# gevaertlab/RNA-GAN

Measured on AMD Instinct MI355X. Metric: training imgs/sec (G+D WGAN-GP step, 256x256), higher is better.
Workload: dtype bf16; 1 GPU; RNA-GAN lung (betaVAE-conditioned wganvae path) 256x256, DCGAN enc2048/step64, per-GPU batch 64, one iteration = G-loss + D-loss + GP steps; global_batch=64, parallelism=dp1, ranks=1, rna_features=19198, hip_graphs=True, dp_statistics=rank-local (DDP)

## Files before the change

include/rnagan_hip.h:

```cpp
#ifndef RNAGAN_HIP_H
#define RNAGAN_HIP_H

#include <stddef.h>
#include <stdint.h>

#ifdef __cplusplus
extern "C" {
#endif

#define RG_OK 0
#define RG_EINVAL (-1)
#define RG_EUNSUPPORTED (-2)
#define RG_EWORKSPACE (-3)
#define RG_EHIP (-4)

#define RG_F32 0
#define RG_BF16 1
#define RG_F16 2

#define RG_ALGO_AUTO 0
#define RG_ALGO_GENERIC 1
#define RG_ALGO_MFMA 2

int rg_version(void);
const char* rg_last_error(void);
int rg_set_option(const char* name, int value);


int rg_pack_conv_weight(const float* w, void* wdn, void* wup, int O, int I, int dtype, void* stream);
int rg_pack_conv_wup_from_bf16(const void* w_bf16, void* wup, int O, int I, void* stream);
int rg_pack_conv_wup_from_bf16_multi(int n, const void* const* w_bf16, void* const* wup, const int* O, const int* I, void* stream);
int rg_pack_g0_weight_from_bf16(const void* w_bf16, void* wp, int E, int C, void* stream);

int rg_conv_stats_rows(int up, int N, int Hlow, int Wlow, int O, int I, int dtype, int algo);
int rg_conv_down(const void* x, const float* w, const void* wdn, void* y, int N, int Hi, int Wi, int I,
                 int O, float* stats_partial, int dtype, int algo, void* ws, size_t ws_bytes, void* stream);
size_t rg_conv_workspace_bytes(int up, int N, int Hlow, int Wlow, int O, int I, int dtype, int algo);

int rg_conv_up(const void* x, const float* w, const void* wup, void* y, int N, int Ho, int Wo, int O, int I,
               const void* mask_act, float mask_slope, float* stats_partial, int dtype, int algo, void* ws,
               size_t ws_bytes, void* stream);

size_t rg_conv_wgrad_workspace_bytes(int N, int Ho, int Wo, int O, int I, int dtype, int algo);
int rg_conv_wgrad(const void* low, const void* high, float* dw, int N, int Ho, int Wo, int O, int I, int dtype,
                  int accumulate, int algo, void* ws, size_t ws_bytes, void* stream);
int rg_conv_wgrad2(const void* low0, const void* high0, const void* low1, const void* high1, float* dw, int N,
                   int Ho, int Wo, int O, int I, int dtype, int accumulate, int algo, void* ws, size_t ws_bytes,
                   void* stream);
int rg_conv_wgrad_slabs(const void* low0, const void* high0, const void* low1, const void* high1, float* dw, int N, int Ho,
                        int Wo, int O, int I, int dtype, int algo, void* slab, size_t slab_bytes, int* nsplit_out,
                        int* slab_dtype_out, void* stream);
int rg_conv_wgrad_adam_supported(int N, int Ho, int Wo, int O, int I, int two, int dtype, int algo);
int rg_conv_wgrad_adam(const void* low0, const void* high0, const void* low1, const void* high1, float* p, float* m, float* v,
                       const float* hyper, void* shadow_bf16, int N, int Ho, int Wo, int O, int I, int dtype, int algo,
                       void* stream);

int rg_first_down(const float* x_nchw, const float* w, const float* bias, void* y, int N, int H, int W, int I,
                  int O, float slope, int dtype, void* stream);
int rg_last_up(const void* x, const float* w, const float* bias, float* y_nchw, int N, int Ho, int Wo, int O,
               int I, int apply_tanh, int dtype, void* stream);
int rg_first_down_bits(const float* x_nchw, const float* w, const float* bias, void* y, void* bits, int N, int H, int W,
                       int I, int O, float slope, int dtype, void* stream);
int rg_sign_pack(const void* a, void* bits, long long npix, int C, int dtype, void* stream);
int rg_first_down_masked_supported(int H, int W, int I, int O, int dtype);
int rg_first_down_masked(const float* x_nchw, const float* w, void* y, const void* mask_bits, float mask_slope, int N,
                         int H, int W, int I, int O, int dtype, void* stream);
int rg_conv_up_maskbits_supported(int N, int Ho, int Wo, int O, int I, int dtype, int algo);
int rg_conv_up_maskbits(const void* x, const void* wup, void* y, int N, int Ho, int Wo, int O, int I,
                        const void* mask_bits, float mask_slope, int dtype, int algo, void* ws, size_t ws_bytes,
                        void* stream);
int rg_last_up_post_blocks(int N, int Ho, int Wo, int O, int I, int dtype);
int rg_last_up_post(const void* x, const float* w, float* y_nchw, int N, int Ho, int Wo, int O, int I, int dtype,
                    const float* tanh_img, float* part, void* stream);
int rg_last_up_part_chan_sum(const float* part, int nblocks, float* out3, int accumulate, void* stream);
int rg_gp_coef_parts(const float* part, int nblocks, float* sq, float* loss, float* coef, float lambd, void* stream);
int rg_gp_coef_parts_scaled(const float* part, int nblocks, float* sq, float* loss, float* coef, float lambd, float in_scale,
                            float out_scale, void* stream);
int rg_gp_coef_parts_scaled_dev(const float* part, int nblocks, float* sq, float* loss, float* coef, float lambd,
                                const int* amp_state, int slot, void* stream);
int rg_last_up_pre_supported(int Wo, int O, int I, int dtype);
int rg_last_up_pre(const void* z, const float* w, const float* bias, float* y_nchw, const float* mean, const float* invstd,
                   const float* gamma, const float* beta, float slope, int N, int Ho, int Wo, int O, int I, int apply_tanh,
                   int dtype, void* stream);
size_t rg_skinny_wgrad_workspace_bytes(int N, int Ho, int Wo, int O, int I);
int rg_skinny_wgrad(const void* low, const float* high_nchw, float* dw, int N, int Ho, int Wo, int O, int I,
                    int dtype, int accumulate, void* ws, size_t ws_bytes, void* stream);
int rg_skinny_wgrad_slabs(const void* low, const float* high_nchw, int N, int Ho, int Wo, int O, int I, int dtype, void* slab,
                          size_t slab_bytes, int* nslab_out, float* bias_slab, int* bias_done_out, void* stream);
int rg_skinny_wgrad_bias(const void* low, const float* high_nchw, float* dw, float* dbias, int N, int Ho, int Wo, int O, int I,
                         int dtype, int accumulate, int bias_accumulate, void* ws, size_t ws_bytes, int* bias_done_out,
                         void* stream);


int rg_pack_g0_weight(const float* w, void* wp, int E, int C, int dtype, void* stream);
int rg_g0_fwd(const float* z, const float* w, const void* wp, void* y, int N, int E, int C, int dtype, int algo,
              void* ws, size_t ws_bytes, void* stream);
size_t rg_g0_workspace_bytes(int N, int E, int C, int dtype, int algo);
int rg_g0_wgrad(const float* z, const void* gy, float* dw, int N, int E, int C, int dtype, int accumulate,
                int algo, void* ws, size_t ws_bytes, void* stream);

int rg_head_fwd(const void* a, const float* w, float* h, float* out, int N, int C, float slope, int dtype,
                void* stream);
int rg_head_fwd_bias(const void* a, const float* w, const float* bias, float* h, float* out, int N, int C, float slope,
                     int dtype, void* stream);
int rg_vec_sum(const float* x, int n, float* out, int accumulate, void* stream);
int rg_head_grad(const float* h, float* gh, int N, float coef, float slope, void* stream);
int rg_head_grad_dev(const float* h, float* gh, int N, float coef, const int* amp_state, int slot, int part, float slope,
                     void* stream);
int rg_head_bwd_data(const float* gh, const float* w, void* ga, int N, int C, int dtype, void* stream);
int rg_head_wgrad(const float* gh, const void* a, float* dw, int N, int C, int dtype, int accumulate,
                  void* stream);

int rg_pack_linear_weight(const float* w, void* wp, int Nout, int K, int Nout_pad, int K_pad, void* stream);
size_t rg_linear_workspace_bytes(int M, int K, int Nout, int algo);
int rg_linear_affine_act(const float* x, int ldx, const float* w, const void* wp, const float* scale,
                         const float* shift, float* y, int ldy, int M, int K, int Nout, float slope, int algo,
                         void* ws, size_t ws_bytes, void* stream);

size_t rg_colreduce_workspace_bytes(int M, int C, int nq);

int rg_bn_stats(const void* z, float* sum, float* sumsq, int M, int C, int dtype, void* ws, size_t ws_bytes,
                void* stream);
int rg_bn_finalize(const float* sum, const float* sumsq, int M, int C, float eps, float momentum, float* mean,
                   float* invstd, float* running_mean, float* running_var, int64_t* num_batches_tracked,
                   void* stream);
int rg_bn_forward(const void* z, int M, int C, float eps, float momentum, const float* gamma, const float* beta,
                  float slope, float* mean, float* invstd, float* running_mean, float* running_var,
                  int64_t* num_batches_tracked, void* a, int dtype, void* ws, size_t ws_bytes, void* stream);
int rg_bn_forward_partials(const float* partial, int G, const void* z, int M, int C, float eps, float momentum,
                           const float* gamma, const float* beta, float slope, float* mean, float* invstd,
                           float* running_mean, float* running_var, int64_t* num_batches_tracked, void* a, int dtype,
                           void* ws, size_t ws_bytes, void* stream);
int rg_bn_stats_finalize(const void* z, int M, int C, float eps, float momentum, float* mean, float* invstd,
                         float* running_mean, float* running_var, int64_t* num_batches_tracked, int dtype, void* ws,
                         size_t ws_bytes, void* stream);
int rg_bn_act(const void* z, const float* mean, const float* invstd, const float* gamma, const float* beta,
              void* a, int M, int C, float slope, int dtype, void* stream);
int rg_bn_act_bwd(const void* z, const void* ga, const float* mean, const float* invstd, const float* gamma,
                  const float* beta, void* gz, float* s_gy, float* s_gyxh, float* dgamma, float* dbeta,
                  int accumulate, int M, int C, float slope, int dtype, void* ws, size_t ws_bytes, void* stream);
int rg_bn_finalize_partials(const float* partial, int G, int M, int C, float eps, float momentum, float* mean,
                            float* invstd, float* running_mean, float* running_var, int64_t* num_batches_tracked, void* ws,
                            size_t ws_bytes, void* stream);
int rg_g0_wgrad_adam_supported(int N, int E, int C, int dtype);
int rg_g0_wgrad_adam(const float* z, const void* gz0, float* p, float* m, float* v, const float* hyper, void* shadow_bf16,
                     int N, int E, int C, int dtype, void* stream);

int rg_linear_wgrad_adam(const void* gT, const void* xT, int ldn, int N, float* p, float* m, float* v, const float* hyper, int O,
                         int I, void* wpack_bf16, int Kp, void* stream);

int rg_im2col_nhwc(const float* x, int ldx, float* cols, int N, int H, int W, int C, int kh, int kw, int sh, int sw, int ph,
                   int pw, void* stream);
int rg_pool2d_nhwc(const float* x, int ldx, float* y, int ldy, int N, int H, int W, int C, int k, int stride, int pad, int mode,
                   void* stream);
int rg_nchw_to_nhwc_affine(const float* x_nchw, float* y_nhwc, int N, int C, int H, int W, const float* scale, const float* shift,
                           void* stream);
int rg_spatial_mean_nhwc(const float* x, float* y, int N, int HW, int C, void* stream);

int rg_conv_split(int up, int N, int Hlow, int Wlow, int O, int I, int dtype, int algo);
int rg_conv_slab_dtype(int up, int N, int Hlow, int Wlow, int O, int I, int dtype, int algo);
int rg_conv_down_partial(const void* x, const void* wdn, int N, int Hi, int Wi, int I, int O, int dtype, int algo,
                         void* ws, size_t ws_bytes, void* stream);
int rg_conv_up_partial(const void* x, const void* wup, int N, int Ho, int Wo, int O, int I, int dtype, int algo,
                       void* ws, size_t ws_bytes, void* stream);
int rg_slab_bn_supported(long long M, int C, int groups, int nsplit);
size_t rg_slab_bn_scratch_bytes(long long M, int C, int groups);
size_t rg_slab_bn_sync_words(void);
int rg_bn_forward_slabs(const void* slab, int nsplit, size_t slab_stride, int slab_dtype, void* z, void* a, long long M, int C, int groups,
                        float eps, float momentum, const float* gamma, const float* beta, float slope, float* mean,
                        float* invstd, float* running_mean, float* running_var, long long* num_batches_tracked,
                        void* scratch, size_t scratch_bytes, void* sync, void* stream);
int rg_bn_tangent_slabs(const void* slab, int nsplit, size_t slab_stride, int slab_dtype, const void* z, void* zt_out, void* at, long long M,
                        int C, const float* mean, const float* invstd, const float* gamma, const float* beta, float slope,
                        float* s_zt, float* s_xhzt, void* scratch, size_t scratch_bytes, void* sync, void* stream);
int rg_bn_act_bwd_slabs(const void* slab, int nsplit, size_t slab_stride, int slab_dtype, const void* z, void* ga_out, void* gz, long long M,
                        int C, int groups, const float* mean, const float* invstd, const float* gamma, const float* beta,
                        float slope, float* s_gy, float* s_gyxh, float* dgamma, float* dbeta, int accumulate, void* scratch,
                        size_t scratch_bytes, void* sync, void* stream);

int rg_bn_finalize_partials_g2(const float* partial, int G, int nblk, int M, int C, float eps, float momentum, float* mean,
                               float* invstd, float* running_mean, float* running_var, int64_t* num_batches_tracked,
                               void* ws, size_t ws_bytes, void* stream);
int rg_bn_forward_g2(const float* partial, int G, int nblk, const void* z, int M, int C, float eps, float momentum,
                     const float* gamma, const float* beta, float slope, float* mean, float* invstd, float* running_mean,
                     float* running_var, int64_t* num_batches_tracked, void* a, int dtype, void* ws, size_t ws_bytes,
                     void* stream);
int rg_bn_act_bwd_g2(const void* z, const void* ga, const float* mean, const float* invstd, const float* gamma,
                     const float* beta, void* gz, float* s_gy, float* s_gyxh, float* dgamma, float* dbeta, int accumulate,
                     int M, int C, float slope, int dtype, void* ws, size_t ws_bytes, void* stream);
int rg_bn_tangent(const void* z, const void* zt, const float* mean, const float* invstd, const float* gamma,
                  const float* beta, void* at, float* s_zt, float* s_xhzt, int M, int C, float slope, int dtype,
                  void* ws, size_t ws_bytes, void* stream);
int rg_bn_double_bwd(const void* z, const void* qa, const void* zt, const void* ga1, const float* mean,
                     const float* invstd, const float* gamma, const float* beta, const float* s_gy,
                     const float* s_gyxh, const float* s_zt, const float* s_xhzt, void* pz, float* dgamma,
                     float* dbeta, int accumulate, int M, int C, float slope, int dtype, void* ws,
                     size_t ws_bytes, void* stream);

int rg_slab_finish_rows(long long M, int C);
int rg_slab_bias_act(const void* slab, int nsplit, size_t stride, int slab_dtype, const float* bias, void* y, long long M, int C,
                     float slope, void* stream);
int rg_slab_mask(const void* slab, int nsplit, size_t stride, int slab_dtype, const void* mask_act, float mask_slope, void* y,
                 float* col_parts, long long M, int C, void* stream);
int rg_parts_col_sum(const float* parts, int rows, int C, float* out, int accumulate, void* stream);
int rg_bias_act(const void* z, const float* bias, void* y, long long M, int C, float slope, int dtype, void* stream);
int rg_conv_down_epi_supported(int N, int Hi, int Wi, int I, int O, int dtype, int algo);
int rg_conv_down_epi(const void* x, const void* wdn, void* y, int N, int Hi, int Wi, int I, int O, const float* shift, float slope,
                     const void* mask_act, float mask_slope, int dtype, int algo, void* ws, size_t ws_bytes, void* stream);

int rg_lrelu_bwd(const void* g, const void* a, void* out, size_t n, float slope, int dtype, void* stream);
int rg_col_sum(const void* g, float* out, int M, int C, int dtype, int accumulate, void* ws, size_t ws_bytes,
               void* stream);

int rg_tanh_bwd(const float* gy, const float* y, float* gz, size_t n, void* stream);
int rg_nchw_chan_sum(const float* g, float* out, int N, int C, int HW, int accumulate, void* ws, size_t ws_bytes,
                     void* stream);
int rg_interp(const float* real, const float* fake, float* out, size_t n, float eps, void* stream);
int rg_interp_dev(const float* real, const float* fake, float* out, size_t n, const float* eps, void* stream);
size_t rg_reduce_workspace_bytes(size_t n);
int rg_sqnorm(const float* x, float* out, size_t n, void* ws, size_t ws_bytes, void* stream);
int rg_gp_coef(const float* sq, float* loss, float* coef, float lambd, void* stream);
int rg_gp_coef_scaled(const float* sq, float* loss, float* coef, float lambd, float in_scale, float out_scale, void* stream);
int rg_gp_coef_scaled_dev(const float* sq, float* loss, float* coef, float lambd, const int* amp_state, int slot, void* stream);
int rg_scale_by(const float* x, const float* coef, float* out, size_t n, void* stream);
int rg_mean_diff(const float* a, const float* b, float* out, int n, float sign, void* stream);
int rg_latent_prep(const float* u, const float* z, float* out, int N, int E, void* stream);

int rg_adam_step(float* p, const float* g, float* m, float* v, size_t n, int step, double lr, double beta1,
                 double beta2, double eps, void* stream);
int rg_clamp(float* p, size_t n, float lo, float hi, void* stream);
int rg_adam_step_dev(float* p, const float* g, float* m, float* v, size_t n, const float* hyper, void* shadow_bf16,
                     const void* grad_bf16, void* stream);
int rg_adam_step_slabs(float* p, const float* g, float* m, float* v, size_t n, const float* hyper, void* shadow_bf16, int nseg,
                       const unsigned long long* seg_off, const unsigned long long* seg_n, const void* const* seg_slab,
                       const int* seg_nsplit, const int* seg_dtype, void* stream);
int rg_grad_to_wire(const float* g, void* wire_bf16, size_t n, int nseg, const unsigned long long* seg_off,
                    const unsigned long long* seg_n, const void* const* seg_slab, const int* seg_nsplit, const int* seg_dtype,
                    void* stream);
int rg_conv_wgrad_wire(const void* low0, const void* high0, const void* low1, const void* high1, void* wire_bf16, int N, int Ho,
                       int Wo, int O, int I, int dtype, int algo, void* stream);
int rg_adam_hyper_dev(int* step_dev, double lr, double beta1, double beta2, double eps, double weight_decay, float* hyper,
                      void* stream);
int rg_adam_hyper_dev2(int* step_dev, double lr, double beta1, double beta2, double eps, double weight_decay,
                       double grad_scale_inv, float* hyper, void* stream);
#define RG_AMP_EXP 0
#define RG_AMP_TRACKER 1
#define RG_AMP_SKIPPED 2
#define RG_AMP_LATCH 4
#define RG_AMP_FLAG 8
#define RG_AMP_SLOTS 4
#define RG_AMP_STATE_INTS 12
int rg_adam_hyper_dev3(int* step_dev, double lr, double beta1, double beta2, double eps, double weight_decay,
                       const int* amp_state, int slot, float* hyper, void* stream);
int rg_ema_update(const float* p, float* e, size_t n, float decay, const int* step_dev, const float* hyper, void* stream);
int rg_nonfinite_probe(int nseg, const void* const* seg_ptr, const unsigned long long* seg_n, const int* seg_dtype, int* flag,
                       void* stream);
int rg_amp_update(int* amp_state, int slot, int growth_interval, int min_exp, int max_exp, void* stream);
int rg_amp_latch(int* amp_state, int slot, void* stream);
int rg_storage_dtype(void);

int rg_transpose_f32(const float* src, float* dst, int R, int C, void* stream);
int rg_transpose_pack_bf16(const float* src, void* dst, int R, int C, int R_pad, int C_pad, void* stream);
size_t rg_gemm_nt_bf16_workspace_bytes(int M, int K_pad, int Nout);
int rg_gemm_nt_bf16(const void* a, const void* b, const float* scale, const float* shift, float* y, int ldy, int M,
                    int K_pad, int Nout, float slope, void* ws, size_t ws_bytes, void* stream);
int rg_vae_dropout(const float* x, const unsigned char* mask, float* y, int N, int F, int ld, float scale, void* stream);
int rg_vae_reparam(const float* mu, const float* logvar, const float* eps, float* z, size_t n, void* stream);
int rg_vae_reparam_bwd(const float* gz, const float* logvar, const float* eps, const float* gmu_loss,
                       const float* glv_loss, float* gmu, float* glv, size_t n, void* stream);
int rg_tanh_inplace(float* x, size_t n, void* stream);
int rg_add_inplace(float* y, const float* x, size_t n, void* stream);
size_t rg_vae_loss_workspace_bytes(void);
int rg_vae_loss(const float* x, const float* x_recons, int N, int F, int ld, const float* z_mean, const float* z_logvar,
                int Z, float beta, int training, float* losses, float* g_recons, float* g_mean, float* g_logvar, void* ws,
                size_t ws_bytes, void* stream);

int rg_widen_bf16(const void* src, float* dst, size_t n, void* stream);
int rg_cast_pad(const float* src, void* dst, int M, int K, int ldd, int dtype, void* stream);

int rg_selftest_layouts(int* detail, void* stream);

size_t rg_upconv3_workspace_bytes(int N, int H, int W, int Cin, int Cout);
int rg_upconv3_fwd(const void* x, const float* w, const float* bias, void* y, int N, int H, int W, int Cin, int Cout,
                   int out_nchw_f32, int dtype, int algo, void* ws, size_t ws_bytes, void* stream);
int rg_upconv3_bwd_data(const void* gy, int gy_nchw_f32, const float* w, void* gx, int N, int H, int W, int Cin,
                        int Cout, int dtype, int algo, void* ws, size_t ws_bytes, void* stream);
int rg_upconv3_wgrad(const void* gy, int gy_nchw_f32, const void* x, float* dw, int N, int H, int W, int Cin, int Cout,
                     int dtype, int algo, int accumulate, void* ws, size_t ws_bytes, void* stream);

int rg_bn_bwd_sums(const void* z, const void* ga, const float* mean, const float* invstd, const float* gamma,
                   const float* beta, float* s_gy, float* s_gyxh, int M, int C, float slope, int dtype, void* ws,
                   size_t ws_bytes, void* stream);
int rg_bn_bwd_apply(const void* z, const void* ga, const float* mean, const float* invstd, const float* gamma,
                    const float* beta, const float* s_gy, const float* s_gyxh, void* gz, int M, int C, int M_total,
                    float slope, int dtype, void* stream);
int rg_bn_tangent_sums(const void* z, const void* zt, const float* mean, const float* invstd, const float* gamma,
                       const float* beta, float* s_zt, float* s_xhzt, int M, int C, float slope, int dtype, void* ws,
                       size_t ws_bytes, void* stream);
int rg_bn_tangent_apply(const void* z, const void* zt, const float* mean, const float* invstd, const float* gamma,
                        const float* beta, const float* s_zt, const float* s_xhzt, void* at, int M, int C, int M_total,
                        float slope, int dtype, void* stream);
int rg_bn_dbl_sums(const void* z, const void* qa, const void* zt, const void* ga1, const float* mean, const float* invstd,
                   const float* gamma, const float* beta, float* raw3, int M, int C, float slope, int dtype, void* ws,
                   size_t ws_bytes, void* stream);
int rg_bn_dbl_apply(const void* z, const void* qa, const void* zt, const void* ga1, const float* mean, const float* invstd,
                    const float* gamma, const float* beta, const float* s_gy, const float* s_gyxh, const float* s_zt,
                    const float* s_xhzt, const float* raw3_global, const float* raw3_local, void* pz, float* dgamma,
                    float* dbeta, int accumulate, int M, int C, int M_total, float slope, int dtype, void* ws,
                    size_t ws_bytes, void* stream);
int rg_latent_stats(const float* u, const float* z, float* s, float* ss, int N, int E, void* stream);
int rg_latent_apply(const float* u, const float* z, const float* s, const float* ss, float* out, int N, int E, int N_total,
                    void* stream);

int rg_export_images_nhwc(const float* x_nchw, float* y_nhwc, int N, int C, int H, int W, void* stream);

int rg_conv_up_affine(const void* x, const void* wup, void* y, int N, int Ho, int Wo, int O, int I, const float* scale,
                      const float* shift, float slope, void* ws, size_t ws_bytes, void* stream);
int rg_g0_fwd_affine(const float* z, const void* wp, void* y, int N, int E, int C, const float* scale, const float* shift,
                     float slope, void* ws, size_t ws_bytes, void* stream);

int rg_conv_up_fp8(const void* x8, const void* wup8, void* y, int N, int Ho, int Wo, int O, int I, const float* scale,
                   const float* shift, float slope, int out_fp8, void* stream);
int rg_gemm_fp8(const void* a8, const void* b8, void* y, int M, int K, int Ncols, const float* scale, const float* shift,
                float slope, int out_fp8, void* stream);
int rg_fp8_supported(int M, int K, int Ncols, int taps);
int rg_cast_fp8(const float* src, void* dst, size_t n, float mul, void* stream);
int rg_selftest_fp8(int* detail, void* stream);

int rg_u8_to_norm(const void* src_u8, float* dst, size_t n, float mean, float stdv, void* stream);

int rg_split_planes(const float* src, void* planes_bf16, size_t n, void* stream);
int rg_f32p_conv_supported(int up, int N, int Hlow, int Wlow, int O, int I, int products);
size_t rg_f32p_conv_workspace_bytes(int up, int N, int Hlow, int Wlow, int O, int I, int products);
int rg_f32p_conv_stats_rows(int up, int N, int Hlow, int Wlow, int O, int I, int products);
int rg_f32p_conv(int up, const void* x_planes, const void* w_planes, float* y, int N, int Hlow, int Wlow, int O, int I,
                 int products, float* stats_partial, const float* mask_f32, float mask_slope, void* ws, size_t ws_bytes,
                 void* stream);
int rg_f32p_conv_mask_supported(int up, int N, int Hlow, int Wlow, int O, int I, int products);
int rg_f32p_wgrad_supported(int N, int Ho, int Wo, int O, int I, int products);
size_t rg_f32p_wgrad_workspace_bytes(int N, int Ho, int Wo, int O, int I, int products, int two);
int rg_f32p_wgrad(const void* low0, const void* high0, const void* low1, const void* high1, float* dw, int N, int Ho, int Wo,
                  int O, int I, int products, int accumulate, void* ws, size_t ws_bytes, void* stream);

int rg_probe_mfma_bare(int mfma_shape, int waves_per_simd, int blocks, int iters, float* scratch, double* flops_out, void* stream);
int rg_probe_lds_mfma(int mfma_shape, int blocks, int iters, const void* a, const void* b, void* c, double* flops_out,
                      void* stream);
int rg_probe_copy(const void* src, void* dst, size_t nbytes, int variant, int blocks, void* stream);
int rg_probe_fill_bf16(void* p, size_t n, unsigned seed, void* stream);


#ifdef __cplusplus
}
#endif
#endif
```

rna_gan_amd/_abi.py:

```python
from __future__ import annotations

import ctypes as C
import os

_HERE = os.path.dirname(os.path.abspath(__file__))
LIB_PATH = os.path.join(_HERE, "librnagan_hip.so")

RG_F32, RG_BF16, RG_F16 = 0, 1, 2
ALGO_AUTO, ALGO_GENERIC, ALGO_MFMA = 0, 1, 2

_p = C.c_void_p
_i = C.c_int
_f = C.c_float
_d = C.c_double
_z = C.c_size_t

PROTOTYPES = {
    "rg_version": (_i, []),
    "rg_last_error": (C.c_char_p, []),
    "rg_set_option": (_i, [C.c_char_p, _i]),
    "rg_pack_conv_weight": (_i, [_p, _p, _p, _i, _i, _i, _p]),
    "rg_conv_stats_rows": (_i, [_i, _i, _i, _i, _i, _i, _i, _i]),
    "rg_conv_down": (_i, [_p, _p, _p, _p, _i, _i, _i, _i, _i, _p, _i, _i, _p, _z, _p]),
    "rg_conv_up": (_i, [_p, _p, _p, _p, _i, _i, _i, _i, _i, _p, _f, _p, _i, _i, _p, _z, _p]),
    "rg_conv_workspace_bytes": (_z, [_i, _i, _i, _i, _i, _i, _i, _i]),
    "rg_conv_wgrad_workspace_bytes": (_z, [_i, _i, _i, _i, _i, _i, _i]),
    "rg_conv_wgrad": (_i, [_p, _p, _p, _i, _i, _i, _i, _i, _i, _i, _i, _p, _z, _p]),
    "rg_conv_wgrad2": (_i, [_p, _p, _p, _p, _p, _i, _i, _i, _i, _i, _i, _i, _i, _p, _z, _p]),
    "rg_conv_wgrad_slabs": (_i, [_p, _p, _p, _p, _p, _i, _i, _i, _i, _i, _i, _i, _p, _z, _p, _p, _p]),
    "rg_grad_to_wire": (_i, [_p, _p, _z, _i, _p, _p, _p, _p, _p, _p]),
    "rg_conv_wgrad_wire": (_i, [_p, _p, _p, _p, _p, _i, _i, _i, _i, _i, _i, _i, _p]),
    "rg_conv_wgrad_adam_supported": (_i, [_i, _i, _i, _i, _i, _i, _i, _i]),
    "rg_conv_wgrad_adam": (_i, [_p, _p, _p, _p, _p, _p, _p, _p, _p, _i, _i, _i, _i, _i, _i, _i, _p]),
    "rg_first_down": (_i, [_p, _p, _p, _p, _i, _i, _i, _i, _i, _f, _i, _p]),
    "rg_first_down_bits": (_i, [_p, _p, _p, _p, _p, _i, _i, _i, _i, _i, _f, _i, _p]),
    "rg_sign_pack": (_i, [_p, _p, C.c_longlong, _i, _i, _p]),
    "rg_first_down_masked_supported": (_i, [_i, _i, _i, _i, _i]),
    "rg_first_down_masked": (_i, [_p, _p, _p, _p, _f, _i, _i, _i, _i, _i, _i, _p]),
    "rg_conv_up_maskbits_supported": (_i, [_i, _i, _i, _i, _i, _i, _i]),
    "rg_conv_up_maskbits": (_i, [_p, _p, _p, _i, _i, _i, _i, _i, _p, _f, _i, _i, _p, _z, _p]),
    "rg_last_up": (_i, [_p, _p, _p, _p, _i, _i, _i, _i, _i, _i, _i, _p]),
    "rg_skinny_wgrad_workspace_bytes": (_z, [_i, _i, _i, _i, _i]),
    "rg_skinny_wgrad": (_i, [_p, _p, _p, _i, _i, _i, _i, _i, _i, _i, _p, _z, _p]),
    "rg_skinny_wgrad_slabs": (_i, [_p, _p, _i, _i, _i, _i, _i, _i, _p, _z, _p, _p, _p, _p]),
    "rg_skinny_wgrad_bias": (_i, [_p, _p, _p, _p, _i, _i, _i, _i, _i, _i, _i, _i, _p, _z, _p, _p]),
    "rg_pack_g0_weight": (_i, [_p, _p, _i, _i, _i, _p]),
    "rg_pack_conv_wup_from_bf16": (_i, [_p, _p, _i, _i, _p]),
    "rg_pack_conv_wup_from_bf16_multi": (_i, [_i, _p, _p, _p, _p, _p]),
    "rg_pack_g0_weight_from_bf16": (_i, [_p, _p, _i, _i, _p]),
    "rg_g0_fwd": (_i, [_p, _p, _p, _p, _i, _i, _i, _i, _i, _p, _z, _p]),
    "rg_g0_workspace_bytes": (_z, [_i, _i, _i, _i, _i]),
    "rg_g0_wgrad": (_i, [_p, _p, _p, _i, _i, _i, _i, _i, _i, _p, _z, _p]),
    "rg_head_fwd": (_i, [_p, _p, _p, _p, _i, _i, _f, _i, _p]),
    "rg_head_grad": (_i, [_p, _p, _i, _f, _f, _p]),
    "rg_head_grad_dev": (_i, [_p, _p, _i, _f, _p, _i, _i, _f, _p]),
    "rg_adam_hyper_dev3": (_i, [_p, _d, _d, _d, _d, _d, _p, _i, _p, _p]),
    "rg_nonfinite_probe": (_i, [_i, _p, _p, _p, _p, _p]),
    "rg_amp_update": (_i, [_p, _i, _i, _i, _i, _p]),
    "rg_amp_latch": (_i, [_p, _i, _p]),
    "rg_gp_coef_scaled_dev": (_i, [_p, _p, _p, _f, _p, _i, _p]),
    "rg_gp_coef_parts_scaled_dev": (_i, [_p, _i, _p, _p, _p, _f, _p, _i, _p]),
    "rg_head_bwd_data": (_i, [_p, _p, _p, _i, _i, _i, _p]),
    "rg_head_wgrad": (_i, [_p, _p, _p, _i, _i, _i, _i, _p]),
    "rg_pack_linear_weight": (_i, [_p, _p, _i, _i, _i, _i, _p]),
    "rg_linear_workspace_bytes": (_z, [_i, _i, _i, _i]),
    "rg_linear_affine_act": (_i, [_p, _i, _p, _p, _p, _p, _p, _i, _i, _i, _i, _f, _i, _p, _z, _p]),
    "rg_colreduce_workspace_bytes": (_z, [_i, _i, _i]),
    "rg_bn_stats": (_i, [_p, _p, _p, _i, _i, _i, _p, _z, _p]),
    "rg_bn_finalize": (_i, [_p, _p, _i, _i, _f, _f, _p, _p, _p, _p, _p, _p]),
    "rg_bn_forward": (_i, [_p, _i, _i, _f, _f, _p, _p, _f, _p, _p, _p, _p, _p, _p, _i, _p, _z, _p]),
    "rg_bn_forward_partials": (_i, [_p, _i, _p, _i, _i, _f, _f, _p, _p, _f, _p, _p, _p, _p, _p, _p, _i, _p, _z, _p]),
    "rg_bn_stats_finalize": (_i, [_p, _i, _i, _f, _f, _p, _p, _p, _p, _p, _i, _p, _z, _p]),
    "rg_bn_act": (_i, [_p, _p, _p, _p, _p, _p, _i, _i, _f, _i, _p]),
    "rg_bn_act_bwd": (_i, [_p, _p, _p, _p, _p, _p, _p, _p, _p, _p, _p, _i, _i, _i, _f, _i, _p, _z, _p]),
    "rg_bn_act_bwd_g2": (_i, [_p, _p, _p, _p, _p, _p, _p, _p, _p, _p, _p, _i, _i, _i, _f, _i, _p, _z, _p]),
    "rg_bn_finalize_partials": (_i, [_p, _i, _i, _i, _f, _f, _p, _p, _p, _p, _p, _p, _z, _p]),
    "rg_linear_wgrad_adam": (_i, [_p, _p, _i, _i, _p, _p, _p, _p, _i, _i, _p, _i, _p]),
    "rg_last_up_post_blocks": (_i, [_i, _i, _i, _i, _i, _i]),
    "rg_last_up_post": (_i, [_p, _p, _p, _i, _i, _i, _i, _i, _i, _p, _p, _p]),
    "rg_last_up_part_chan_sum": (_i, [_p, _i, _p, _i, _p]),
    "rg_gp_coef_parts": (_i, [_p, _i, _p, _p, _p, _f, _p]),
    "rg_last_up_pre_supported": (_i, [_i, _i, _i, _i]),
    "rg_last_up_pre": (_i, [_p, _p, _p, _p, _p, _p, _p, _p, _f, _i, _i, _i, _i, _i, _i, _i, _p]),
    "rg_bn_forward_g2": (_i, [_p, _i, _i, _p, _i, _i, _f, _f, _p, _p, _f, _p, _p, _p, _p, _p, _p, _i, _p, _z, _p]),
    "rg_bn_finalize_partials_g2": (_i, [_p, _i, _i, _i, _i, _f, _f, _p, _p, _p, _p, _p, _p, _z, _p]),
    "rg_bn_tangent": (_i, [_p, _p, _p, _p, _p, _p, _p, _p, _p, _i, _i, _f, _i, _p, _z, _p]),
    "rg_bn_double_bwd": (_i, [_p, _p, _p, _p, _p, _p, _p, _p, _p, _p, _p, _p, _p, _p, _p, _i, _i, _i, _f, _i,
                              _p, _z, _p]),
    "rg_lrelu_bwd": (_i, [_p, _p, _p, _z, _f, _i, _p]),
    "rg_col_sum": (_i, [_p, _p, _i, _i, _i, _i, _p, _z, _p]),
    "rg_tanh_bwd": (_i, [_p, _p, _p, _z, _p]),
    "rg_nchw_chan_sum": (_i, [_p, _p, _i, _i, _i, _i, _p, _z, _p]),
    "rg_interp": (_i, [_p, _p, _p, _z, _f, _p]),
    "rg_reduce_workspace_bytes": (_z, [_z]),
    "rg_sqnorm": (_i, [_p, _p, _z, _p, _z, _p]),
    "rg_gp_coef": (_i, [_p, _p, _p, _f, _p]),
    "rg_scale_by": (_i, [_p, _p, _p, _z, _p]),
    "rg_mean_diff": (_i, [_p, _p, _p, _i, _f, _p]),
    "rg_latent_prep": (_i, [_p, _p, _p, _i, _i, _p]),
    "rg_adam_step": (_i, [_p, _p, _p, _p, _z, _i, _d, _d, _d, _d, _p]),
    "rg_clamp": (_i, [_p, _z, _f, _f, _p]),
    "rg_upconv3_workspace_bytes": (_z, [_i, _i, _i, _i, _i]),
    "rg_upconv3_fwd": (_i, [_p, _p, _p, _p, _i, _i, _i, _i, _i, _i, _i, _i, _p, _z, _p]),
    "rg_upconv3_bwd_data": (_i, [_p, _i, _p, _p, _i, _i, _i, _i, _i, _i, _i, _p, _z, _p]),
    "rg_upconv3_wgrad": (_i, [_p, _i, _p, _p, _i, _i, _i, _i, _i, _i, _i, _i, _p, _z, _p]),
    "rg_export_images_nhwc": (_i, [_p, _p, _i, _i, _i, _i, _p]),
    "rg_bn_bwd_sums": (_i, [_p, _p, _p, _p, _p, _p, _p, _p, _i, _i, _f, _i, _p, _z, _p]),
    "rg_bn_bwd_apply": (_i, [_p, _p, _p, _p, _p, _p, _p, _p, _p, _i, _i, _i, _f, _i, _p]),
    "rg_bn_tangent_sums": (_i, [_p, _p, _p, _p, _p, _p, _p, _p, _i, _i, _f, _i, _p, _z, _p]),
    "rg_bn_tangent_apply": (_i, [_p, _p, _p, _p, _p, _p, _p, _p, _p, _i, _i, _i, _f, _i, _p]),
    "rg_bn_dbl_sums": (_i, [_p, _p, _p, _p, _p, _p, _p, _p, _p, _i, _i, _f, _i, _p, _z, _p]),
    "rg_bn_dbl_apply": (_i, [_p] * 17 + [_i, _i, _i, _i, _f, _i, _p, _z, _p]),
    "rg_latent_stats": (_i, [_p, _p, _p, _p, _i, _i, _p]),
    "rg_latent_apply": (_i, [_p, _p, _p, _p, _p, _i, _i, _i, _p]),
    "rg_adam_step_dev": (_i, [_p, _p, _p, _p, _z, _p, _p, _p, _p]),
    "rg_adam_step_slabs": (_i, [_p, _p, _p, _p, _z, _p, _p, _i, _p, _p, _p, _p, _p, _p]),
    "rg_ema_update": (_i, [_p, _p, _z, _f, _p, _p, _p]),
    "rg_interp_dev": (_i, [_p, _p, _p, _z, _p, _p]),
    "rg_adam_hyper_dev": (_i, [_p, _d, _d, _d, _d, _d, _p, _p]),
    "rg_adam_hyper_dev2": (_i, [_p, _d, _d, _d, _d, _d, _d, _p, _p]),
    "rg_storage_dtype": (_i, []),
    "rg_gp_coef_scaled": (_i, [_p, _p, _p, _f, _f, _f, _p]),
    "rg_gp_coef_parts_scaled": (_i, [_p, _i, _p, _p, _p, _f, _f, _f, _p]),
    "rg_transpose_f32": (_i, [_p, _p, _i, _i, _p]),
    "rg_transpose_pack_bf16": (_i, [_p, _p, _i, _i, _i, _i, _p]),
    "rg_gemm_nt_bf16_workspace_bytes": (_z, [_i, _i, _i]),
    "rg_gemm_nt_bf16": (_i, [_p, _p, _p, _p, _p, _i, _i, _i, _i, _f, _p, _z, _p]),
    "rg_vae_dropout": (_i, [_p, _p, _p, _i, _i, _i, _f, _p]),
    "rg_vae_reparam": (_i, [_p, _p, _p, _p, _z, _p]),
    "rg_vae_reparam_bwd": (_i, [_p, _p, _p, _p, _p, _p, _p, _z, _p]),
    "rg_tanh_inplace": (_i, [_p, _z, _p]),
    "rg_add_inplace": (_i, [_p, _p, _z, _p]),
    "rg_vae_loss_workspace_bytes": (_z, []),
    "rg_vae_loss": (_i, [_p, _p, _i, _i, _i, _p, _p, _i, _f, _i, _p, _p, _p, _p, _p, _z, _p]),
    "rg_widen_bf16": (_i, [_p, _p, _z, _p]),
    "rg_cast_pad": (_i, [_p, _p, _i, _i, _i, _i, _p]),
    "rg_selftest_layouts": (_i, [_p, _p]),
    "rg_u8_to_norm": (_i, [_p, _p, _z, _f, _f, _p]),
    "rg_conv_up_fp8": (_i, [_p, _p, _p, _i, _i, _i, _i, _i, _p, _p, _f, _i, _p]),
    "rg_gemm_fp8": (_i, [_p, _p, _p, _i, _i, _i, _p, _p, _f, _i, _p]),
    "rg_fp8_supported": (_i, [_i, _i, _i, _i]),
    "rg_cast_fp8": (_i, [_p, _p, _z, _f, _p]),
    "rg_selftest_fp8": (_i, [_p, _p]),
    "rg_g0_wgrad_adam_supported": (_i, [_i, _i, _i, _i]),
    "rg_g0_wgrad_adam": (_i, [_p, _p, _p, _p, _p, _p, _p, _i, _i, _i, _i, _p]),
    "rg_im2col_nhwc": (_i, [_p, _i, _p, _i, _i, _i, _i, _i, _i, _i, _i, _i, _i, _p]),
    "rg_pool2d_nhwc": (_i, [_p, _i, _p, _i, _i, _i, _i, _i, _i, _i, _i, _i, _p]),
    "rg_nchw_to_nhwc_affine": (_i, [_p, _p, _i, _i, _i, _i, _p, _p, _p]),
    "rg_spatial_mean_nhwc": (_i, [_p, _p, _i, _i, _i, _p]),
    "rg_conv_split": (_i, [_i, _i, _i, _i, _i, _i, _i, _i]),
    "rg_conv_slab_dtype": (_i, [_i, _i, _i, _i, _i, _i, _i, _i]),
    "rg_conv_down_partial": (_i, [_p, _p, _i, _i, _i, _i, _i, _i, _i, _p, _z, _p]),
    "rg_conv_up_partial": (_i, [_p, _p, _i, _i, _i, _i, _i, _i, _i, _p, _z, _p]),
    "rg_slab_bn_supported": (_i, [C.c_longlong, _i, _i, _i]),
    "rg_slab_bn_scratch_bytes": (_z, [C.c_longlong, _i, _i]),
    "rg_slab_bn_sync_words": (_z, []),
    "rg_bn_forward_slabs": (_i, [_p, _i, _z, _i, _p, _p, C.c_longlong, _i, _i, _f, _f, _p, _p, _f, _p, _p, _p, _p, _p, _p, _z, _p, _p]),
    "rg_bn_tangent_slabs": (_i, [_p, _i, _z, _i, _p, _p, _p, C.c_longlong, _i, _p, _p, _p, _p, _f, _p, _p, _p, _z, _p, _p]),
    "rg_bn_act_bwd_slabs": (_i, [_p, _i, _z, _i, _p, _p, _p, C.c_longlong, _i, _i, _p, _p, _p, _p, _f, _p, _p, _p, _p, _i, _p, _z,
                                 _p, _p]),
    "rg_conv_up_affine": (_i, [_p, _p, _p, _i, _i, _i, _i, _i, _p, _p, _f, _p, _z, _p]),
    "rg_g0_fwd_affine": (_i, [_p, _p, _p, _i, _i, _i, _p, _p, _f, _p, _z, _p]),
    "rg_split_planes": (_i, [_p, _p, _z, _p]),
    "rg_f32p_conv_supported": (_i, [_i, _i, _i, _i, _i, _i, _i]),
    "rg_f32p_conv_workspace_bytes": (_z, [_i, _i, _i, _i, _i, _i, _i]),
    "rg_f32p_conv_stats_rows": (_i, [_i, _i, _i, _i, _i, _i, _i]),
    "rg_f32p_conv": (_i, [_i, _p, _p, _p, _i, _i, _i, _i, _i, _i, _p, _p, _f, _p, _z, _p]),
    "rg_f32p_conv_mask_supported": (_i, [_i, _i, _i, _i, _i, _i, _i]),
    "rg_f32p_wgrad_supported": (_i, [_i, _i, _i, _i, _i, _i]),
    "rg_f32p_wgrad_workspace_bytes": (_z, [_i, _i, _i, _i, _i, _i, _i]),
    "rg_f32p_wgrad": (_i, [_p, _p, _p, _p, _p, _i, _i, _i, _i, _i, _i, _i, _p, _z, _p]),
    "rg_slab_finish_rows": (_i, [C.c_longlong, _i]),
    "rg_slab_bias_act": (_i, [_p, _i, _z, _i, _p, _p, C.c_longlong, _i, _f, _p]),
    "rg_slab_mask": (_i, [_p, _i, _z, _i, _p, _f, _p, _p, C.c_longlong, _i, _p]),
    "rg_parts_col_sum": (_i, [_p, _i, _i, _p, _i, _p]),
    "rg_bias_act": (_i, [_p, _p, _p, C.c_longlong, _i, _f, _i, _p]),
    "rg_vec_sum": (_i, [_p, _i, _p, _i, _p]),
    "rg_conv_down_epi_supported": (_i, [_i, _i, _i, _i, _i, _i, _i]),
    "rg_conv_down_epi": (_i, [_p, _p, _p, _i, _i, _i, _i, _i, _p, _f, _p, _f, _i, _i, _p, _z, _p]),
    "rg_head_fwd_bias": (_i, [_p, _p, _p, _p, _p, _i, _i, _f, _i, _p]),
    "rg_probe_mfma_bare": (_i, [_i, _i, _i, _i, _p, _p, _p]),
    "rg_probe_lds_mfma": (_i, [_i, _i, _i, _p, _p, _p, _p, _p]),
    "rg_probe_copy": (_i, [_p, _p, _z, _i, _i, _p]),
    "rg_probe_fill_bf16": (_i, [_p, _z, C.c_uint, _p]),
}

ABI_VERSION = 615

_libs = {}
LIB_PATH_F16 = os.path.join(_HERE, "librnagan_hip_f16.so")
BF16_ONLY_PREFIXES = ("rg_probe_", "rg_split_planes", "rg_f32p_")


def load(half: str = "bf16"):
    if half in _libs:
        return _libs[half]
    if half not in ("bf16", "f16"):
        raise ValueError("half must be 'bf16' or 'f16'")
    path = LIB_PATH if half == "bf16" else LIB_PATH_F16
    if not os.path.exists(path):
        raise RuntimeError(
            "rna_gan_amd: %s not found. Build it with `python -m rna_gan_amd.build` "
            "(hipcc --offload-arch=gfx950). There is no CPU / eager fallback." % path)
    try:
        lib = C.CDLL(path)
    except OSError as e:
        raise RuntimeError("rna_gan_amd: cannot load %s: %s" % (path, e))
    for name, (res, args) in PROTOTYPES.items():
        if half == "f16" and name.startswith(BF16_ONLY_PREFIXES):
            continue
        fn = getattr(lib, name, None)
        if fn is None:
            raise RuntimeError("rna_gan_amd: symbol %s missing from %s: the library is older than this package -- rebuild "
                               "it with `python -m rna_gan_amd.build`" % (name, path))
        fn.restype = res
        fn.argtypes = args
    got = lib.rg_version()
    if got != ABI_VERSION:
        raise RuntimeError("rna_gan_amd: %s reports ABI version %d, this package binds version %d (a stale or swapped "
                           "build): rebuild it with `python -m rna_gan_amd.build`" % (path, got, ABI_VERSION))
    want = RG_BF16 if half == "bf16" else RG_F16
    if lib.rg_storage_dtype() != want:
        raise RuntimeError("rna_gan_amd: %s stores dtype code %d, expected %d (a swapped build)" % (path, lib.rg_storage_dtype(), want))
    _libs[half] = lib
    return lib


_LAST_ERR_LIBS = ("bf16", "f16")


def check(rc: int, what: str):
    if rc != 0:
        msgs = []
        for h in _LAST_ERR_LIBS:
            if h in _libs:
                m = _libs[h].rg_last_error()
                if m:
                    msgs.append(m.decode() if len(_libs) == 1 else "[%s build] %s" % (h, m.decode()))
        raise RuntimeError("rna_gan_amd: %s failed (%d): %s" % (what, rc, " | ".join(msgs) if msgs else "?"))
```

rna_gan_amd/build.py:

```python
import os
import subprocess
import sys
from concurrent.futures import ThreadPoolExecutor

HERE = os.path.dirname(os.path.abspath(__file__))
CSRC = os.path.join(HERE, "csrc")
OUT = os.path.join(HERE, "librnagan_hip.so")
OUT_F16 = os.path.join(HERE, "librnagan_hip_f16.so")
OBJ = os.path.join(HERE, "csrc", "_obj")
SOURCES = ["rg_api.hip", "rg_generic.hip", "rg_bn.hip", "rg_misc.hip", "rg_mfma.hip", "rg_conv8.hip", "rg_convp.hip", "rg_convd.hip", "rg_wgrad8.hip", "rg_skinny.hip", "rg_vae.hip", "rg_splitbn.hip", "rg_incep.hip", "rg_g0adam.hip", "rg_upimg.hip", "rg_probe.hip", "rg_conv8f.hip", "rg_wgrad8f.hip", "rg_amp.hip", "rg_plainact.hip"]
EXTRA_DEPS = {"rg_probe.hip": ["rg_conv8.hip"], "rg_conv8f.hip": ["rg_conv8.hip"], "rg_wgrad8f.hip": ["rg_wgrad8.hip"]}
BF16_ONLY = ("rg_probe.hip", "rg_conv8f.hip", "rg_wgrad8f.hip")
FLAGS = ["--offload-arch=gfx950", "-O3", "-fPIC", "-std=c++17", "-Wall", "-Wno-unused-function",
         "-ffp-contract=off"]


def _stale(target, deps):
    if not os.path.exists(target):
        return True
    t = os.path.getmtime(target)
    return any(os.path.getmtime(d) > t for d in deps)


def build_library(force=False, verbose=True, half="bf16"):
    if half not in ("bf16", "f16"):
        raise ValueError("half must be 'bf16' or 'f16'")
    hipcc = os.environ.get("HIPCC", "/opt/rocm/bin/hipcc")
    if not os.path.exists(hipcc):
        hipcc = "hipcc"
    f16 = half == "f16"
    objdir = OBJ + ("_f16" if f16 else "")
    out = OUT_F16 if f16 else OUT
    sources = [s for s in SOURCES if not (f16 and s in BF16_ONLY)]
    flags = FLAGS + (["-DRG_HALF_F16=1"] if f16 else [])
    os.makedirs(objdir, exist_ok=True)
    headers = [os.path.join(CSRC, f) for f in os.listdir(CSRC) if f.endswith(".h")]
    headers.append(os.path.join(os.path.dirname(HERE), "include", "rnagan_hip.h"))
    jobs = []
    for s in sources:
        src = os.path.join(CSRC, s)
        obj = os.path.join(objdir, s.replace(".hip", ".o"))
        if force or _stale(obj, [src] + headers + [os.path.join(CSRC, d) for d in EXTRA_DEPS.get(s, [])]):
            jobs.append((src, obj))

    def cc(job):
        src, obj = job
        cmd = [hipcc] + flags + ["-c", src, "-o", obj]
        r = subprocess.run(cmd, capture_output=True, text=True)
        if r.returncode != 0:
            raise RuntimeError("hipcc failed for %s:\n%s" % (src, r.stderr[-4000:]))
        if verbose and r.stderr.strip():
            sys.stderr.write(r.stderr[-2000:])
        return obj

    with ThreadPoolExecutor(max_workers=6) as ex:
        list(ex.map(cc, jobs))
    objs = [os.path.join(objdir, s.replace(".hip", ".o")) for s in sources]
    if force or jobs or _stale(out, objs):
        cmd = [hipcc, "--offload-arch=gfx950", "-shared", "-fPIC", "-o", out] + objs
        r = subprocess.run(cmd, capture_output=True, text=True)
        if r.returncode != 0:
            raise RuntimeError("link failed:\n%s" % r.stderr[-4000:])
    return out


def build_all(force=False, verbose=True):
    return [build_library(force, verbose, "bf16"), build_library(force, verbose, "f16")]


def build_debug_library(force=False):
    hipcc = os.environ.get("HIPCC", "/opt/rocm/bin/hipcc")
    if not os.path.exists(hipcc):
        hipcc = "hipcc"
    d = os.path.join(os.path.dirname(HERE), "tools", "debug")
    src = os.path.join(d, "rg_debug_hold.hip")
    d_out = d if os.access(d, os.W_OK) else os.path.join(os.path.expanduser("~"), ".cache", "rna_gan_amd")
    os.makedirs(d_out, exist_ok=True)
    out = os.path.join(d_out, "librnagan_debug.so")
    if force or _stale(out, [src]):
        tmp = "%s.%d.tmp" % (out, os.getpid())
        r = subprocess.run([hipcc, "--offload-arch=gfx950", "-O3", "-fPIC", "-shared", "-o", tmp, src], capture_output=True, text=True)
        if r.returncode != 0:
            raise RuntimeError("hipcc failed for %s:\n%s" % (src, r.stderr[-4000:]))
        os.replace(tmp, out)
    return out


if __name__ == "__main__":
    print("\n".join(build_all(force="--force" in sys.argv)))
```

rna_gan_amd/csrc/rg_api.hip:

```cpp
#include "rg_common.h"
#include "rg_internal.h"
#include <stdarg.h>
#include <stdio.h>
#include <stdlib.h>
#include <string.h>
#include <ctype.h>

static thread_local char g_err[512] = "";

void rg_set_error(const char* fmt, ...) {
  va_list ap;
  va_start(ap, fmt);
  vsnprintf(g_err, sizeof(g_err), fmt, ap);
  va_end(ap);
}

extern "C" int rg_version(void) { return 615; }
extern "C" const char* rg_last_error(void) { return g_err; }

static const char* const g_opt_names[] = {"conv8", "conv8_blocks", "conv_tile", "xcd", "class_fast", "wgrad_blocks",
                                          "wgrad8", "conv_v1", "stream_tile", "narrow8", "conv8_mfma", "conv8_epi", "wgrad8_blocks", "korder", "convp", "convp_blocks",
                                          "fp8_mx", "wgrad8n", "f32mma", "convd", "convd_blocks", "skinny128", "slab16", "wslab16", "bn_rev", "wgrad8_mfma", "narrow32", "upimg", "upimg_blocks"};
constexpr int G_NOPT = sizeof(g_opt_names) / sizeof(g_opt_names[0]);
static int g_opt_override[G_NOPT];
static int g_opt_env[G_NOPT];

int rg_option(const char* name, int dflt) {
  for (int i = 0; i < G_NOPT; ++i) {
    if (strcmp(name, g_opt_names[i]) != 0) continue;
    if (g_opt_override[i] > 0) return g_opt_override[i] - 1;
    if (g_opt_env[i] == 0) {
      char var[64] = "RNAGAN_";
      size_t n = strlen(var);
      for (const char* c = name; *c && n + 1 < sizeof(var); ++c) var[n++] = (char)toupper((unsigned char)*c);
      var[n] = 0;
      const char* e = getenv(var);
      g_opt_env[i] = e ? atoi(e) + 1 : -1;
      if (g_opt_env[i] == 0) g_opt_env[i] = -1;
    }
    return g_opt_env[i] > 0 ? g_opt_env[i] - 1 : dflt;
  }
  return dflt;
}

extern "C" int rg_set_option(const char* name, int value) {
  RG_REQUIRE(name, RG_EINVAL, "set_option: null name");
  for (int i = 0; i < G_NOPT; ++i)
    if (strcmp(name, g_opt_names[i]) == 0) { g_opt_override[i] = value < 0 ? 0 : value + 1; return RG_OK; }
  rg_set_error("set_option: unknown option '%s'", name);
  return RG_EINVAL;
}

static bool want_mfma(int algo, int dtype) { return algo != RG_ALGO_GENERIC && dtype == RG_H16; }

extern "C" int rg_pack_conv_weight(const float* w, void* wdn, void* wup, int O, int I, int dtype, void* stream) {
  RG_REQUIRE(w && O > 0 && I > 0, RG_EINVAL, "pack_conv_weight: bad args");
  RG_REQUIRE(dtype == RG_H16, RG_EUNSUPPORTED, "pack_conv_weight: only bf16 packs exist (fp32 kernels read w)");
  return rg_mfma_pack_conv_weight(w, wdn, wup, O, I, rg_stream(stream));
}

extern "C" size_t rg_conv_workspace_bytes(int up, int N, int Hlow, int Wlow, int O, int I, int dtype, int algo) {
  if (!want_mfma(algo, dtype)) return 0;
  if (!rg_mfma_conv_supported(N, Hlow, Wlow, up ? O : I, up ? I : O)) return 0;
  return rg_mfma_conv_ws_bytes(up, N, Hlow, Wlow, O, I);
}

extern "C" int rg_conv_stats_rows(int up, int N, int Hlow, int Wlow, int O, int I, int dtype, int algo) {
  if (N <= 0 || Hlow <= 0 || Wlow <= 0 || O <= 0 || I <= 0 || !want_mfma(algo, dtype)) return 0;
  if (!rg_mfma_conv_supported(N, Hlow, Wlow, up ? O : I, up ? I : O)) return 0;
  return rg_mfma_conv_stats_rows(up, N, Hlow, Wlow, O, I);
}

extern "C" int rg_conv_split(int up, int N, int Hlow, int Wlow, int O, int I, int dtype, int algo) {
  if (N <= 0 || Hlow <= 0 || Wlow <= 0 || O <= 0 || I <= 0 || !want_mfma(algo, dtype)) return 1;
  if (!rg_mfma_conv_supported(N, Hlow, Wlow, up ? O : I, up ? I : O)) return 1;
  return rg_mfma_conv_nsplit(up, N, Hlow, Wlow, O, I);
}

extern "C" int rg_conv_slab_dtype(int up, int N, int Hlow, int Wlow, int O, int I, int dtype, int algo) {
  if (rg_conv_split(up, N, Hlow, Wlow, O, I, dtype, algo) <= 1) return RG_F32;
  return rg_mfma_conv_slab16(up, N, Hlow, Wlow, O, I) ? RG_H16 : RG_F32;
}

extern "C" int rg_conv_down_partial(const void* x, const void* wdn, int N, int Hi, int Wi, int I, int O, int dtype, int algo,
                                    void* ws, size_t ws_bytes, void* stream) {
  RG_REQUIRE(x && wdn && ws && N > 0 && Hi > 0 && Wi > 0 && I > 0 && O > 0 && Hi % 2 == 0 && Wi % 2 == 0, RG_EINVAL,
             "conv_down_partial: bad args");
  RG_REQUIRE(rg_conv_split(0, N, Hi / 2, Wi / 2, O, I, dtype, algo) > 1, RG_EUNSUPPORTED,
             "conv_down_partial: this shape does not run split-K (rg_conv_split)");
  return rg_mfma_conv_down(x, wdn, nullptr, N, Hi, Wi, I, O, nullptr, ws, ws_bytes, rg_stream(stream), 1);
}

extern "C" int rg_conv_up_partial(const void* x, const void* wup, int N, int Ho, int Wo, int O, int I, int dtype, int algo,
                                  void* ws, size_t ws_bytes, void* stream) {
  RG_REQUIRE(x && wup && ws && N > 0 && Ho > 0 && Wo > 0 && I > 0 && O > 0, RG_EINVAL, "conv_up_partial: bad args");
  RG_REQUIRE(rg_conv_split(1, N, Ho, Wo, O, I, dtype, algo) > 1, RG_EUNSUPPORTED,
             "conv_up_partial: this shape does not run split-K (rg_conv_split)");
  return rg_mfma_conv_up(x, wup, nullptr, N, Ho, Wo, O, I, nullptr, 1.f, nullptr, ws, ws_bytes, rg_stream(stream), nullptr,
                         nullptr, 1.f, 0, 1);
}

extern "C" int rg_conv_down(const void* x, const float* w, const void* wdn, void* y, int N, int Hi, int Wi, int I,
                            int O, float* stats_partial, int dtype, int algo, void* ws, size_t ws_bytes, void* stream) {
  RG_REQUIRE(x && y && N > 0 && Hi > 0 && Wi > 0 && I > 0 && O > 0 && Hi % 2 == 0 && Wi % 2 == 0, RG_EINVAL,
             "conv_down: bad args");
  if (want_mfma(algo, dtype) && wdn && rg_mfma_conv_supported(N, Hi / 2, Wi / 2, I, O))
    return rg_mfma_conv_down(x, wdn, y, N, Hi, Wi, I, O, stats_partial, ws, ws_bytes, rg_stream(stream));
  RG_REQUIRE(!stats_partial, RG_EUNSUPPORTED, "conv_down: statistics come from the MFMA epilogue only");
  RG_REQUIRE(algo != RG_ALGO_MFMA, RG_EUNSUPPORTED, "conv_down: shape/dtype not supported by the MFMA kernel");
  RG_REQUIRE(w, RG_EINVAL, "conv_down: generic kernel needs the fp32 master weight");
  return rg_generic_conv_down(x, w, y, N, Hi, Wi, I, O, dtype, rg_stream(stream));
}

extern "C" int rg_conv_up(const void* x, const float* w, const void* wup, void* y, int N, int Ho, int Wo, int O, int I,
                          const void* mask_act, float mask_slope, float* stats_partial, int dtype, int algo, void* ws,
                          size_t ws_bytes, void* stream) {
  RG_REQUIRE(x && y && N > 0 && Ho > 0 && Wo > 0 && I > 0 && O > 0, RG_EINVAL, "conv_up: bad args");
  RG_REQUIRE(!(mask_act && stats_partial), RG_EINVAL, "conv_up: mask and statistics are exclusive");
  if (want_mfma(algo, dtype) && wup && rg_mfma_conv_supported(N, Ho, Wo, O, I))
    return rg_mfma_conv_up(x, wup, y, N, Ho, Wo, O, I, mask_act, mask_slope, stats_partial, ws, ws_bytes,
                           rg_stream(stream));
  RG_REQUIRE(!stats_partial, RG_EUNSUPPORTED, "conv_up: statistics come from the MFMA epilogue only");
  RG_REQUIRE(algo != RG_ALGO_MFMA, RG_EUNSUPPORTED, "conv_up: shape/dtype not supported by the MFMA kernel");
  RG_REQUIRE(w, RG_EINVAL, "conv_up: generic kernel needs the fp32 master weight");
  return rg_generic_conv_up(x, w, y, N, Ho, Wo, O, I, mask_act, mask_slope, dtype, rg_stream(stream));
}

extern "C" size_t rg_conv_wgrad_workspace_bytes(int N, int Ho, int Wo, int O, int I, int dtype, int algo) {
  size_t a = rg_generic_wgrad_ws_bytes(N, Ho, Wo, O, I);
  size_t b = 0;
  if (want_mfma(algo, dtype) && rg_mfma_wgrad_supported(N, Ho, Wo, O, I)) {
    b = rg_mfma_wgrad_ws_bytes(N, Ho, Wo, O, I);
    size_t c = rg_mfma_wgrad2_ws_bytes(N, Ho, Wo, O, I);
    if (c > b) b = c;
  }
  return a > b ? a : b;
}

extern "C" int rg_conv_wgrad2(const void* low0, const void* high0, const void* low1, const void* high1, float* dw,
                              int N, int Ho, int Wo, int O, int I, int dtype, int accumulate, int algo, void* ws,
                              size_t ws_bytes, void* stream) {
  RG_REQUIRE(low0 && high0 && low1 && high1 && dw && N > 0 && Ho > 0 && Wo > 0 && I > 0 && O > 0, RG_EINVAL,
             "conv_wgrad2: bad args");
  if (want_mfma(algo, dtype) && rg_mfma_wgrad_supported(N, Ho, Wo, O, I))
    return rg_mfma_conv_wgrad2(low0, high0, low1, high1, dw, N, Ho, Wo, O, I, accumulate, ws, ws_bytes,
                               rg_stream(stream));
  RG_REQUIRE(algo != RG_ALGO_MFMA, RG_EUNSUPPORTED, "conv_wgrad2: shape/dtype not supported by the MFMA kernel");
  int rc = rg_generic_conv_wgrad(low0, high0, dw, N, Ho, Wo, O, I, dtype, accumulate, ws, ws_bytes, rg_stream(stream));
  if (rc) return rc;
  return rg_generic_conv_wgrad(low1, high1, dw, N, Ho, Wo, O, I, dtype, 1, ws, ws_bytes, rg_stream(stream));
}

extern "C" int rg_conv_wgrad_slabs(const void* low0, const void* high0, const void* low1, const void* high1, float* dw, int N,
                                   int Ho, int Wo, int O, int I, int dtype, int algo, void* slab, size_t slab_bytes,
                                   int* nsplit_out, int* slab_dtype_out, void* stream) {
  RG_REQUIRE(low0 && high0 && dw && nsplit_out && slab_dtype_out && (low1 == nullptr) == (high1 == nullptr) && N > 0 && Ho > 0 &&
                 Wo > 0 && I > 0 && O > 0, RG_EINVAL, "conv_wgrad_slabs: bad args");
  *slab_dtype_out = RG_F32;
  if (!(want_mfma(algo, dtype) && rg_mfma_wgrad_supported(N, Ho, Wo, O, I))) {
    *nsplit_out = 1;
    RG_REQUIRE(algo != RG_ALGO_MFMA, RG_EUNSUPPORTED, "conv_wgrad_slabs: shape/dtype not supported by the MFMA kernel");
    int rc = rg_generic_conv_wgrad(low0, high0, dw, N, Ho, Wo, O, I, dtype, 0, slab, slab_bytes, rg_stream(stream));
    if (rc || !low1) return rc;
    return rg_generic_conv_wgrad(low1, high1, dw, N, Ho, Wo, O, I, dtype, 1, slab, slab_bytes, rg_stream(stream));
  }
  return rg_mfma_conv_wgrad2(low0, high0, low1, high1, dw, N, Ho, Wo, O, I, 0, slab, slab_bytes, rg_stream(stream), nsplit_out,
                             slab_dtype_out);
}

extern "C" int rg_conv_wgrad_adam_supported(int N, int Ho, int Wo, int O, int I, int two, int dtype, int algo) {
  return N > 0 && Ho > 0 && Wo > 0 && O > 0 && I > 0 && want_mfma(algo, dtype) && rg_mfma_wgrad_supported(N, Ho, Wo, O, I) &&
         rg_mfma_conv_wgrad_adam_supported(N, Ho, Wo, O, I, two != 0) ? 1 : 0;
}
extern "C" int rg_conv_wgrad_adam(const void* low0, const void* high0, const void* low1, const void* high1, float* p, float* m,
                                  float* v, const float* hyper, void* shadow_bf16, int N, int Ho, int Wo, int O, int I, int dtype,
                                  int algo, void* stream) {
  RG_REQUIRE(low0 && high0 && p && m && v && hyper && (low1 == nullptr) == (high1 == nullptr) && N > 0 && Ho > 0 && Wo > 0 &&
                 I > 0 && O > 0, RG_EINVAL, "conv_wgrad_adam: bad args");
  RG_REQUIRE((((uintptr_t)p | (uintptr_t)m | (uintptr_t)v) & 15) == 0 && ((uintptr_t)shadow_bf16 & 7) == 0, RG_EINVAL,
             "conv_wgrad_adam: p, m, v must be 16-byte aligned (the bf16 image 8-byte)");
  RG_REQUIRE(rg_conv_wgrad_adam_supported(N, Ho, Wo, O, I, low1 != nullptr, dtype, algo), RG_EUNSUPPORTED,
             "conv_wgrad_adam: shape / dtype without a single-split matrix-core plan");
  return rg_mfma_conv_wgrad_adam(low0, high0, low1, high1, N, Ho, Wo, O, I, p, m, v, (uint16_t*)shadow_bf16, hyper,
                                 rg_stream(stream));
}

extern "C" int rg_conv_wgrad_wire(const void* low0, const void* high0, const void* low1, const void* high1, void* wire_bf16, int N,
                                  int Ho, int Wo, int O, int I, int dtype, int algo, void* stream) {
  RG_REQUIRE(low0 && high0 && wire_bf16 && (low1 == nullptr) == (high1 == nullptr) && N > 0 && Ho > 0 && Wo > 0 && I > 0 && O > 0,
             RG_EINVAL, "conv_wgrad_wire: bad args");
  RG_REQUIRE(((uintptr_t)wire_bf16 & 15) == 0, RG_EINVAL, "conv_wgrad_wire: the wire slice must be 16-byte aligned");
  RG_REQUIRE(rg_conv_wgrad_adam_supported(N, Ho, Wo, O, I, low1 != nullptr, dtype, algo), RG_EUNSUPPORTED,
             "conv_wgrad_wire: shape / dtype without a single-split matrix-core plan");
  return rg_mfma_conv_wgrad_wire(low0, high0, low1, high1, N, Ho, Wo, O, I, (uint16_t*)wire_bf16, rg_stream(stream));
}

extern "C" int rg_conv_wgrad(const void* low, const void* high, float* dw, int N, int Ho, int Wo, int O, int I,
                             int dtype, int accumulate, int algo, void* ws, size_t ws_bytes, void* stream) {
  RG_REQUIRE(low && high && dw && N > 0 && Ho > 0 && Wo > 0 && I > 0 && O > 0, RG_EINVAL, "conv_wgrad: bad args");
  if (want_mfma(algo, dtype) && rg_mfma_wgrad_supported(N, Ho, Wo, O, I))
    return rg_mfma_conv_wgrad2(low, high, nullptr, nullptr, dw, N, Ho, Wo, O, I, accumulate, ws, ws_bytes,
                               rg_stream(stream));
  RG_REQUIRE(algo != RG_ALGO_MFMA, RG_EUNSUPPORTED, "conv_wgrad: shape/dtype not supported by the MFMA kernel");
  return rg_generic_conv_wgrad(low, high, dw, N, Ho, Wo, O, I, dtype, accumulate, ws, ws_bytes, rg_stream(stream));
}

extern "C" int rg_first_down(const float* x_nchw, const float* w, const float* bias, void* y, int N, int H, int W,
                             int I, int O, float slope, int dtype, void* stream) {
  RG_REQUIRE(x_nchw && w && y && N > 0 && H > 0 && W > 0 && H % 2 == 0 && W % 2 == 0 && I > 0 && O > 0, RG_EINVAL,
             "first_down: bad args");
  if (rg_skinny_supported(I, O) && !(dtype == RG_F32 && rg_generic_f32_image_side(N, H, W, I, O)))
    return rg_skinny_first_down(x_nchw, w, bias, y, nullptr, N, H, W, I, O, slope, dtype, rg_stream(stream));
  return rg_generic_first_down(x_nchw, w, bias, y, N, H, W, I, O, slope, dtype, rg_stream(stream));
}

extern "C" int rg_first_down_bits(const float* x_nchw, const float* w, const float* bias, void* y, void* bits, int N, int H,
                                  int W, int I, int O, float slope, int dtype, void* stream) {
  RG_REQUIRE(x_nchw && w && y && bits && N > 0 && H > 0 && W > 0 && H % 2 == 0 && W % 2 == 0 && I > 0 && O == 64 &&
                 dtype == RG_H16, RG_EINVAL, "first_down_bits: bad args (64 bf16 output channels)");
  if (rg_skinny_supported(I, O))
    return rg_skinny_first_down(x_nchw, w, bias, y, bits, N, H, W, I, O, slope, dtype, rg_stream(stream));
  int rc = rg_generic_first_down(x_nchw, w, bias, y, N, H, W, I, O, slope, dtype, rg_stream(stream));
  return rc != RG_OK ? rc : rg_skinny_sign_pack(y, bits, (long long)N * (H / 2) * (W / 2), O, dtype, rg_stream(stream));
}

extern "C" int rg_first_down_masked_supported(int H, int W, int I, int O, int dtype) {
  return rg_skinny_supported(I, O) && rg_skinny_first_down_masked_supported(H, W, I, O, dtype);
}
extern "C" int rg_first_down_masked(const float* x_nchw, const float* w, void* y, const void* mask_bits, float mask_slope,
                                    int N, int H, int W, int I, int O, int dtype, void* stream) {
  RG_REQUIRE(x_nchw && w && y && mask_bits && N > 0 && H > 0 && W > 0 && H % 2 == 0 && W % 2 == 0, RG_EINVAL,
             "first_down_masked: bad args");
  RG_REQUIRE(rg_first_down_masked_supported(H, W, I, O, dtype), RG_EUNSUPPORTED, "first_down_masked: shape");
  return rg_skinny_first_down_masked(x_nchw, w, y, mask_bits, mask_slope, N, H, W, I, O, dtype, rg_stream(stream));
}

extern "C" int rg_sign_pack(const void* a, void* bits, long long npix, int C, int dtype, void* stream) {
  RG_REQUIRE(a && bits && npix > 0, RG_EINVAL, "sign_pack: bad args");
  return rg_skinny_sign_pack(a, bits, npix, C, dtype, rg_stream(stream));
}

extern "C" int rg_conv_up_maskbits_supported(int N, int Ho, int Wo, int O, int I, int dtype, int algo) {
  return want_mfma(algo, dtype) && N > 0 && Ho > 0 && Wo > 0 && rg_mfma_conv_supported(N, Ho, Wo, O, I) &&
         rg_mfma_conv_up_maskbits_supported(N, Ho, Wo, O, I);
}

extern "C" int rg_conv_up_maskbits(const void* x, const void* wup, void* y, int N, int Ho, int Wo, int O, int I,
                                   const void* mask_bits, float mask_slope, int dtype, int algo, void* ws, size_t ws_bytes,
                                   void* stream) {
  RG_REQUIRE(x && wup && y && mask_bits, RG_EINVAL, "conv_up_maskbits: bad args");
  RG_REQUIRE(rg_conv_up_maskbits_supported(N, Ho, Wo, O, I, dtype, algo), RG_EUNSUPPORTED, "conv_up_maskbits: shape");
  return rg_mfma_conv_up(x, wup, y, N, Ho, Wo, O, I, mask_bits, mask_slope, nullptr, ws, ws_bytes, rg_stream(stream),
                         nullptr, nullptr, 1.f, 1);
}

extern "C" int rg_last_up_pre_supported(int Wo, int O, int I, int dtype) {
  return rg_skinny_supported(I, O) && rg_skinny_last_up_pre_supported(Wo, O, dtype);
}
extern "C" int rg_last_up_pre(const void* z, const float* w, const float* bias, float* y_nchw, const float* mean,
                              const float* invstd, const float* gamma, const float* beta, float slope, int N, int Ho, int Wo,
                              int O, int I, int apply_tanh, int dtype, void* stream) {
  RG_REQUIRE(z && w && y_nchw && mean && invstd && gamma && beta && N > 0 && Ho > 0 && Wo > 0, RG_EINVAL,
             "last_up_pre: bad args");
  RG_REQUIRE(rg_last_up_pre_supported(Wo, O, I, dtype), RG_EUNSUPPORTED, "last_up_pre: shape");
  return rg_skinny_last_up(z, w, bias, y_nchw, N, Ho, Wo, O, I, apply_tanh, dtype, rg_stream(stream), mean, invstd, gamma,
                           beta, slope);
}

extern "C" int rg_last_up(const void* x, const float* w, const float* bias, float* y_nchw, int N, int Ho, int Wo,
                          int O, int I, int apply_tanh, int dtype, void* stream) {
  RG_REQUIRE(x && w && y_nchw && N > 0 && Ho > 0 && Wo > 0 && I > 0 && O > 0, RG_EINVAL, "last_up: bad args");
  if (rg_skinny_supported(I, O))
    return rg_skinny_last_up(x, w, bias, y_nchw, N, Ho, Wo, O, I, apply_tanh, dtype, rg_stream(stream));
  return rg_generic_last_up(x, w, bias, y_nchw, N, Ho, Wo, O, I, apply_tanh, dtype, rg_stream(stream));
}

extern "C" int rg_last_up_post_blocks(int N, int Ho, int Wo, int O, int I, int dtype) {
  return rg_skinny_supported(I, O) ? rg_skinny_last_up_post_blocks(N, Ho, Wo, O, dtype) : 0;
}
extern "C" int rg_last_up_post(const void* x, const float* w, float* y_nchw, int N, int Ho, int Wo, int O, int I, int dtype,
                               const float* tanh_img, float* part, void* stream) {
  RG_REQUIRE(x && w && y_nchw && N > 0 && Ho > 0 && Wo > 0 && (tanh_img || part), RG_EINVAL, "last_up_post: bad args");
  RG_REQUIRE(rg_last_up_post_blocks(N, Ho, Wo, O, I, dtype) > 0, RG_EUNSUPPORTED, "last_up_post: shape");
  RG_REQUIRE((((uintptr_t)tanh_img | (uintptr_t)part) & 15) == 0, RG_EINVAL, "last_up_post: 16-byte aligned buffers required");
  return rg_skinny_last_up(x, w, nullptr, y_nchw, N, Ho, Wo, O, I, 0, dtype, rg_stream(stream), nullptr, nullptr, nullptr,
                           nullptr, 1.f, tanh_img, part);
}
extern "C" int rg_last_up_part_chan_sum(const float* part, int nblocks, float* out3, int accumulate, void* stream) {
  RG_REQUIRE(part && out3 && nblocks > 0, RG_EINVAL, "last_up_part_chan_sum: bad args");
  return rg_skinny_lu_part_final(part, nblocks, out3, accumulate, 0, nullptr, nullptr, 0.f, rg_stream(stream));
}
extern "C" int rg_gp_coef_parts_scaled(const float* part, int nblocks, float* sq, float* loss, float* coef, float lambd,
                                       float in_scale, float out_scale, void* stream) {
  RG_REQUIRE(part && loss && coef && nblocks > 0 && in_scale > 0.f && out_scale > 0.f, RG_EINVAL, "gp_coef_parts: bad args");
  return rg_skinny_lu_part_final(part, nblocks, sq, 0, 1, loss, coef, lambd, rg_stream(stream), in_scale, out_scale);
}
extern "C" int rg_storage_dtype(void) { return RG_H16; }
extern "C" int rg_gp_coef_parts(const float* part, int nblocks, float* sq, float* loss, float* coef, float lambd,
                                void* stream) {
  RG_REQUIRE(part && loss && coef && nblocks > 0, RG_EINVAL, "gp_coef_parts: bad args");
  return rg_skinny_lu_part_final(part, nblocks, sq, 0, 1, loss, coef, lambd, rg_stream(stream));
}

extern "C" size_t rg_skinny_wgrad_workspace_bytes(int N, int Ho, int Wo, int O, int I) {
  size_t a = rg_generic_wgrad_ws_bytes(N, Ho, Wo, O, I);
  size_t b = rg_skinny_supported(I, O) ? rg_skinny_wgrad_ws_bytes(N, Ho, Wo, O, I) : 0;
  return a > b ? a : b;
}

extern "C" int rg_skinny_wgrad(const void* low, const float* high_nchw, float* dw, int N, int Ho, int Wo, int O, int I,
                               int dtype, int accumulate, void* ws, size_t ws_bytes, void* stream) {
  RG_REQUIRE(low && high_nchw && dw && N > 0 && Ho > 0 && Wo > 0 && I > 0 && O > 0, RG_EINVAL,
             "skinny_wgrad: bad args");
  if (rg_skinny_supported(I, O) && !(dtype == RG_F32 && rg_generic_f32_image_side(N, 2 * Ho, 2 * Wo, I, O)))
    return rg_skinny_wgrad_impl(low, high_nchw, dw, N, Ho, Wo, O, I, dtype, accumulate, ws, ws_bytes,
                                rg_stream(stream));
  return rg_generic_skinny_wgrad(low, high_nchw, dw, N, Ho, Wo, O, I, dtype, accumulate, ws, ws_bytes,
                                 rg_stream(stream));
}

extern "C" int rg_skinny_wgrad_bias(const void* low, const float* high_nchw, float* dw, float* dbias, int N, int Ho, int Wo, int O,
                                    int I, int dtype, int accumulate, int bias_accumulate, void* ws, size_t ws_bytes,
                                    int* bias_done_out, void* stream) {
  RG_REQUIRE(low && high_nchw && dw && bias_done_out && N > 0 && Ho > 0 && Wo > 0 && I > 0 && O > 0, RG_EINVAL,
             "skinny_wgrad_bias: bad args");
// ... 191 lines not shown
```

rna_gan_amd/csrc/rg_misc.hip:

```cpp
#include "rg_common.h"

namespace {

constexpr int RED_BLOCKS = 1024;

inline unsigned grid_for(size_t n, int per_thread = 1) {
  size_t b = (n + (size_t)256 * per_thread - 1) / ((size_t)256 * per_thread);
  if (b > 8192) b = 8192;
  if (b < 1) b = 1;
  return (unsigned)b;
}

template <class F>
__global__ __launch_bounds__(256) void ew4_kernel(F f, size_t n) {
  size_t n4 = n / 4;
  size_t stride = (size_t)gridDim.x * blockDim.x;
  for (size_t i = (size_t)blockIdx.x * blockDim.x + threadIdx.x; i < n4; i += stride) f.vec(i * 4);
  size_t t = n4 * 4 + (size_t)blockIdx.x * blockDim.x + threadIdx.x;
  if (t < n) f.one(t);
}

struct TanhBwd {
  const float* gy; const float* y; float* gz;
  __device__ void vec(size_t i) const {
    float4 g = *(const float4*)(gy + i), v = *(const float4*)(y + i);
    *(float4*)(gz + i) = make_float4(g.x * (1.f - v.x * v.x), g.y * (1.f - v.y * v.y), g.z * (1.f - v.z * v.z),
                                     g.w * (1.f - v.w * v.w));
  }
  __device__ void one(size_t i) const { gz[i] = gy[i] * (1.f - y[i] * y[i]); }
};
struct Interp {
  const float* r; const float* f; float* o; float eps;
  __device__ void vec(size_t i) const {
    float4 a = *(const float4*)(r + i), b = *(const float4*)(f + i);
    float e = eps, e1 = 1.f - eps;
    *(float4*)(o + i) = make_float4(e * a.x + e1 * b.x, e * a.y + e1 * b.y, e * a.z + e1 * b.z, e * a.w + e1 * b.w);
  }
  __device__ void one(size_t i) const { o[i] = eps * r[i] + (1.f - eps) * f[i]; }
};
struct InterpDev {
  const float* r; const float* f; float* o; const float* eps;
  __device__ void vec(size_t i) const {
    float4 a = *(const float4*)(r + i), b = *(const float4*)(f + i);
    float e = eps[0], e1 = 1.f - e;
    *(float4*)(o + i) = make_float4(e * a.x + e1 * b.x, e * a.y + e1 * b.y, e * a.z + e1 * b.z, e * a.w + e1 * b.w);
  }
  __device__ void one(size_t i) const { float e = eps[0]; o[i] = e * r[i] + (1.f - e) * f[i]; }
};
struct ScaleBy {
  const float* x; const float* coef; float* o;
  __device__ void vec(size_t i) const {
    float c = coef[0];
    float4 a = *(const float4*)(x + i);
    *(float4*)(o + i) = make_float4(a.x * c, a.y * c, a.z * c, a.w * c);
  }
  __device__ void one(size_t i) const { o[i] = x[i] * coef[0]; }
};
struct Clamp {
  float* p; float lo, hi;
  __device__ void vec(size_t i) const {
    float4 a = *(float4*)(p + i);
    *(float4*)(p + i) = make_float4(fminf(fmaxf(a.x, lo), hi), fminf(fmaxf(a.y, lo), hi), fminf(fmaxf(a.z, lo), hi),
                                    fminf(fmaxf(a.w, lo), hi));
  }
  __device__ void one(size_t i) const { p[i] = fminf(fmaxf(p[i], lo), hi); }
};
struct Adam {
  float* p; const float* g; float* m; float* v; float b1, b2, omb1, omb2, eps, step_size, inv_sqrt_bc2, wd = 0.f;
  float ginv = 1.f;
  __device__ __forceinline__ void upd(float& pp, float gg, float& mm, float& vv) const {
    rg_adam_upd(pp, gg * ginv, mm, vv, b2, omb1, omb2, eps, step_size, inv_sqrt_bc2, wd);
  }
  __device__ void vec(size_t i) const {
    float4 P = *(float4*)(p + i), G = *(const float4*)(g + i), M = *(float4*)(m + i), V = *(float4*)(v + i);
    upd(P.x, G.x, M.x, V.x); upd(P.y, G.y, M.y, V.y); upd(P.z, G.z, M.z, V.z); upd(P.w, G.w, M.w, V.w);
    *(float4*)(p + i) = P; *(float4*)(m + i) = M; *(float4*)(v + i) = V;
  }
  __device__ void one(size_t i) const { upd(p[i], g[i], m[i], v[i]); }
};

typedef float nt_f4 __attribute__((ext_vector_type(4)));
__device__ __forceinline__ float4 nt_ld4(const float* p) {
  nt_f4 t = __builtin_nontemporal_load(reinterpret_cast<const nt_f4*>(p));
  return make_float4(t.x, t.y, t.z, t.w);
}
__device__ __forceinline__ void nt_st4(float* p, float4 v) {
  nt_f4 t = {v.x, v.y, v.z, v.w};
  __builtin_nontemporal_store(t, reinterpret_cast<nt_f4*>(p));
}
template <bool WIRE, bool SHADOW>
__global__ __launch_bounds__(256) void adam_dev_kernel(float* __restrict__ p, const float* __restrict__ g,
                                                       float* __restrict__ m, float* __restrict__ v,
                                                       const float* __restrict__ hyper, uint16_t* __restrict__ shadow,
                                                       const uint16_t* __restrict__ gw, size_t n) {
  if (hyper[9] != 0.f) return;
  const Adam a{p, g, m, v, hyper[0], hyper[1], hyper[2], hyper[3], hyper[4], hyper[5], hyper[6], hyper[7], hyper[8]};
  const size_t n4 = n / 4, stride = (size_t)gridDim.x * blockDim.x;
  for (size_t q = (size_t)blockIdx.x * blockDim.x + threadIdx.x; q < n4; q += stride) {
    const size_t i = q * 4;
    float4 P = *(float4*)(p + i), M = nt_ld4(m + i), V = nt_ld4(v + i), G;
    if (WIRE) {
      const uint2 w = *(const uint2*)(gw + i);
      G = make_float4(h16lo_to_f32(w.x), h16hi_to_f32(w.x), h16lo_to_f32(w.y),
                      h16hi_to_f32(w.y));
    } else {
      G = nt_ld4(g + i);
    }
    a.upd(P.x, G.x, M.x, V.x); a.upd(P.y, G.y, M.y, V.y); a.upd(P.z, G.z, M.z, V.z); a.upd(P.w, G.w, M.w, V.w);
    *(float4*)(p + i) = P; nt_st4(m + i, M); nt_st4(v + i, V);
    if (SHADOW)
      *(uint2*)(shadow + i) = make_uint2((uint32_t)f32_to_h16(P.x) | ((uint32_t)f32_to_h16(P.y) << 16),
                                         (uint32_t)f32_to_h16(P.z) | ((uint32_t)f32_to_h16(P.w) << 16));
  }
  const size_t t = n4 * 4 + (size_t)blockIdx.x * blockDim.x + threadIdx.x;
  if (t < n) {
    a.upd(p[t], WIRE ? h16_to_f32(gw[t]) : g[t], m[t], v[t]);
    if (SHADOW) shadow[t] = f32_to_h16(p[t]);
  }
}

constexpr unsigned EMA_MAX_BLOCKS = 2048;
__global__ __launch_bounds__(256) void ema_kernel(const float* __restrict__ p, float* __restrict__ e, size_t n, float decay,
                                                  const int* __restrict__ step_dev, const float* __restrict__ hyper) {
  if (hyper != nullptr && hyper[9] != 0.f) return;
  float d = decay;
  if (step_dev != nullptr) {
    const float t = (float)step_dev[0];
    d = fminf(decay, (1.f + t) / (10.f + t));
  }
  const float omd = 1.f - d;
  const size_t n4 = n / 4, stride = (size_t)gridDim.x * blockDim.x;
  for (size_t q = (size_t)blockIdx.x * blockDim.x + threadIdx.x; q < n4; q += stride) {
    const size_t i = q * 4;
    const float4 P = *(const float4*)(p + i);
    float4 E = nt_ld4(e + i);
    E.x = E.x + omd * (P.x - E.x); E.y = E.y + omd * (P.y - E.y); E.z = E.z + omd * (P.z - E.z); E.w = E.w + omd * (P.w - E.w);
    nt_st4(e + i, E);
  }
  const size_t t = n4 * 4 + (size_t)blockIdx.x * blockDim.x + threadIdx.x;
  if (t < n) e[t] = e[t] + omd * (p[t] - e[t]);
}

constexpr int ADAM_MAX_SEGS = 24;
struct AdamSeg { unsigned long long off, n; const float* slab; int nsplit; int s16; };
struct AdamSegs { int nseg; int pad; AdamSeg s[ADAM_MAX_SEGS]; };

template <bool S16>
__device__ __forceinline__ float4 adam_slab_ld(const float* __restrict__ slab, size_t z, size_t n, size_t q) {
  if (S16) {
    typedef unsigned nt_u2 __attribute__((ext_vector_type(2)));
    const nt_u2 w = __builtin_nontemporal_load(reinterpret_cast<const nt_u2*>(reinterpret_cast<const uint16_t*>(slab) + z * n + q * 4));
    return make_float4(h16lo_to_f32(w.x), h16hi_to_f32(w.x), h16lo_to_f32(w.y),
                       h16hi_to_f32(w.y));
  }
  return nt_ld4(slab + z * n + q * 4);
}

template <bool SHADOW, int SL, bool S16>
__device__ __forceinline__ void adam_slab_segment(const Adam& a, float* __restrict__ p, float* __restrict__ m,
                                                  float* __restrict__ v, uint16_t* __restrict__ shadow,
                                                  const float* __restrict__ slab, int nsplit, size_t n, float4 (*sm)[64]) {
  constexpr int COLS = 256 / SL;
  const int col = threadIdx.x % COLS, l = threadIdx.x / COLS;
  const size_t n4 = n / 4;
  const size_t trips = (n4 + COLS - 1) / COLS;
  for (size_t tb = blockIdx.x; tb < trips; tb += gridDim.x) {
    const size_t q = tb * COLS + col;
    float4 s = make_float4(0.f, 0.f, 0.f, 0.f);
    if (q < n4) {
      int z = l;
      for (; z + 7 * SL < nsplit; z += 8 * SL) {
        float4 t[8];
#pragma unroll
        for (int k = 0; k < 8; ++k) t[k] = adam_slab_ld<S16>(slab, (size_t)(z + k * SL), n, q);
#pragma unroll
        for (int k = 0; k < 8; ++k) { s.x += t[k].x; s.y += t[k].y; s.z += t[k].z; s.w += t[k].w; }
      }
      for (; z < nsplit; z += SL) {
        const float4 t = adam_slab_ld<S16>(slab, (size_t)z, n, q);
        s.x += t.x; s.y += t.y; s.z += t.z; s.w += t.w;
      }
    }
    if (SL > 1) {
      __syncthreads();
      sm[l][col] = s;
      __syncthreads();
      if (l == 0) {
#pragma unroll
        for (int k = 1; k < SL; ++k) { const float4 t = sm[k][col]; s.x += t.x; s.y += t.y; s.z += t.z; s.w += t.w; }
      }
    }
    if (l == 0 && q < n4) {
      const size_t i = q * 4;
      float4 P = *(float4*)(p + i), M = nt_ld4(m + i), V = nt_ld4(v + i);
      a.upd(P.x, s.x, M.x, V.x); a.upd(P.y, s.y, M.y, V.y); a.upd(P.z, s.z, M.z, V.z); a.upd(P.w, s.w, M.w, V.w);
      *(float4*)(p + i) = P; nt_st4(m + i, M); nt_st4(v + i, V);
      if (SHADOW)
        *(uint2*)(shadow + i) = make_uint2((uint32_t)f32_to_h16(P.x) | ((uint32_t)f32_to_h16(P.y) << 16),
                                           (uint32_t)f32_to_h16(P.z) | ((uint32_t)f32_to_h16(P.w) << 16));
    }
  }
}

template <bool SHADOW>
__global__ __launch_bounds__(256) void adam_segs_kernel(float* __restrict__ p, const float* __restrict__ g,
                                                        float* __restrict__ m, float* __restrict__ v,
                                                        const float* __restrict__ hyper, uint16_t* __restrict__ shadow,
                                                        AdamSegs t) {
  __shared__ float4 sm[16][64];
  if (hyper[9] != 0.f) return;
  const Adam a{p, g, m, v, hyper[0], hyper[1], hyper[2], hyper[3], hyper[4], hyper[5], hyper[6], hyper[7], hyper[8]};
  for (int si = 0; si < t.nseg; ++si) {
    const AdamSeg sg = t.s[si];
    if (sg.nsplit < 0) continue;
    float* ps = p + sg.off; float* ms = m + sg.off; float* vs = v + sg.off;
    uint16_t* sh = SHADOW ? shadow + sg.off : nullptr;
    if (sg.slab) {
      if (sg.s16) {
        if (sg.nsplit <= 4) adam_slab_segment<SHADOW, 1, true>(a, ps, ms, vs, sh, sg.slab, sg.nsplit, sg.n, sm);
        else if (sg.nsplit <= 32) adam_slab_segment<SHADOW, 4, true>(a, ps, ms, vs, sh, sg.slab, sg.nsplit, sg.n, sm);
        else adam_slab_segment<SHADOW, 16, true>(a, ps, ms, vs, sh, sg.slab, sg.nsplit, sg.n, reinterpret_cast<float4(*)[64]>(sm));
      } else {
        if (sg.nsplit <= 4) adam_slab_segment<SHADOW, 1, false>(a, ps, ms, vs, sh, sg.slab, sg.nsplit, sg.n, sm);
        else if (sg.nsplit <= 32) adam_slab_segment<SHADOW, 4, false>(a, ps, ms, vs, sh, sg.slab, sg.nsplit, sg.n, sm);
        else adam_slab_segment<SHADOW, 16, false>(a, ps, ms, vs, sh, sg.slab, sg.nsplit, sg.n, reinterpret_cast<float4(*)[64]>(sm));
      }
      continue;
    }
    const float* gs = g + sg.off;
    const size_t n4 = sg.n / 4, stride = (size_t)gridDim.x * blockDim.x;
    for (size_t q = (size_t)blockIdx.x * blockDim.x + threadIdx.x; q < n4; q += stride) {
      const size_t i = q * 4;
      float4 P = *(float4*)(ps + i), M = nt_ld4(ms + i), V = nt_ld4(vs + i), G = nt_ld4(gs + i);
      a.upd(P.x, G.x, M.x, V.x); a.upd(P.y, G.y, M.y, V.y); a.upd(P.z, G.z, M.z, V.z); a.upd(P.w, G.w, M.w, V.w);
      *(float4*)(ps + i) = P; nt_st4(ms + i, M); nt_st4(vs + i, V);
      if (SHADOW)
        *(uint2*)(sh + i) = make_uint2((uint32_t)f32_to_h16(P.x) | ((uint32_t)f32_to_h16(P.y) << 16),
                                       (uint32_t)f32_to_h16(P.z) | ((uint32_t)f32_to_h16(P.w) << 16));
    }
    const size_t tl = n4 * 4 + (size_t)blockIdx.x * blockDim.x + threadIdx.x;
    if (tl < sg.n) {
      a.upd(ps[tl], gs[tl], ms[tl], vs[tl]);
      if (SHADOW) sh[tl] = f32_to_h16(ps[tl]);
    }
  }
}

template <int SL, bool S16>
__device__ __forceinline__ void wire_slab_segment(uint16_t* __restrict__ wire, const float* __restrict__ slab, int nsplit,
                                                  size_t n, float4 (*sm)[64]) {
  constexpr int COLS = 256 / SL;
  const int col = threadIdx.x % COLS, l = threadIdx.x / COLS;
  const size_t n4 = n / 4;
  const size_t trips = (n4 + COLS - 1) / COLS;
  for (size_t tb = blockIdx.x; tb < trips; tb += gridDim.x) {
    const size_t q = tb * COLS + col;
    float4 s = make_float4(0.f, 0.f, 0.f, 0.f);
    if (q < n4) {
      int z = l;
      for (; z + 7 * SL < nsplit; z += 8 * SL) {
        float4 t[8];
#pragma unroll
        for (int k = 0; k < 8; ++k) t[k] = adam_slab_ld<S16>(slab, (size_t)(z + k * SL), n, q);
#pragma unroll
        for (int k = 0; k < 8; ++k) { s.x += t[k].x; s.y += t[k].y; s.z += t[k].z; s.w += t[k].w; }
      }
      for (; z < nsplit; z += SL) {
        const float4 t = adam_slab_ld<S16>(slab, (size_t)z, n, q);
        s.x += t.x; s.y += t.y; s.z += t.z; s.w += t.w;
      }
    }
    if (SL > 1) {
      __syncthreads();
      sm[l][col] = s;
      __syncthreads();
      if (l == 0) {
#pragma unroll
        for (int k = 1; k < SL; ++k) { const float4 t = sm[k][col]; s.x += t.x; s.y += t.y; s.z += t.z; s.w += t.w; }
      }
    }
    if (l == 0 && q < n4)
      *(uint2*)(wire + q * 4) = make_uint2((uint32_t)f32_to_h16(s.x) | ((uint32_t)f32_to_h16(s.y) << 16),
                                           (uint32_t)f32_to_h16(s.z) | ((uint32_t)f32_to_h16(s.w) << 16));
  }
}

__global__ __launch_bounds__(256) void wire_segs_kernel(const float* __restrict__ g, uint16_t* __restrict__ wire, AdamSegs t) {
  __shared__ float4 sm[16][64];
  for (int si = 0; si < t.nseg; ++si) {
    const AdamSeg sg = t.s[si];
    if (sg.nsplit < 0) continue;
    uint16_t* ws = wire + sg.off;
    if (sg.slab) {
      if (sg.s16) {
        if (sg.nsplit <= 4) wire_slab_segment<1, true>(ws, sg.slab, sg.nsplit, sg.n, sm);
        else if (sg.nsplit <= 32) wire_slab_segment<4, true>(ws, sg.slab, sg.nsplit, sg.n, sm);
        else wire_slab_segment<16, true>(ws, sg.slab, sg.nsplit, sg.n, reinterpret_cast<float4(*)[64]>(sm));
      } else {
        if (sg.nsplit <= 4) wire_slab_segment<1, false>(ws, sg.slab, sg.nsplit, sg.n, sm);
        else if (sg.nsplit <= 32) wire_slab_segment<4, false>(ws, sg.slab, sg.nsplit, sg.n, sm);
        else wire_slab_segment<16, false>(ws, sg.slab, sg.nsplit, sg.n, reinterpret_cast<float4(*)[64]>(sm));
      }
      continue;
    }
    const float* gs = g + sg.off;
    const size_t n4 = sg.n / 4, stride = (size_t)gridDim.x * blockDim.x;
    for (size_t q = (size_t)blockIdx.x * blockDim.x + threadIdx.x; q < n4; q += stride) {
      const float4 G = nt_ld4(gs + q * 4);
      *(uint2*)(ws + q * 4) = make_uint2((uint32_t)f32_to_h16(G.x) | ((uint32_t)f32_to_h16(G.y) << 16),
                                         (uint32_t)f32_to_h16(G.z) | ((uint32_t)f32_to_h16(G.w) << 16));
    }
    const size_t tl = n4 * 4 + (size_t)blockIdx.x * blockDim.x + threadIdx.x;
    if (tl < sg.n) ws[tl] = f32_to_h16(gs[tl]);
  }
}

__global__ __launch_bounds__(256) void adam_dev_scalar_kernel(float* __restrict__ p, const float* __restrict__ g,
                                                              float* __restrict__ m, float* __restrict__ v,
                                                              const float* __restrict__ hyper, size_t n) {
  if (hyper[9] != 0.f) return;
  const Adam a{p, g, m, v, hyper[0], hyper[1], hyper[2], hyper[3], hyper[4], hyper[5], hyper[6], hyper[7], hyper[8]};
  for (size_t i = (size_t)blockIdx.x * blockDim.x + threadIdx.x; i < n; i += (size_t)gridDim.x * blockDim.x)
    a.upd(p[i], g[i], m[i], v[i]);
}

__device__ __forceinline__ void adam_hyper_advance(int* step_dev, double lr, double b1, double b2, double eps, float* hyper) {
  int step = *step_dev + 1;
  *step_dev = step;
  double bc1 = 1.0 - pow(b1, (double)step);
  double bc2 = 1.0 - pow(b2, (double)step);
  hyper[0] = (float)b1; hyper[1] = (float)b2; hyper[2] = (float)(1.0 - b1); hyper[3] = (float)(1.0 - b2);
  hyper[4] = (float)eps; hyper[5] = (float)(lr / bc1); hyper[6] = (float)(1.0 / sqrt(bc2));
}
__global__ void adam_hyper_kernel(int* step_dev, double lr, double b1, double b2, double eps, double wd, double ginv, float* hyper) {
  hyper[7] = (float)wd;
  hyper[8] = (float)ginv;
  hyper[9] = 0.f;
  adam_hyper_advance(step_dev, lr, b1, b2, eps, hyper);
}
__global__ void adam_hyper3_kernel(int* step_dev, double lr, double b1, double b2, double eps, double wd, const int* amp,
                                   int slot, float* hyper) {
  const int skip = amp[RG_AMP_FLAG + slot] != 0;
  hyper[7] = (float)wd;
  hyper[8] = ldexpf(1.f, -amp[RG_AMP_LATCH + slot]);
  hyper[9] = skip ? 1.f : 0.f;
  if (!skip) adam_hyper_advance(step_dev, lr, b1, b2, eps, hyper);
}

template <class F>
__global__ __launch_bounds__(256) void reduce1_kernel(F f, size_t n, float* partial) {
  __shared__ float sm[4];
  float s = 0.f;
  size_t stride = (size_t)gridDim.x * blockDim.x;
  for (size_t i = (size_t)blockIdx.x * blockDim.x + threadIdx.x; i < n; i += stride) s += f(i);
  float t = block_sum_256(s, sm);
  if (threadIdx.x == 0) partial[blockIdx.x] = t;
}
template <class Fin>
__global__ __launch_bounds__(256) void reduce2_kernel(Fin fin, const float* partial, int nb) {
  __shared__ float sm[4];
  float s = 0.f;
  for (int i = threadIdx.x; i < nb; i += 256) s += partial[i];
  float t = block_sum_256(s, sm);
  if (threadIdx.x == 0) fin(t);
}
struct SqF {
  const float* x;
  __device__ float operator()(size_t i) const { float v = x[i]; return v * v; }
};
struct StoreFin {
  float* out;
  __device__ void operator()(float t) const { out[0] = t; }
};

__global__ __launch_bounds__(256) void nchw_chan_partial_kernel(const float* g, float* partial, int N, int C, int HW,
                                                                int chunks) {
  __shared__ float sm[4];
  int c = blockIdx.x, ch = blockIdx.y;
  size_t per = ((size_t)N * HW + chunks - 1) / chunks;
  size_t b = (size_t)ch * per, e = b + per;
  size_t tot = (size_t)N * HW;
  if (e > tot) e = tot;
  float s = 0.f;
  for (size_t i = b + threadIdx.x; i < e; i += 256) {
    size_t n = i / HW, hw = i - n * HW;
    s += g[(n * C + c) * (size_t)HW + hw];
  }
  float t = block_sum_256(s, sm);
  if (threadIdx.x == 0) partial[(size_t)c * chunks + ch] = t;
}
__global__ void nchw_chan_final_kernel(const float* partial, float* out, int C, int chunks, int accumulate) {
  int c = blockIdx.x * blockDim.x + threadIdx.x;
  if (c >= C) return;
  float s = 0.f;
  for (int i = 0; i < chunks; ++i) s += partial[(size_t)c * chunks + i];
  out[c] = accumulate ? out[c] + s : s;
}

__global__ void gp_coef_kernel(const float* sq, float* loss, float* coef, float lambd, float in_inv, float out_scale,
                               const int* scale_exp) {
  if (scale_exp) rg_gp_scales_from_exp(*scale_exp, in_inv, out_scale);
  float nrm = sqrtf(sq[0]) * in_inv;
  loss[0] = (nrm - 1.f) * (nrm - 1.f);
  coef[0] = lambd * 2.f * (nrm - 1.f) / nrm * (in_inv * out_scale);
}

__global__ __launch_bounds__(256) void mean_diff_kernel(const float* a, const float* b, float* out, int n, float sign) {
  __shared__ float sm[4];
  float s = 0.f;
  for (int i = threadIdx.x; i < n; i += 256) s += b ? (a[i] - b[i]) : a[i];
  float t = block_sum_256(s, sm);
  if (threadIdx.x == 0) out[0] = sign * t / (float)n;
}

__global__ __launch_bounds__(256) void latent_prep_kernel(const float* __restrict__ u, const float* __restrict__ z,
                                                          float* __restrict__ out, int N, int E) {
  __shared__ float sm[4][64];
  const int col = threadIdx.x & 63, rg = threadIdx.x >> 6;
  const int e = blockIdx.x * 64 + col;
  const bool ok = e < E;
  float v[16];
  float s = 0.f;
#pragma unroll
  for (int k = 0; k < 16; ++k) {
    const int n = rg + 4 * k;
    v[k] = 0.f;
    if (ok && n < N) v[k] = u[(size_t)n * E + e] + z[(size_t)n * E + e];
    s += v[k];
  }
  sm[rg][col] = s;
  __syncthreads();
  const float mu = (sm[0][col] + sm[1][col] + sm[2][col] + sm[3][col]) / (float)N;
  __syncthreads();
  float ss = 0.f;
#pragma unroll
  for (int k = 0; k < 16; ++k) {
    const float d = v[k] - mu;
    if (rg + 4 * k < N) ss += d * d;
  }
  sm[rg][col] = ss;
  __syncthreads();
  const float sd = sqrtf((sm[0][col] + sm[1][col] + sm[2][col] + sm[3][col]) / (float)(N - 1));
#pragma unroll
  for (int k = 0; k < 16; ++k) {
    const int n = rg + 4 * k;
    if (ok && n < N) out[(size_t)n * E + e] = (v[k] - mu) / sd;
  }
}
__global__ void latent_prep_big_kernel(const float* u, const float* z, float* out, int N, int E) {
  int e = blockIdx.x * blockDim.x + threadIdx.x;
  if (e >= E) return;
  float s = 0.f;
  for (int n = 0; n < N; ++n) s += u[(size_t)n * E + e] + z[(size_t)n * E + e];
  float mu = s / (float)N;
  float ss = 0.f;
  for (int n = 0; n < N; ++n) {
    float d = u[(size_t)n * E + e] + z[(size_t)n * E + e] - mu;
    ss += d * d;
// ... 568 lines not shown
```

rna_gan_amd/csrc/rg_wgrad8.hip:

```cpp
#include "rg_gather.h"
#include <stdlib.h>
#include <type_traits>

namespace {

template <int V> using ic = std::integral_constant<int, V>;
typedef unsigned u32x2_t __attribute__((ext_vector_type(2)));

struct W8Args {
  const uint16_t* low[2];
  const uint16_t* high[2];
  unsigned low_bytes, high_bytes;
  int Kseg[2];
  float* out;
  int O, I;
  int lgWo, lgHo, Hh, Wh;
  int tiles_c, tiles_o, nsplit;
  int kt_per_split;
  int accumulate;
  float* ap; float* am; float* av; uint16_t* ash; const float* hyper;
  int slab16;
  unsigned low_plane, high_plane;
};

__device__ __forceinline__ void w8_store_slab16(const float* cs, uint16_t* tile, long long ldw, int rows, int t) {
  const int c8 = (t & 15) * 8, r32 = t >> 4;
#pragma unroll 4
  for (int p = 0; p < rows / 32; ++p) {
    const int row = r32 + 32 * p;
    const float4 a = *reinterpret_cast<const float4*>(cs + row * 128 + c8);
    const float4 b = *reinterpret_cast<const float4*>(cs + row * 128 + c8 + 4);
    uint4 o;
    o.x = (uint32_t)f32_to_h16(a.x) | ((uint32_t)f32_to_h16(a.y) << 16);
    o.y = (uint32_t)f32_to_h16(a.z) | ((uint32_t)f32_to_h16(a.w) << 16);
    o.z = (uint32_t)f32_to_h16(b.x) | ((uint32_t)f32_to_h16(b.y) << 16);
    o.w = (uint32_t)f32_to_h16(b.z) | ((uint32_t)f32_to_h16(b.w) << 16);
    *reinterpret_cast<uint4*>(tile + (long long)row * ldw + c8) = o;
  }
}

__device__ __forceinline__ int w8_swz(int row) { return ((row & 3) << 2) | ((row >> 2) & 3); }

template <bool ADAM, int NP = 0, int MF = 32>
__global__ __launch_bounds__(512, 2) void wgrad8_kernel(W8Args g) {
  constexpr int NAT = MF == 32 ? 2 : 4;
  constexpr int NBT = MF == 32 ? 1 : 2;
  constexpr int NKS = MF == 32 ? 4 : 2;
  constexpr int KSB = MF == 32 ? 4096 : 8192;
  constexpr int HT = 64 * 256;
  constexpr int STAGE = 4 * HT;
  constexpr int OFF_B = 0, OFF_A = 2 * HT;
  constexpr int LDS_BYTES = 2 * STAGE;
  __shared__ __attribute__((aligned(16))) uint4 lds[LDS_BYTES / 16];
  if constexpr (ADAM) {
    if (g.hyper[9] != 0.f) return;
  }

  const int t = threadIdx.x;
  const int wave = __builtin_amdgcn_readfirstlane(t >> 6);
  const int lane = t & 63;
  const int ntiles = g.tiles_o * g.tiles_c;
  const int total = ntiles * g.nsplit;
  int wid = blockIdx.x;
  {
    const int q = total >> 3, r = total & 7, xcd = wid & 7, j = wid >> 3;
    wid = (xcd < r ? xcd * (q + 1) : r * (q + 1) + (xcd - r) * q) + j;
  }
  const int zs = wid / ntiles;
  const int tid = wid - zs * ntiles;
  const int tile_o = tid / g.tiles_c, tile_c = tid - tile_o * g.tiles_c;
  const int o0 = tile_o * 256, c0 = tile_c * 256;
  const int Ktot = g.Kseg[0] + g.Kseg[1];
  const int nkt_all = ((Ktot + 63) >> 6) * (NP > 0 ? NP : 1);
  const int kt_begin = zs * g.kt_per_split;
  const int nkt = min(nkt_all, kt_begin + g.kt_per_split) - kt_begin;
  constexpr unsigned OOB = 0x80000000u;

  const __amdgpu_buffer_rsrc_t rsL0 = __builtin_amdgcn_make_buffer_rsrc((void*)g.low[0], 0, g.low_bytes, 0x00020000);
  const __amdgpu_buffer_rsrc_t rsH0 = __builtin_amdgcn_make_buffer_rsrc((void*)g.high[0], 0, g.high_bytes, 0x00020000);
  const __amdgpu_buffer_rsrc_t rsL1 = __builtin_amdgcn_make_buffer_rsrc((void*)g.low[1], 0, g.low_bytes, 0x00020000);
  const __amdgpu_buffer_rsrc_t rsH1 = __builtin_amdgcn_make_buffer_rsrc((void*)g.high[1], 0, g.high_bytes, 0x00020000);

  const int lrow = wave * 4 + (lane >> 4);
  const int lc = (lane & 15) ^ ((((lane >> 4) & 3) << 2) | (wave & 3));
  const int Wo = 1 << g.lgWo, Ho = 1 << g.lgHo;
  int a_off[2];
  int b_ci[2], b_kh[2], b_kw[2];
#pragma unroll
  for (int h = 0; h < 2; ++h) {
    a_off[h] = (lrow * g.O + o0 + h * 128 + lc * 8) * 2;
    const int col = c0 + h * 128 + lc * 8;
    const int tap = col / g.I;
    b_ci[h] = (col - tap * g.I) * 2;
    b_kh[h] = tap >> 2;
    b_kw[h] = tap & 3;
  }
  char* const ldsb = reinterpret_cast<char*>(lds);

  int px_base[2], px_h[2], px_w[2];
  bool px_ok[2];
  int px_plane = 0;
  auto flat_tile = [&](int ktr, int& lo_off, int& hi_off) -> int {
    int q = kt_begin + ktr;
    lo_off = 0; hi_off = 0;
    if constexpr (NP > 0) {
      const int pp = q % NP;
      q = q / NP;
      lo_off = ((0x120100 >> (4 * pp)) & 15) * (int)g.low_plane;
      hi_off = ((0x102010 >> (4 * pp)) & 15) * (int)g.high_plane;
    }
    return q * 64;
  };
  auto decode_pixels = [&](int ktr) {
    int lo_off;
    const int p0 = flat_tile(ktr, lo_off, px_plane);
    const bool seg1 = p0 >= g.Kseg[0];
    const int pb = seg1 ? p0 - g.Kseg[0] : p0;
    const int kend = (ktr < nkt) ? (seg1 ? g.Kseg[1] : g.Kseg[0]) : 0;
#pragma unroll
    for (int jj = 0; jj < 2; ++jj) {
      const int p = pb + jj * 32 + lrow;
      px_ok[jj] = p < kend;
      const int wo = p & (Wo - 1), ho = (p >> g.lgWo) & (Ho - 1), n = p >> (g.lgWo + g.lgHo);
      px_h[jj] = 2 * ho - 1;
      px_w[jj] = 2 * wo - 1;
      px_base[jj] = n * g.Hh;
    }
  };
  auto issue_a = [&](auto S, auto H, int ktr) {
    constexpr int s = decltype(S)::value, h = decltype(H)::value;
    int lo_off, hi_off;
    const int p0 = flat_tile(ktr, lo_off, hi_off);
    const bool seg1 = p0 >= g.Kseg[0];
    const int pb = seg1 ? p0 - g.Kseg[0] : p0;
    const int kend = (ktr < nkt) ? (seg1 ? g.Kseg[1] : g.Kseg[0]) : 0;
    const __amdgpu_buffer_rsrc_t rs = seg1 ? rsL1 : rsL0;
    const int so = pb * g.O * 2 + lo_off;
#pragma unroll
    for (int jj = 0; jj < 2; ++jj) {
      const bool ok = pb + jj * 32 + lrow < kend;
      const unsigned vo = ok ? (unsigned)(a_off[h] + jj * 64 * g.O + so) : OOB;
      __builtin_amdgcn_raw_ptr_buffer_load_lds(rs, (lds_vptr_t)(ldsb + s * STAGE + OFF_A + h * HT + jj * 8192 + wave * 1024),
                                               16, vo, 0, 0, 0);
    }
  };
  auto issue_b = [&](auto S, auto H, int ktr) {
    constexpr int s = decltype(S)::value, h = decltype(H)::value;
    if (h == 0) decode_pixels(ktr);
    int lo_off, hi_off;
    const bool seg1 = flat_tile(ktr, lo_off, hi_off) >= g.Kseg[0];
    const __amdgpu_buffer_rsrc_t rs = seg1 ? rsH1 : rsH0;
#pragma unroll
    for (int jj = 0; jj < 2; ++jj) {
      const int hi = px_h[jj] + b_kh[h], wi = px_w[jj] + b_kw[h];
      const bool v = px_ok[jj] && (unsigned)hi < (unsigned)g.Hh && (unsigned)wi < (unsigned)g.Wh;
      const unsigned vo = v ? (unsigned)(((px_base[jj] + hi) * g.Wh + wi) * g.I * 2 + b_ci[h] + px_plane) : OOB;
      __builtin_amdgcn_raw_ptr_buffer_load_lds(rs, (lds_vptr_t)(ldsb + s * STAGE + OFF_B + h * HT + jj * 8192 + wave * 1024),
                                               16, vo, 0, 0, 0);
    }
  };

  const int wm = wave >> 2, wn = wave & 3;
  const int grp = lane >> 4, idx = lane & 15;
  const int q = idx >> 2, p4 = idx & 3, fh = grp >> 1, cb = grp & 1;
  const unsigned lds_base = (unsigned)(size_t)(lds_vptr_t)lds;
  auto frag_addr = [&](int tile, int hi) -> unsigned {
    const int oct = MF == 32 ? fh : grp;
    const int prow = 8 * oct + q + 4 * hi;
    const int ca = MF == 32 ? tile * 4 + 2 * cb + (p4 >> 1) : tile * 2 + (p4 >> 1);
    const int swz = (q << 2) | ((2 * oct + hi) & 3);
    return (unsigned)(prow * 256 + ((ca ^ swz) << 4) + (p4 & 1) * 8);
  };
  unsigned aA[2][NAT][2], bA[2][NBT][2];
#pragma unroll
  for (int s = 0; s < 2; ++s)
#pragma unroll
    for (int hl = 0; hl < 2; ++hl) {
#pragma unroll
      for (int ti = 0; ti < NAT; ++ti) aA[s][ti][hl] = lds_base + s * STAGE + OFF_A + frag_addr(wm * NAT + ti, hl);
#pragma unroll
      for (int tj = 0; tj < NBT; ++tj) bA[s][tj][hl] = lds_base + s * STAGE + OFF_B + frag_addr(wn * NBT + tj, hl);
    }
  using acc_t = std::conditional_t<MF == 32, f32x16_t, rg_f32x4>;
  constexpr int NACC = NAT * NBT, ACC_R = MF == 32 ? 16 : 4;
  acc_t acc[2][2][NACC];
#pragma unroll
  for (int i = 0; i < 2; ++i)
#pragma unroll
    for (int j = 0; j < 2; ++j)
#pragma unroll
      for (int s = 0; s < NACC; ++s)
#pragma unroll
        for (int r = 0; r < ACC_R; ++r) acc[i][j][s][r] = 0.f;
  u32x2_t aR[16];
  u32x2_t bS[3][8];

#define W8_DSR(dst, addr, off) \
  asm volatile("ds_read_b64_tr_b16 %0, %1 offset:%2" : "=v"(dst) : "v"(addr), "n"(off) : "memory")
#define W8_READ_A(S, H)                                                                                   \
  do {                                                                                                    \
    _Pragma("unroll") for (int ks_ = 0; ks_ < NKS; ++ks_) _Pragma("unroll") for (int ti_ = 0; ti_ < NAT; ++ti_) { \
      W8_DSR(aR[(ti_ * NKS + ks_) * 2], aA[S][ti_][0], (H) * HT + ks_ * KSB);                             \
      W8_DSR(aR[(ti_ * NKS + ks_) * 2 + 1], aA[S][ti_][1], (H) * HT + ks_ * KSB);                         \
    }                                                                                                     \
  } while (0)
#define W8_READ_B(S, H, SET)                                                                              \
  do {                                                                                                    \
    _Pragma("unroll") for (int ks_ = 0; ks_ < NKS; ++ks_) _Pragma("unroll") for (int tj_ = 0; tj_ < NBT; ++tj_) { \
      W8_DSR(bS[SET][(tj_ * NKS + ks_) * 2], bA[S][tj_][0], (H) * HT + ks_ * KSB);                        \
      W8_DSR(bS[SET][(tj_ * NKS + ks_) * 2 + 1], bA[S][tj_][1], (H) * HT + ks_ * KSB);                    \
    }                                                                                                     \
  } while (0)
#define W8_WAIT_A()                                                                                        \
  asm volatile("s_waitcnt lgkmcnt(0)"                                                                      \
               : "+v"(aR[0]), "+v"(aR[1]), "+v"(aR[2]), "+v"(aR[3]), "+v"(aR[4]), "+v"(aR[5]), "+v"(aR[6]), "+v"(aR[7]), \
                 "+v"(aR[8]), "+v"(aR[9]), "+v"(aR[10]), "+v"(aR[11]), "+v"(aR[12]), "+v"(aR[13]), "+v"(aR[14]),        \
                 "+v"(aR[15])::"memory")
#define W8_WAIT_B(SET)                                                                                     \
  asm volatile("s_waitcnt lgkmcnt(0)"                                                                      \
               : "+v"(bS[SET][0]), "+v"(bS[SET][1]), "+v"(bS[SET][2]), "+v"(bS[SET][3]), "+v"(bS[SET][4]), \
                 "+v"(bS[SET][5]), "+v"(bS[SET][6]), "+v"(bS[SET][7])::"memory")
#define W8_FRAG(lo, hi) __builtin_bit_cast(h16x8_t, __builtin_shufflevector(lo, hi, 0, 1, 2, 3))
#define W8_MFMAS(I, J, SET)                                                                                \
  do {                                                                                                     \
    __builtin_amdgcn_s_setprio(1);                                                                         \
    _Pragma("unroll") for (int ks_ = 0; ks_ < NKS; ++ks_) _Pragma("unroll") for (int ti_ = 0; ti_ < NAT; ++ti_) \
    _Pragma("unroll") for (int tj_ = 0; tj_ < NBT; ++tj_) {                                                \
      const h16x8_t fa_ = W8_FRAG(aR[(ti_ * NKS + ks_) * 2], aR[(ti_ * NKS + ks_) * 2 + 1]);               \
      const h16x8_t fb_ = W8_FRAG(bS[SET][(tj_ * NKS + ks_) * 2], bS[SET][(tj_ * NKS + ks_) * 2 + 1]);     \
      if constexpr (MF == 32) acc[I][J][ti_ * NBT + tj_] = rg_mfma_h16_32x32x16(fa_, fb_, acc[I][J][ti_ * NBT + tj_], 0, 0, 0); \
      else acc[I][J][ti_ * NBT + tj_] = rg_mfma_h16_16x16x32(fa_, fb_, acc[I][J][ti_ * NBT + tj_], 0, 0, 0); \
    }                                                                                                      \
    __builtin_amdgcn_s_setprio(0);                                                                         \
  } while (0)
#define W8_SYNC() do { __builtin_amdgcn_sched_barrier(0); __builtin_amdgcn_s_barrier(); __builtin_amdgcn_sched_barrier(0); } while (0)
  constexpr int W_ALL = vmcnt_imm(10);
#define W8_TILE(S, SB0, SNX, U)                                                             \
  do {                                                                                      \
    W8_READ_A(S, 0);                                                                        \
    issue_a(ic<1 - (S)>{}, ic<1>{}, (U) + 1);                                               \
    __builtin_amdgcn_s_waitcnt(W_ALL);                                                      \
    W8_SYNC();                                                                              \
    W8_WAIT_A();                                                                            \
    W8_MFMAS(0, 0, SB0);                                                                    \
    W8_SYNC();                                                                              \
    W8_READ_B(S, 1, 1);                                                                     \
    issue_b(ic<(S)>{}, ic<0>{}, (U) + 2);                                                   \
    __builtin_amdgcn_s_waitcnt(W_ALL);                                                      \
    W8_SYNC();                                                                              \
    W8_WAIT_B(1);                                                                           \
    W8_MFMAS(0, 1, 1);                                                                      \
    W8_SYNC();                                                                              \
    W8_READ_A(S, 1);                                                                        \
    issue_a(ic<(S)>{}, ic<0>{}, (U) + 2);                                                   \
    __builtin_amdgcn_s_waitcnt(W_ALL);                                                      \
    W8_SYNC();                                                                              \
    W8_WAIT_A();                                                                            \
    W8_MFMAS(1, 1, 1);                                                                      \
    W8_SYNC();                                                                              \
    W8_READ_B(1 - (S), 0, SNX);                                                             \
    issue_b(ic<(S)>{}, ic<1>{}, (U) + 2);                                                   \
    __builtin_amdgcn_s_waitcnt(W_ALL);                                                      \
    W8_SYNC();                                                                              \
    W8_WAIT_B(SNX);                                                                         \
    W8_MFMAS(1, 0, SB0);                                                                    \
    W8_SYNC();                                                                              \
  } while (0)

  issue_b(ic<0>{}, ic<0>{}, 0);
  issue_a(ic<0>{}, ic<0>{}, 0);
  issue_b(ic<0>{}, ic<1>{}, 0);
  issue_a(ic<0>{}, ic<1>{}, 0);
  issue_b(ic<1>{}, ic<0>{}, 1);
  issue_a(ic<1>{}, ic<0>{}, 1);
  issue_b(ic<1>{}, ic<1>{}, 1);
  __builtin_amdgcn_s_waitcnt(W_ALL);
  W8_SYNC();
  W8_READ_B(0, 0, 0);
  W8_WAIT_B(0);
  if (wave >= 4) __builtin_amdgcn_s_barrier();
  __builtin_amdgcn_sched_barrier(0);
  for (int u = 0; u < nkt; u += 2) {
    W8_TILE(0, 0, 2, u);
    W8_TILE(1, 2, 0, u + 1);
  }
  if (wave < 4) __builtin_amdgcn_s_barrier();
  __builtin_amdgcn_sched_barrier(0);
#undef W8_TILE
#undef W8_SYNC
#undef W8_MFMAS
#undef W8_FRAG
#undef W8_WAIT_A
#undef W8_WAIT_B
#undef W8_READ_A
#undef W8_READ_B
#undef W8_DSR
  asm volatile("s_waitcnt vmcnt(0)" ::: "memory");
  __syncthreads();

  float* cs = reinterpret_cast<float*>(lds);
  const int fr = lane & 31, fh2 = lane >> 5;
  const long long ldw = (long long)16 * g.I;
  float* outp = g.out + (g.nsplit > 1 ? (long long)zs * g.O * ldw : 0);
  const int c4 = (t & 31) * 4, rr = t >> 5;
#pragma unroll
  for (int ep = 0; ep < 2; ++ep) {
    if (ep) __syncthreads();
#pragma unroll
    for (int i = 0; i < 2; ++i)
#pragma unroll
      for (int ti = 0; ti < NAT; ++ti)
#pragma unroll
        for (int tj = 0; tj < NBT; ++tj)
#pragma unroll
          for (int r = 0; r < ACC_R; ++r) {
            const int row = MF == 32 ? i * 128 + wm * 64 + ti * 32 + (r & 3) + 8 * (r >> 2) + 4 * fh2
                                     : i * 128 + wm * 64 + ti * 16 + 4 * (lane >> 4) + r;
            const int col = MF == 32 ? wn * 32 + fr : wn * 32 + tj * 16 + (lane & 15);
            cs[row * 128 + col] = acc[i][ep][ti * NBT + tj][r];
          }
    __syncthreads();
    if constexpr (ADAM) {
      RgAdamHyper hy;
      hy.load(g.hyper);
#pragma unroll 1
      for (int pq = 0; pq < 4; ++pq) {
        typedef float f32x4_nt __attribute__((ext_vector_type(4)));
        f32x4_nt P[4], M[4], V[4];
        long long off[4];
#pragma unroll
        for (int k = 0; k < 4; ++k) {
          const int row = rr + 16 * (4 * pq + k);
          off[k] = (long long)(o0 + row) * ldw + c0 + ep * 128 + c4;
          P[k] = *reinterpret_cast<const f32x4_nt*>(g.ap + off[k]);
          M[k] = __builtin_nontemporal_load(reinterpret_cast<const f32x4_nt*>(g.am + off[k]));
          V[k] = __builtin_nontemporal_load(reinterpret_cast<const f32x4_nt*>(g.av + off[k]));
        }
#pragma unroll
        for (int k = 0; k < 4; ++k) {
          const int row = rr + 16 * (4 * pq + k);
          const float4 gv = *reinterpret_cast<const float4*>(cs + row * 128 + c4);
          float pe[4] = {P[k].x, P[k].y, P[k].z, P[k].w}, me[4] = {M[k].x, M[k].y, M[k].z, M[k].w};
          float ve[4] = {V[k].x, V[k].y, V[k].z, V[k].w};
          const float ge[4] = {gv.x, gv.y, gv.z, gv.w};
#pragma unroll
          for (int e = 0; e < 4; ++e) hy.upd(pe[e], ge[e], me[e], ve[e]);
          *reinterpret_cast<f32x4_nt*>(g.ap + off[k]) = f32x4_nt{pe[0], pe[1], pe[2], pe[3]};
          __builtin_nontemporal_store(f32x4_nt{me[0], me[1], me[2], me[3]}, reinterpret_cast<f32x4_nt*>(g.am + off[k]));
          __builtin_nontemporal_store(f32x4_nt{ve[0], ve[1], ve[2], ve[3]}, reinterpret_cast<f32x4_nt*>(g.av + off[k]));
          if (g.ash)
            *reinterpret_cast<uint2*>(g.ash + off[k]) =
                make_uint2((uint32_t)f32_to_h16(pe[0]) | ((uint32_t)f32_to_h16(pe[1]) << 16),
                           (uint32_t)f32_to_h16(pe[2]) | ((uint32_t)f32_to_h16(pe[3]) << 16));
        }
      }
    } else if (g.slab16) {
      w8_store_slab16(cs, reinterpret_cast<uint16_t*>(g.out) + ((long long)zs * g.O + o0) * ldw + c0 + ep * 128, ldw, 256, t);
    } else {
#pragma unroll 4
      for (int p = 0; p < 16; ++p) {
        const int row = rr + 16 * p;
        float4* d = reinterpret_cast<float4*>(outp + (long long)(o0 + row) * ldw + c0 + ep * 128 + c4);
        float4 v = *reinterpret_cast<const float4*>(cs + row * 128 + c4);
        if (g.accumulate) {
          const float4 a = *d;
          v.x += a.x; v.y += a.y; v.z += a.z; v.w += a.w;
        }
        *d = v;
      }
    }
  }
}


template <int NP = 0>
__global__ __launch_bounds__(512, 2) void wgrad8n_kernel(W8Args g) {
  constexpr int HT = 64 * 256;
  constexpr int STAGE = 5 * HT;
  constexpr int OFF_B = 0, OFF_A = 4 * HT;
  constexpr int LDS_BYTES = 2 * STAGE;
  __shared__ __attribute__((aligned(16))) uint4 lds[LDS_BYTES / 16];

  const int t = threadIdx.x;
  const int wave = __builtin_amdgcn_readfirstlane(t >> 6);
  const int lane = t & 63;
  const int ntiles = g.tiles_o * g.tiles_c;
  const int total = ntiles * g.nsplit;
  int wid = blockIdx.x;
  {
    const int q = total >> 3, r = total & 7, xcd = wid & 7, j = wid >> 3;
    wid = (xcd < r ? xcd * (q + 1) : r * (q + 1) + (xcd - r) * q) + j;
  }
  const int zs = wid / ntiles;
  const int tid = wid - zs * ntiles;
  const int tile_o = tid / g.tiles_c, tile_c = tid - tile_o * g.tiles_c;
  const int o0 = tile_o * 128, c0 = tile_c * 512;
  const int Ktot = g.Kseg[0] + g.Kseg[1];
  const int nkt_all = ((Ktot + 63) >> 6) * (NP > 0 ? NP : 1);
  const int kt_begin = zs * g.kt_per_split;
  const int nkt = min(nkt_all, kt_begin + g.kt_per_split) - kt_begin;
  constexpr unsigned OOB = 0x80000000u;

  const __amdgpu_buffer_rsrc_t rsL0 = __builtin_amdgcn_make_buffer_rsrc((void*)g.low[0], 0, g.low_bytes, 0x00020000);
  const __amdgpu_buffer_rsrc_t rsH0 = __builtin_amdgcn_make_buffer_rsrc((void*)g.high[0], 0, g.high_bytes, 0x00020000);
  const __amdgpu_buffer_rsrc_t rsL1 = __builtin_amdgcn_make_buffer_rsrc((void*)g.low[1], 0, g.low_bytes, 0x00020000);
  const __amdgpu_buffer_rsrc_t rsH1 = __builtin_amdgcn_make_buffer_rsrc((void*)g.high[1], 0, g.high_bytes, 0x00020000);

  const int lrow = wave * 4 + (lane >> 4);
  const int lc = (lane & 15) ^ ((((lane >> 4) & 3) << 2) | (wave & 3));
  const int Wo = 1 << g.lgWo, Ho = 1 << g.lgHo;
  const int a_off = (lrow * g.O + o0 + lc * 8) * 2;
  int b_ci[4], b_kh[4], b_kw[4];
#pragma unroll
  for (int h = 0; h < 4; ++h) {
    const int col = c0 + h * 128 + lc * 8;
    const int tap = col / g.I;
    b_ci[h] = (col - tap * g.I) * 2;
    b_kh[h] = tap >> 2;
    b_kw[h] = tap & 3;
  }
  char* const ldsb = reinterpret_cast<char*>(lds);

  int px_base[2], px_h[2], px_w[2];
  bool px_ok[2];
  int px_plane = 0;
  auto flat_tile = [&](int ktr, int& lo_off, int& hi_off) -> int {
    int q = kt_begin + ktr;
    lo_off = 0; hi_off = 0;
    if constexpr (NP > 0) {
      const int pp = q % NP;
      q = q / NP;
      lo_off = ((0x120100 >> (4 * pp)) & 15) * (int)g.low_plane;
      hi_off = ((0x102010 >> (4 * pp)) & 15) * (int)g.high_plane;
    }
    return q * 64;
  };
  auto decode_pixels = [&](int ktr) {
    int lo_off;
    const int p0 = flat_tile(ktr, lo_off, px_plane);
    const bool seg1 = p0 >= g.Kseg[0];
    const int pb = seg1 ? p0 - g.Kseg[0] : p0;
    const int kend = (ktr < nkt) ? (seg1 ? g.Kseg[1] : g.Kseg[0]) : 0;
#pragma unroll
    for (int jj = 0; jj < 2; ++jj) {
      const int p = pb + jj * 32 + lrow;
      px_ok[jj] = p < kend;
      const int wo = p & (Wo - 1), ho = (p >> g.lgWo) & (Ho - 1), n = p >> (g.lgWo + g.lgHo);
      px_h[jj] = 2 * ho - 1;
      px_w[jj] = 2 * wo - 1;
      px_base[jj] = n * g.Hh;
    }
  };
  auto issue_a = [&](auto S, int ktr) {
    constexpr int s = decltype(S)::value;
    int lo_off, hi_off;
    const int p0 = flat_tile(ktr, lo_off, hi_off);
    const bool seg1 = p0 >= g.Kseg[0];
    const int pb = seg1 ? p0 - g.Kseg[0] : p0;
    const int kend = (ktr < nkt) ? (seg1 ? g.Kseg[1] : g.Kseg[0]) : 0;
    const __amdgpu_buffer_rsrc_t rs = seg1 ? rsL1 : rsL0;
    const int so = pb * g.O * 2 + lo_off;
#pragma unroll
    for (int jj = 0; jj < 2; ++jj) {
      const bool ok = pb + jj * 32 + lrow < kend;
      const unsigned vo = ok ? (unsigned)(a_off + jj * 64 * g.O + so) : OOB;
      __builtin_amdgcn_raw_ptr_buffer_load_lds(rs, (lds_vptr_t)(ldsb + s * STAGE + OFF_A + jj * 8192 + wave * 1024), 16, vo, 0, 0, 0);
    }
  };
  auto issue_b = [&](auto S, auto H, int ktr) {
    constexpr int s = decltype(S)::value, h = decltype(H)::value;
    if (h == 0) decode_pixels(ktr);
    int lo_off, hi_off;
    const bool seg1 = flat_tile(ktr, lo_off, hi_off) >= g.Kseg[0];
    const __amdgpu_buffer_rsrc_t rs = seg1 ? rsH1 : rsH0;
#pragma unroll
    for (int jj = 0; jj < 2; ++jj) {
      const int hi = px_h[jj] + b_kh[h], wi = px_w[jj] + b_kw[h];
      const bool v = px_ok[jj] && (unsigned)hi < (unsigned)g.Hh && (unsigned)wi < (unsigned)g.Wh;
      const unsigned vo = v ? (unsigned)(((px_base[jj] + hi) * g.Wh + wi) * g.I * 2 + b_ci[h] + px_plane) : OOB;
      __builtin_amdgcn_raw_ptr_buffer_load_lds(rs, (lds_vptr_t)(ldsb + s * STAGE + OFF_B + h * HT + jj * 8192 + wave * 1024),
                                               16, vo, 0, 0, 0);
    }
  };

  const int wm = wave >> 2, wn = wave & 3;
  const int grp = lane >> 4, idx = lane & 15;
  const int q = idx >> 2, p4 = idx & 3, fh = grp >> 1, cb = grp & 1;
  const int f1 = (q << 2) | (2 * fh), f2 = (q << 2) | (2 * fh + 1);
  const unsigned lds_base = (unsigned)(size_t)(lds_vptr_t)lds;
  auto frag_addr = [&](int cb32, int hi) -> unsigned {
    const int prow = 8 * fh + q + 4 * hi;
    const int ca = cb32 * 4 + 2 * cb + (p4 >> 1);
    return (unsigned)(prow * 256 + ((ca ^ (hi ? f2 : f1)) << 4) + (p4 & 1) * 8);
  };
  unsigned aA[2][2][2], bA[2][2];
#pragma unroll
  for (int s = 0; s < 2; ++s)
#pragma unroll
    for (int hl = 0; hl < 2; ++hl) {
#pragma unroll
      for (int ti = 0; ti < 2; ++ti) aA[s][ti][hl] = lds_base + s * STAGE + OFF_A + frag_addr(wm * 2 + ti, hl);
      bA[s][hl] = lds_base + s * STAGE + OFF_B + frag_addr(wn, hl);
    }
  f32x16_t acc[4][2];
#pragma unroll
  for (int j = 0; j < 4; ++j)
#pragma unroll
    for (int s = 0; s < 2; ++s)
#pragma unroll
      for (int r = 0; r < 16; ++r) acc[j][s][r] = 0.f;
  u32x2_t aR[2][4][2];
  u32x2_t bS[3][4][2];

#define WN_DSR(dst, addr, off) \
  asm volatile("ds_read_b64_tr_b16 %0, %1 offset:%2" : "=v"(dst) : "v"(addr), "n"(off) : "memory")
#define WN_READ_A(S)                                                                                      \
  do {                                                                                                    \
    _Pragma("unroll") for (int ks_ = 0; ks_ < 4; ++ks_) _Pragma("unroll") for (int ti_ = 0; ti_ < 2; ++ti_) { \
      WN_DSR(aR[ti_][ks_][0], aA[S][ti_][0], ks_ * 4096);                                                 \
      WN_DSR(aR[ti_][ks_][1], aA[S][ti_][1], ks_ * 4096);                                                 \
    }                                                                                                     \
  } while (0)
#define WN_READ_B(S, H, SET)                                                                              \
  do {                                                                                                    \
    _Pragma("unroll") for (int ks_ = 0; ks_ < 4; ++ks_) {                                                 \
      WN_DSR(bS[SET][ks_][0], bA[S][0], (H) * HT + ks_ * 4096);                                           \
      WN_DSR(bS[SET][ks_][1], bA[S][1], (H) * HT + ks_ * 4096);                                           \
    }                                                                                                     \
  } while (0)
#define WN_WAIT_A()                                                                                        \
  asm volatile("s_waitcnt lgkmcnt(0)"                                                                      \
               : "+v"(aR[0][0][0]), "+v"(aR[0][0][1]), "+v"(aR[0][1][0]), "+v"(aR[0][1][1]), "+v"(aR[0][2][0]), \
                 "+v"(aR[0][2][1]), "+v"(aR[0][3][0]), "+v"(aR[0][3][1]), "+v"(aR[1][0][0]), "+v"(aR[1][0][1]), \
                 "+v"(aR[1][1][0]), "+v"(aR[1][1][1]), "+v"(aR[1][2][0]), "+v"(aR[1][2][1]), "+v"(aR[1][3][0]), \
                 "+v"(aR[1][3][1])::"memory")
#define WN_WAIT_B(SET)                                                                                     \
  asm volatile("s_waitcnt lgkmcnt(0)"                                                                      \
               : "+v"(bS[SET][0][0]), "+v"(bS[SET][0][1]), "+v"(bS[SET][1][0]), "+v"(bS[SET][1][1]),       \
                 "+v"(bS[SET][2][0]), "+v"(bS[SET][2][1]), "+v"(bS[SET][3][0]), "+v"(bS[SET][3][1])::"memory")
#define WN_FRAG(lo, hi) __builtin_bit_cast(h16x8_t, __builtin_shufflevector(lo, hi, 0, 1, 2, 3))
#define WN_MFMAS(J, SET)                                                                                   \
  do {                                                                                                     \
    __builtin_amdgcn_s_setprio(1);                                                                         \
    _Pragma("unroll") for (int ks_ = 0; ks_ < 4; ++ks_) _Pragma("unroll") for (int ti_ = 0; ti_ < 2; ++ti_) \
        acc[J][ti_] = rg_mfma_h16_32x32x16(WN_FRAG(aR[ti_][ks_][0], aR[ti_][ks_][1]),   \
                                                              WN_FRAG(bS[SET][ks_][0], bS[SET][ks_][1]),   \
                                                              acc[J][ti_], 0, 0, 0);                       \
    __builtin_amdgcn_s_setprio(0);                                                                         \
  } while (0)
#define WN_SYNC() do { __builtin_amdgcn_sched_barrier(0); __builtin_amdgcn_s_barrier(); __builtin_amdgcn_sched_barrier(0); } while (0)
  constexpr int WN_ALL = vmcnt_imm(12);
#define WN_TILE(S, U)                                                                       \
  do {                                                                                      \
    WN_READ_A(S);                                                                           \
    issue_b(ic<1 - (S)>{}, ic<2>{}, (U) + 1);                                               \
    __builtin_amdgcn_s_waitcnt(WN_ALL);                                                     \
    WN_SYNC();                                                                              \
    WN_WAIT_A();                                                                            \
    WN_MFMAS(0, 0);                                                                         \
    WN_SYNC();                                                                              \
    WN_READ_B(S, 1, 1);                                                                     \
    issue_b(ic<1 - (S)>{}, ic<3>{}, (U) + 1);                                               \
    issue_b(ic<(S)>{}, ic<0>{}, (U) + 2);                                                   \
    __builtin_amdgcn_s_waitcnt(WN_ALL);                                                     \
    WN_SYNC();                                                                              \
    WN_WAIT_B(1);                                                                           \
    WN_MFMAS(1, 1);                                                                         \
    WN_SYNC();                                                                              \
    WN_READ_B(S, 2, 2);                                                                     \
    issue_a(ic<(S)>{}, (U) + 2);                                                            \
    __builtin_amdgcn_s_waitcnt(WN_ALL);                                                     \
    WN_SYNC();                                                                              \
    WN_WAIT_B(2);                                                                           \
    WN_MFMAS(2, 2);                                                                         \
    WN_SYNC();                                                                              \
    WN_READ_B(S, 3, 1);                                                                     \
    WN_READ_B(1 - (S), 0, 0);                                                               \
    issue_b(ic<(S)>{}, ic<1>{}, (U) + 2);                                                   \
    __builtin_amdgcn_s_waitcnt(WN_ALL);                                                     \
    WN_SYNC();                                                                              \
    WN_WAIT_B(1);                                                                           \
    WN_WAIT_B(0);                                                                           \
    WN_MFMAS(3, 1);                                                                         \
    WN_SYNC();                                                                              \
  } while (0)

  issue_b(ic<0>{}, ic<0>{}, 0);
  issue_a(ic<0>{}, 0);
  issue_b(ic<0>{}, ic<1>{}, 0);
  issue_b(ic<0>{}, ic<2>{}, 0);
  issue_b(ic<0>{}, ic<3>{}, 0);
  issue_b(ic<1>{}, ic<0>{}, 1);
  issue_a(ic<1>{}, 1);
  issue_b(ic<1>{}, ic<1>{}, 1);
  __builtin_amdgcn_s_waitcnt(WN_ALL);
  WN_SYNC();
  WN_READ_B(0, 0, 0);
  WN_WAIT_B(0);
  if (wave >= 4) __builtin_amdgcn_s_barrier();
  __builtin_amdgcn_sched_barrier(0);
  for (int u = 0; u < nkt; u += 2) {
    WN_TILE(0, u);
    WN_TILE(1, u + 1);
  }
  if (wave < 4) __builtin_amdgcn_s_barrier();
  __builtin_amdgcn_sched_barrier(0);
#undef WN_TILE
#undef WN_SYNC
#undef WN_MFMAS
#undef WN_FRAG
#undef WN_WAIT_A
#undef WN_WAIT_B
#undef WN_READ_A
#undef WN_READ_B
#undef WN_DSR
  asm volatile("s_waitcnt vmcnt(0)" ::: "memory");
  __syncthreads();

  float* cs = reinterpret_cast<float*>(lds);
  const int fr = lane & 31, fh2 = lane >> 5;
  const long long ldw = (long long)16 * g.I;
  float* outp = g.out + (g.nsplit > 1 ? (long long)zs * g.O * ldw : 0);
  const int c4 = (t & 31) * 4, rr = t >> 5;
#pragma unroll
  for (int ep = 0; ep < 4; ++ep) {
    if (ep) __syncthreads();
#pragma unroll
    for (int s = 0; s < 2; ++s)
#pragma unroll
      for (int r = 0; r < 16; ++r) {
        const int row = wm * 64 + s * 32 + (r & 3) + 8 * (r >> 2) + 4 * fh2;
        cs[row * 128 + wn * 32 + fr] = acc[ep][s][r];
      }
    __syncthreads();
    if (g.slab16) {
      w8_store_slab16(cs, reinterpret_cast<uint16_t*>(g.out) + ((long long)zs * g.O + o0) * ldw + c0 + ep * 128, ldw, 128, t);
      continue;
    }
#pragma unroll 4
    for (int p = 0; p < 8; ++p) {
      const int row = rr + 16 * p;
      float4* d = reinterpret_cast<float4*>(outp + (long long)(o0 + row) * ldw + c0 + ep * 128 + c4);
      float4 v = *reinterpret_cast<const float4*>(cs + row * 128 + c4);
      if (g.accumulate) {
        const float4 a = *d;
        v.x += a.x; v.y += a.y; v.z += a.z; v.w += a.w;
      }
      *d = v;
    }
  }
}

}

#ifndef RG_WGRAD8_KERNEL_ONLY
bool rg_wgrad8_supported(int K, int O, int I) {
  return O % 256 == 0 && (16 * I) % 256 == 0 && I % 8 == 0 && K >= 256;
}

int rg_wgrad8_split(int K, int O, int I, int* kt_per_split) {
  const int tiles = (O / 256) * (16 * I / 256);
  const int nkt = (K + 63) / 64;
  const int target = rg_option("wgrad8_blocks", 256);
  int ns = (target + tiles - 1) / tiles;
  if (ns < 1) ns = 1;
  int per = (nkt + ns - 1) / ns;
  if (per < 4) per = 4;
  per = (per + 1) & ~1;
  ns = (nkt + per - 1) / per;
  *kt_per_split = per;
  return ns;
}

bool rg_wgrad8n_supported(int K, int O, int I) {
  return O % 128 == 0 && O % 256 != 0 && (16 * I) % 512 == 0 && I % 8 == 0 && K >= 256;
}
int rg_wgrad8n_split(int K, int O, int I, int* kt_per_split) {
  const int tiles = (O / 128) * (16 * I / 512);
  const int nkt = (K + 63) / 64;
  const int target = rg_option("wgrad8_blocks", 256);
  int ns = (target + tiles - 1) / tiles;
  if (ns < 1) ns = 1;
  int per = (nkt + ns - 1) / ns;
  if (per < 4) per = 4;
  per = (per + 1) & ~1;
  ns = (nkt + per - 1) / per;
  *kt_per_split = per;
  return ns;
}
int rg_wgrad8n_launch(const void* low0, const void* high0, const void* low1, const void* high1, float* out, int Kseg,
                      int two, int O, int I, int Ho, int Wo, int nsplit, int kt_per_split, int accumulate, hipStream_t st,
                      int slab16) {
  W8Args g{};
  g.low[0] = (const uint16_t*)low0; g.high[0] = (const uint16_t*)high0;
  g.low[1] = (const uint16_t*)(two ? low1 : low0); g.high[1] = (const uint16_t*)(two ? high1 : high0);
  g.low_bytes = (unsigned)((size_t)Kseg * O * 2); g.high_bytes = (unsigned)((size_t)Kseg * 4 * I * 2);
  g.Kseg[0] = Kseg; g.Kseg[1] = two ? Kseg : 0;
  g.out = out; g.O = O; g.I = I;
  g.lgWo = rg_ilog2(Wo); g.lgHo = rg_ilog2(Ho); g.Hh = 2 * Ho; g.Wh = 2 * Wo;
  g.tiles_o = O / 128; g.tiles_c = 16 * I / 512; g.nsplit = nsplit; g.kt_per_split = kt_per_split;
  g.accumulate = nsplit == 1 ? accumulate : 0;
  g.slab16 = nsplit > 1 ? slab16 : 0;
  hipLaunchKernelGGL(wgrad8n_kernel<0>, dim3((unsigned)(g.tiles_o * g.tiles_c * nsplit)), dim3(512), 0, st, g);
  RG_LAUNCH_CHECK("conv_wgrad(mfma, ping-pong, 128 x 512)");
  return RG_OK;
}

int rg_wgrad8_launch(const void* low0, const void* high0, const void* low1, const void* high1, float* out, int Kseg,
                     int two, int O, int I, int Ho, int Wo, int nsplit, int kt_per_split, int accumulate,
                     hipStream_t st, int slab16) {
  W8Args g{};
  g.low[0] = (const uint16_t*)low0; g.high[0] = (const uint16_t*)high0;
  g.low[1] = (const uint16_t*)(two ? low1 : low0); g.high[1] = (const uint16_t*)(two ? high1 : high0);
  g.low_bytes = (unsigned)((size_t)Kseg * O * 2); g.high_bytes = (unsigned)((size_t)Kseg * 4 * I * 2);
  g.Kseg[0] = Kseg; g.Kseg[1] = two ? Kseg : 0;
  g.out = out; g.O = O; g.I = I;
  g.lgWo = rg_ilog2(Wo); g.lgHo = rg_ilog2(Ho); g.Hh = 2 * Ho; g.Wh = 2 * Wo;
  g.tiles_o = O / 256; g.tiles_c = 16 * I / 256; g.nsplit = nsplit; g.kt_per_split = kt_per_split;
  g.accumulate = nsplit == 1 ? accumulate : 0;
  g.slab16 = nsplit > 1 ? slab16 : 0;
  if (rg_option("wgrad8_mfma", RG_WGRAD8_MFMA_DEFAULT) == 16)
    hipLaunchKernelGGL((wgrad8_kernel<false, 0, 16>), dim3((unsigned)(g.tiles_o * g.tiles_c * nsplit)), dim3(512), 0, st, g);
  else
    hipLaunchKernelGGL((wgrad8_kernel<false, 0, 32>), dim3((unsigned)(g.tiles_o * g.tiles_c * nsplit)), dim3(512), 0, st, g);
  RG_LAUNCH_CHECK("conv_wgrad(mfma, ping-pong)");
  return RG_OK;
}

int rg_wgrad8_wire_launch(const void* low0, const void* high0, const void* low1, const void* high1, uint16_t* out16, int Kseg,
                          int two, int O, int I, int Ho, int Wo, int kt_per_split, hipStream_t st) {
  W8Args g{};
  g.low[0] = (const uint16_t*)low0; g.high[0] = (const uint16_t*)high0;
  g.low[1] = (const uint16_t*)(two ? low1 : low0); g.high[1] = (const uint16_t*)(two ? high1 : high0);
  g.low_bytes = (unsigned)((size_t)Kseg * O * 2); g.high_bytes = (unsigned)((size_t)Kseg * 4 * I * 2);
  g.Kseg[0] = Kseg; g.Kseg[1] = two ? Kseg : 0;
  g.out = reinterpret_cast<float*>(out16); g.O = O; g.I = I;
  g.lgWo = rg_ilog2(Wo); g.lgHo = rg_ilog2(Ho); g.Hh = 2 * Ho; g.Wh = 2 * Wo;
  g.tiles_o = O / 256; g.tiles_c = 16 * I / 256; g.nsplit = 1; g.kt_per_split = kt_per_split;
  g.slab16 = 1;
  if (rg_option("wgrad8_mfma", RG_WGRAD8_MFMA_DEFAULT) == 16)
    hipLaunchKernelGGL((wgrad8_kernel<false, 0, 16>), dim3((unsigned)(g.tiles_o * g.tiles_c)), dim3(512), 0, st, g);
  else
    hipLaunchKernelGGL((wgrad8_kernel<false, 0, 32>), dim3((unsigned)(g.tiles_o * g.tiles_c)), dim3(512), 0, st, g);
  RG_LAUNCH_CHECK("conv_wgrad_wire(mfma, ping-pong)");
  return RG_OK;
}

int rg_wgrad8_adam_launch(const void* low0, const void* high0, const void* low1, const void* high1, int Kseg, int two, int O,
                          int I, int Ho, int Wo, int kt_per_split, float* p, float* m, float* v, uint16_t* shadow,
                          const float* hyper, hipStream_t st) {
  W8Args g{};
  g.low[0] = (const uint16_t*)low0; g.high[0] = (const uint16_t*)high0;
  g.low[1] = (const uint16_t*)(two ? low1 : low0); g.high[1] = (const uint16_t*)(two ? high1 : high0);
  g.low_bytes = (unsigned)((size_t)Kseg * O * 2); g.high_bytes = (unsigned)((size_t)Kseg * 4 * I * 2);
  g.Kseg[0] = Kseg; g.Kseg[1] = two ? Kseg : 0;
  g.out = nullptr; g.O = O; g.I = I;
  g.lgWo = rg_ilog2(Wo); g.lgHo = rg_ilog2(Ho); g.Hh = 2 * Ho; g.Wh = 2 * Wo;
  g.tiles_o = O / 256; g.tiles_c = 16 * I / 256; g.nsplit = 1; g.kt_per_split = kt_per_split;
  g.ap = p; g.am = m; g.av = v; g.ash = shadow; g.hyper = hyper;
  if (rg_option("wgrad8_mfma", RG_WGRAD8_MFMA_DEFAULT) == 16)
    hipLaunchKernelGGL((wgrad8_kernel<true, 0, 16>), dim3((unsigned)(g.tiles_o * g.tiles_c)), dim3(512), 0, st, g);
  else
    hipLaunchKernelGGL((wgrad8_kernel<true, 0, 32>), dim3((unsigned)(g.tiles_o * g.tiles_c)), dim3(512), 0, st, g);
  RG_LAUNCH_CHECK("conv_wgrad_adam(mfma, ping-pong)");
  return RG_OK;
}
#endif
```

rna_gan_amd/optim.py:

```python
from __future__ import annotations

import torch

from .models import _flat_view

from . import _abi
from ._abi import check


class Adam(torch.optim.Adam):
    def __init__(self, params, lr=1e-3, betas=(0.9, 0.999), eps=1e-8, weight_decay=0, amsgrad=False, **kw):
        if amsgrad:
            raise NotImplementedError("rna_gan_amd.optim.Adam: amsgrad is not on the RNA-GAN path")
        super().__init__(params, lr=lr, betas=betas, eps=eps, weight_decay=weight_decay, amsgrad=False,
                         foreach=False, fused=False)
        self._module = None
        self._m = None
        self._v = None
        self._flat_id = None
        self._step_dev = None
        self._hyper = None
        self._host_steps = 0
        self.buf_gen = 0
        self.grad_wire = None
        self._ema = None

    def bind(self, module, fuse_linear_wgrad=False):
        mine = {id(p) for g in self.param_groups for p in g["params"]}
        theirs = list(module.parameters())
        if len(self.param_groups) != 1 or mine != {id(p) for p in theirs}:
            raise ValueError("rna_gan_amd.optim.Adam: one param group holding exactly module.parameters() is required "
                             "(the fused kernel steps the module's whole flat buffer)")
        if not all(p.requires_grad for p in theirs):
            raise ValueError("rna_gan_amd.optim.Adam: frozen parameters (requires_grad=False) are not supported")
        self._module = module
        if fuse_linear_wgrad:
            module._fuse_linear_wgrad = True
            if hasattr(module, "_trt"):
                module._trt = None
        return self

    def attach_ema(self, ema):
        if self._module is None or ema.source is not self._module:
            raise ValueError("rna_gan_amd.optim.Adam: attach_ema needs an optimizer bound to the module the ParamEMA averages")
        if self._ema is not None and self._ema is not ema:
            raise RuntimeError("rna_gan_amd.optim.Adam: another ParamEMA is attached (detach_ema() first)")
        from . import dist as D_
        D_.flush()
        ema._attach(self)
        self._ema = ema
        self.buf_gen += 1
        return ema

    def detach_ema(self):
        ema, self._ema = self._ema, None
        if ema is not None:
            from . import dist as D_
            D_.flush()
            ema._detach()
            self.buf_gen += 1
        return ema

    def _ensure(self):
        if self._module is None:
            raise RuntimeError("rna_gan_amd.optim.Adam must be bound to its module (Adam(...).bind(module))")
        flat = self._module.flat
        if self._flat_id is not flat:
            old = {p: self.state.get(p) for p in flat.params}
            self._m = torch.zeros_like(flat.data)
            self._v = torch.zeros_like(flat.data)
            step0 = 0
            for p, (off, n) in zip(flat.params, flat.offsets):
                st = old.get(p) or {}
                m = _flat_view(self._m, off, n, p)
                v = _flat_view(self._v, off, n, p)
                if "exp_avg" in st:
                    m.copy_(st["exp_avg"]); v.copy_(st["exp_avg_sq"])
                step0 = max(step0, int(float(st.get("step", 0))))
                self.state[p] = {"step": torch.tensor(float(step0)), "exp_avg": m, "exp_avg_sq": v}
            self._host_steps = step0
            self._step_dev = torch.tensor([step0], dtype=torch.int32, device=flat.data.device)
            self._hyper = torch.zeros(12, dtype=torch.float32, device=flat.data.device)
            self._flat_id = flat
            self.buf_gen += 1
        if self._ema is not None and not torch.cuda.is_current_stream_capturing() and self._ema._rehomed():
            self.buf_gen += 1
        return flat

    def _sync_step_state(self):
        for p in (self._flat_id.params if self._flat_id is not None else []):
            self.state[p]["step"] = torch.tensor(float(self._host_steps))

    def _amp(self):
        return getattr(getattr(self._module, "_rt_ops", None), "amp", None) if self._module is not None else None

    def state_dict(self):
        from . import dist as D_
        D_.flush()
        if self._amp() is not None and self._step_dev is not None:
            self._host_steps = int(self._step_dev.item())
        self._sync_step_state()
        return super().state_dict()

    def load_state_dict(self, state_dict):
        from . import dist as D_
        D_.flush()
        super().load_state_dict(state_dict)
        flat = self._flat_id
        if flat is None or self._module is None or self._module._rt_flat is not flat:
            self._flat_id = None
            return
        step0 = 0
        with torch.no_grad():
            for p, (off, n) in zip(flat.params, flat.offsets):
                st = self.state.get(p) or {}
                m, v = _flat_view(self._m, off, n, p), _flat_view(self._v, off, n, p)
                if "exp_avg" in st:
                    m.copy_(st["exp_avg"]); v.copy_(st["exp_avg_sq"])
                else:
                    m.zero_(); v.zero_()
                step0 = max(step0, int(float(st.get("step", 0))))
                self.state[p] = {"step": torch.tensor(float(step0)), "exp_avg": m, "exp_avg_sq": v}
            self._step_dev.fill_(step0)
        self._host_steps = step0

    def zero_grad(self, set_to_none: bool = False):
        if self._module is not None and not set_to_none:
            from . import dist as D_
            D_.flush()
            self._module.flat.grad.zero_()

    def note_replayed(self):
        self._host_steps += 1
        if self._ema is not None:
            self._ema.module.weights_changed()

    @torch.no_grad()
    def step(self, closure=None):
        flat = self._ensure()
        g = self.param_groups[0]
        mops = getattr(self._module, "_rt_ops", None)
        lib = mops.lib if mops is not None else _abi.load()
        ginv = 1.0 / float(getattr(mops, "loss_scale", 1.0)) if mops is not None else 1.0
        stream = torch.cuda.current_stream(flat.data.device).cuda_stream
        amp = getattr(mops, "amp", None) if mops is not None else None
        launches, probes = [], []
        if amp is None:
            check(lib.rg_adam_hyper_dev2(self._step_dev.data_ptr(), float(g["lr"]), float(g["betas"][0]),
                                         float(g["betas"][1]), float(g["eps"]), float(g.get("weight_decay", 0.0)), ginv,
                                         self._hyper.data_ptr(), stream),
                  "rg_adam_hyper_dev2")
        H16 = getattr(mops, "H16", _abi.RG_BF16)

        def seg(t, n=None, dt=None):
            if torch.is_tensor(t):
                return (t.data_ptr(), t.numel() if n is None else n, _abi.RG_F32 if t.dtype == torch.float32 else H16)
            return (t, n, dt)
        shadow = flat.shadow
        lo = 0
        g0 = getattr(getattr(self._module, "_rt_net", None), "g0", None)
        pend = None if g0 is None else g0.pending_wgrad
        if pend is not None:
            g0.pending_wgrad = None
            z, gy, dt = pend
            off = (g0.w.data_ptr() - flat.data.data_ptr()) // 4
            n0 = g0.w.numel()
            if off != 0:
                raise RuntimeError("rna_gan_amd.optim.Adam: the deferred G.0 weight gradient expects that tensor at the head "
                                   "of the flat buffer")
            E, C = g0.w.shape[0], g0.w.shape[1]
            launches.append(lambda z=z, gy=gy, E=E, C=C, dt=dt: check(lib.rg_g0_wgrad_adam(
                z.data_ptr(), gy.data_ptr(), flat.data.data_ptr(), self._m.data_ptr(), self._v.data_ptr(),
                self._hyper.data_ptr(), 0 if shadow is None else shadow.data_ptr(), z.shape[0], E, C, dt, stream),
                "rg_g0_wgrad_adam"))
            probes += [seg(z), seg(gy)]
            lo = n0
        segs = []
        pend_lin = getattr(self._module, "_rg_pending_linear", None)
        if pend_lin:
            self._module._rg_pending_linear = []
            if shadow is not None or self.grad_wire is not None:
                raise RuntimeError("rna_gan_amd.optim.Adam: fused linear weight gradients expect an fp32-only, single-process step")
            for w, gT, xT, nsamp, pack in pend_lin:
                off = (w.data_ptr() - flat.data.data_ptr()) // 4
                O_, I_ = w.shape
                if not w.is_contiguous() or off < 0 or off + O_ * I_ > flat.data.numel():
                    raise RuntimeError("rna_gan_amd.optim.Adam: a pending linear weight is not a dense view of the flat buffer")
                img = None if pack is None else pack["image"]
                launches.append(lambda gT=gT, xT=xT, nsamp=nsamp, off=off, O_=O_, I_=I_, img=img: check(lib.rg_linear_wgrad_adam(
                    gT.data_ptr(), xT.data_ptr(), gT.shape[1], nsamp, flat.data.data_ptr() + 4 * off,
                    self._m.data_ptr() + 4 * off, self._v.data_ptr() + 4 * off, self._hyper.data_ptr(), O_, I_,
                    0 if img is None else img.data_ptr(), 0 if img is None else img.shape[1], stream), "rg_linear_wgrad_adam"))
                probes += [seg(gT), seg(xT)]
                if pack is not None:
                    pack["version"] = w._version
                segs.append((off, off + O_ * I_))
            segs.sort()
        slab_segs = []
        net = getattr(self._module, "_rt_net", None)
        for cw in (net.convs() if net is not None and hasattr(net, "convs") else []):
            ps = getattr(cw, "pending_slabs", None)
            if ps is not None:
                cw.pending_slabs = None
                slab_segs.append(((cw.w.data_ptr() - flat.data.data_ptr()) // 4, cw.w.numel(), ps[0], ps[1], ps[2]))
            pb = getattr(cw, "pending_bias", None)
            if pb is not None:
                cw.pending_bias = None
                slab_segs.append(((cw.bias.data_ptr() - flat.data.data_ptr()) // 4, cw.bias.numel(), pb[0], pb[1], 0))
            pw = getattr(cw, "pending_wgrad", None)
            if isinstance(pw, tuple) and isinstance(pw[0], str) and pw[0] == "conv":
                cw.pending_wgrad = None
                _, low0, high0, low1, high1, (N_, Ho_, Wo_, O_, I_), dt, algo, flops = pw
                off = (cw.w.data_ptr() - flat.data.data_ptr()) // 4
                if shadow is None or off % 4 or off < lo:
                    raise RuntimeError("rna_gan_amd.optim.Adam: a deferred single-launch weight gradient expects a bf16 step and "
                                       "a 16-byte aligned tensor inside the flat buffer")
                ops = getattr(self._module, "_rt_ops", None)
                call = lambda low0=low0, high0=high0, low1=low1, high1=high1, off=off, N_=N_, Ho_=Ho_, Wo_=Wo_, O_=O_, I_=I_, \
                    dt=dt, algo=algo: check(lib.rg_conv_wgrad_adam(
                    low0.data_ptr(), high0.data_ptr(), 0 if low1 is None else low1.data_ptr(),
                    0 if high1 is None else high1.data_ptr(), flat.data.data_ptr() + 4 * off, self._m.data_ptr() + 4 * off,
                    self._v.data_ptr() + 4 * off, self._hyper.data_ptr(), shadow.data_ptr() + 2 * off, N_, Ho_, Wo_, O_, I_, dt,
                    algo, stream), "rg_conv_wgrad_adam")
                if ops is not None and hasattr(ops, "_timed"):
                    launches.append(lambda call=call, flops=flops, cw=cw, ops=ops: ops._timed("conv_wgrad_adam", flops, call, cw=cw))
                else:
                    launches.append(call)
                probes += [seg(t) for t in (low0, high0, low1, high1) if t is not None]
                slab_segs.append((off, cw.w.numel(), None, -1, 0))
        if slab_segs:
            if segs or self.grad_wire is not None:
                raise RuntimeError("rna_gan_amd.optim.Adam: deferred split-K slabs expect a single-process step without fused "
                                   "linear weight gradients")
            import ctypes as C
            slab_segs.sort(key=lambda t: t[0])
            total = flat.data.numel()
            table, pos = [], lo
            for off, n, buf, ns, sdt in slab_segs:
                if off < pos or off % 4 or n % 4 or off + n > total:
                    raise RuntimeError("rna_gan_amd.optim.Adam: a deferred weight gradient does not sit 16-byte aligned inside "
                                       "the part of the flat buffer this launch steps")
                if off > pos:
                    table.append((pos - lo, off - pos, 0, 0, 0))
                table.append((off - lo, n, 0 if buf is None else buf.data_ptr(), ns, sdt))
                pos = off + n
            if total > pos:
                table.append((pos - lo, total - pos, 0, 0, 0))
            k = len(table)
            offs = (C.c_ulonglong * k)(*[t[0] for t in table])
            lens = (C.c_ulonglong * k)(*[t[1] for t in table])
            slabs = (C.c_void_p * k)(*[t[2] or None for t in table])
            nsp = (C.c_int * k)(*[t[3] for t in table])
            sdts = (C.c_int * k)(*[t[4] for t in table])
            launches.append(lambda k=k, offs=offs, lens=lens, slabs=slabs, nsp=nsp, sdts=sdts: check(lib.rg_adam_step_slabs(
                flat.data.data_ptr() + 4 * lo, flat.grad.data_ptr() + 4 * lo, self._m.data_ptr() + 4 * lo,
                self._v.data_ptr() + 4 * lo, total - lo, self._hyper.data_ptr(),
                0 if shadow is None else shadow.data_ptr() + 2 * lo, k, C.addressof(offs), C.addressof(lens),
                C.addressof(slabs), C.addressof(nsp), C.addressof(sdts), stream), "rg_adam_step_slabs"))
            for off, n, sp, ns, sdt in table:
                if sp:
                    probes.append(seg(sp, ns * n, _abi.RG_F32 if sdt == _abi.RG_F32 else H16))
                elif ns == 0:
                    probes.append(seg(flat.grad.data_ptr() + 4 * (lo + off), n, _abi.RG_F32))
            segs = [(lo, total)]
        pos = lo
        wire = self.grad_wire
        for a, b in segs + [(flat.data.numel(), flat.data.numel())]:
            if a > pos:
                launches.append(lambda pos=pos, a=a: check(lib.rg_adam_step_dev(
                    flat.data.data_ptr() + 4 * pos, flat.grad.data_ptr() + 4 * pos, self._m.data_ptr() + 4 * pos,
                    self._v.data_ptr() + 4 * pos, a - pos, self._hyper.data_ptr(),
                    0 if shadow is None else shadow.data_ptr() + 2 * pos, 0 if wire is None else wire.data_ptr() + 2 * pos,
                    stream), "rg_adam_step_dev"))
                probes.append(seg(flat.grad.data_ptr() + 4 * pos, a - pos, _abi.RG_F32) if wire is None else
                              seg(wire.data_ptr() + 2 * pos, a - pos, H16))
            pos = max(pos, b)
        if amp is not None:
            amp.probe(lib, self._module, probes, stream)
            amp.hyper(lib, self._module, self._step_dev, g, self._hyper, stream)
        for fn in launches:
            fn()
        if self._ema is not None:
            self._ema._launch(lib, self._hyper, self._step_dev, stream)
        if amp is not None:
            amp.update(lib, self._module, stream)
        if not torch.cuda.is_current_stream_capturing():
            self._host_steps += 1
        self._module.weights_changed(by_optimizer=True)
        return None
```

Before: 6189 imgs/sec.

## Merge fused wgrad-Adam tiles and slab Adam chunks into one persistent work-queue kernel

Adds a persistent kernel that pulls work items from an atomic counter. Each item is either a fused weight-gradient+Adam MFMA tile for the one deferred conv or a chunk of the segmented slab Adam update. This replaces two back-to-back launches (conv_wgrad_adam, then adam_step_slabs), so the memory-bound Adam chunks can overlap the compute-bound tiles and the tail of the first kernel is no longer idle. It adds an atomic counter per item, a sync word that the last block must reset, and a more complex ordering and interleave of work items.

New measurement: 6244 imgs/sec (median of 6 runs). About the same (+0.9%).

```diff
diff --git a/include/rnagan_hip.h b/include/rnagan_hip.h
--- a/include/rnagan_hip.h
+++ b/include/rnagan_hip.h
@@ -234,6 +234,11 @@
 int rg_adam_step_slabs(float* p, const float* g, float* m, float* v, size_t n, const float* hyper, void* shadow_bf16, int nseg,
                        const unsigned long long* seg_off, const unsigned long long* seg_n, const void* const* seg_slab,
                        const int* seg_nsplit, const int* seg_dtype, void* stream);
+int rg_adam_step_queue(const void* low0, const void* high0, const void* low1, const void* high1, int N, int Ho, int Wo, int O,
+                       int I, int dtype, int algo, int fused_seg, float* p, const float* g, float* m, float* v, size_t n,
+                       const float* hyper, void* shadow_bf16, int nseg, const unsigned long long* seg_off,
+                       const unsigned long long* seg_n, const void* const* seg_slab, const int* seg_nsplit, const int* seg_dtype,
+                       void* sync_word, void* stream);
 int rg_grad_to_wire(const float* g, void* wire_bf16, size_t n, int nseg, const unsigned long long* seg_off,
                     const unsigned long long* seg_n, const void* const* seg_slab, const int* seg_nsplit, const int* seg_dtype,
                     void* stream);
diff --git a/rna_gan_amd/_abi.py b/rna_gan_amd/_abi.py
--- a/rna_gan_amd/_abi.py
+++ b/rna_gan_amd/_abi.py
@@ -116,6 +116,7 @@
     "rg_adam_step_dev": (_i, [_p, _p, _p, _p, _z, _p, _p, _p, _p]),
     "rg_adam_step_slabs": (_i, [_p, _p, _p, _p, _z, _p, _p, _i, _p, _p, _p, _p, _p, _p]),
     "rg_ema_update": (_i, [_p, _p, _z, _f, _p, _p, _p]),
+    "rg_adam_step_queue": (_i, [_p, _p, _p, _p, _i, _i, _i, _i, _i, _i, _i, _i, _p, _p, _p, _p, _z, _p, _p, _i, _p, _p, _p, _p, _p, _p, _p]),
     "rg_interp_dev": (_i, [_p, _p, _p, _z, _p, _p]),
     "rg_adam_hyper_dev": (_i, [_p, _d, _d, _d, _d, _d, _p, _p]),
     "rg_adam_hyper_dev2": (_i, [_p, _d, _d, _d, _d, _d, _d, _p, _p]),
@@ -185,7 +186,7 @@
     "rg_probe_fill_bf16": (_i, [_p, _z, C.c_uint, _p]),
 }
 
-ABI_VERSION = 615
+ABI_VERSION = 616
 
 _libs = {}
 LIB_PATH_F16 = os.path.join(_HERE, "librnagan_hip_f16.so")
diff --git a/rna_gan_amd/build.py b/rna_gan_amd/build.py
--- a/rna_gan_amd/build.py
+++ b/rna_gan_amd/build.py
@@ -8,8 +8,8 @@
 OUT = os.path.join(HERE, "librnagan_hip.so")
 OUT_F16 = os.path.join(HERE, "librnagan_hip_f16.so")
 OBJ = os.path.join(HERE, "csrc", "_obj")
-SOURCES = ["rg_api.hip", "rg_generic.hip", "rg_bn.hip", "rg_misc.hip", "rg_mfma.hip", "rg_conv8.hip", "rg_convp.hip", "rg_convd.hip", "rg_wgrad8.hip", "rg_skinny.hip", "rg_vae.hip", "rg_splitbn.hip", "rg_incep.hip", "rg_g0adam.hip", "rg_upimg.hip", "rg_probe.hip", "rg_conv8f.hip", "rg_wgrad8f.hip", "rg_amp.hip", "rg_plainact.hip"]
-EXTRA_DEPS = {"rg_probe.hip": ["rg_conv8.hip"], "rg_conv8f.hip": ["rg_conv8.hip"], "rg_wgrad8f.hip": ["rg_wgrad8.hip"]}
+SOURCES = ["rg_api.hip", "rg_generic.hip", "rg_bn.hip", "rg_misc.hip", "rg_mfma.hip", "rg_conv8.hip", "rg_convp.hip", "rg_convd.hip", "rg_wgrad8.hip", "rg_skinny.hip", "rg_vae.hip", "rg_splitbn.hip", "rg_incep.hip", "rg_g0adam.hip", "rg_upimg.hip", "rg_probe.hip", "rg_conv8f.hip", "rg_wgrad8f.hip", "rg_amp.hip", "rg_plainact.hip", "rg_adamq.hip"]
+EXTRA_DEPS = {"rg_probe.hip": ["rg_conv8.hip"], "rg_conv8f.hip": ["rg_conv8.hip"], "rg_wgrad8f.hip": ["rg_wgrad8.hip"], "rg_adamq.hip": ["rg_wgrad8.hip"]}
 BF16_ONLY = ("rg_probe.hip", "rg_conv8f.hip", "rg_wgrad8f.hip")
 FLAGS = ["--offload-arch=gfx950", "-O3", "-fPIC", "-std=c++17", "-Wall", "-Wno-unused-function",
          "-ffp-contract=off"]
diff --git a/rna_gan_amd/csrc/rg_adamq.hip b/rna_gan_amd/csrc/rg_adamq.hip
--- /dev/null
+++ b/rna_gan_amd/csrc/rg_adamq.hip
@@ -0,0 +1,326 @@
+#define RG_WGRAD8_KERNEL_ONLY 1
+#include "rg_wgrad8.hip"
+#include <algorithm>
+
+namespace {
+
+#include "rg_adamseg.h"
+
+struct AqArgs {
+  W8Args w;
+  float* p; const float* g; float* m; float* v; uint16_t* shadow; const float* hyper;
+  AdamSegs t;
+  int cstart[ADAM_MAX_SEGS + 1];
+  unsigned char ord[ADAM_MAX_SEGS];
+  int cel[ADAM_MAX_SEGS];
+  int nt, nc;
+  int qn, qd;
+  int i1, a1;
+  unsigned* sync;
+};
+
+#define AQ_PIN(v) asm volatile("" : "+v"((v).x), "+v"((v).y), "+v"((v).z), "+v"((v).w))
+#define AQ_PIN4(A) do { AQ_PIN((A)[0]); AQ_PIN((A)[1]); AQ_PIN((A)[2]); AQ_PIN((A)[3]); } while (0)
+
+template <bool SHADOW>
+__device__ __forceinline__ void aq_plain(const RgAdamHyper& hy, float* __restrict__ ps, const float* __restrict__ gs,
+                                         float* __restrict__ ms, float* __restrict__ vs, uint16_t* __restrict__ sh, size_t q0,
+                                         size_t q1, int t) {
+  size_t qb = q0 + t;
+  for (; qb + 3 * 512 < q1; qb += 4 * 512) {
+    float4 P[4], M[4], V[4], G[4];
+#pragma unroll
+    for (int k = 0; k < 4; ++k) {
+      const size_t i = (qb + k * 512) * 4;
+      P[k] = *(const float4*)(ps + i); M[k] = nt_ld4(ms + i); V[k] = nt_ld4(vs + i); G[k] = nt_ld4(gs + i);
+    }
+    AQ_PIN4(P);
+#pragma unroll
+    for (int k = 0; k < 4; ++k) {
+      const size_t i = (qb + k * 512) * 4;
+      hy.upd(P[k].x, G[k].x, M[k].x, V[k].x); hy.upd(P[k].y, G[k].y, M[k].y, V[k].y);
+      hy.upd(P[k].z, G[k].z, M[k].z, V[k].z); hy.upd(P[k].w, G[k].w, M[k].w, V[k].w);
+      *(float4*)(ps + i) = P[k]; nt_st4(ms + i, M[k]); nt_st4(vs + i, V[k]);
+      if (SHADOW) *(uint2*)(sh + i) = adam_pack_h16x4(P[k]);
+    }
+  }
+  for (; qb < q1; qb += 512) {
+    const size_t i = qb * 4;
+    float4 P = *(const float4*)(ps + i), M = nt_ld4(ms + i), V = nt_ld4(vs + i), G = nt_ld4(gs + i);
+    hy.upd(P.x, G.x, M.x, V.x); hy.upd(P.y, G.y, M.y, V.y); hy.upd(P.z, G.z, M.z, V.z); hy.upd(P.w, G.w, M.w, V.w);
+    *(float4*)(ps + i) = P; nt_st4(ms + i, M); nt_st4(vs + i, V);
+    if (SHADOW) *(uint2*)(sh + i) = adam_pack_h16x4(P);
+  }
+}
+
+template <bool SHADOW, bool S16, int NS>
+__device__ __forceinline__ void aq_slab1(const RgAdamHyper& hy, float* __restrict__ ps, float* __restrict__ ms,
+                                         float* __restrict__ vs, uint16_t* __restrict__ sh, const float* __restrict__ slab,
+                                         size_t n, size_t q0, size_t q1, int t) {
+  for (size_t qb = q0 + t; qb < q1; qb += 2 * 512) {
+    const bool two = qb + 512 < q1;
+    const size_t qq[2] = {qb, two ? qb + 512 : qb};
+    float4 P[2], M[2], V[2], T[2][NS];
+#pragma unroll
+    for (int c = 0; c < 2; ++c) { P[c] = *(const float4*)(ps + qq[c] * 4); M[c] = nt_ld4(ms + qq[c] * 4); V[c] = nt_ld4(vs + qq[c] * 4); }
+#pragma unroll
+    for (int z = 0; z < NS; ++z)
+#pragma unroll
+      for (int c = 0; c < 2; ++c) T[c][z] = adam_slab_ld<S16>(slab, (size_t)z, n, qq[c]);
+    AQ_PIN(P[0]); AQ_PIN(P[1]);
+    float4 s[2] = {make_float4(0.f, 0.f, 0.f, 0.f), make_float4(0.f, 0.f, 0.f, 0.f)};
+#pragma unroll
+    for (int z = 0; z < NS; ++z)
+#pragma unroll
+      for (int c = 0; c < 2; ++c) { s[c].x += T[c][z].x; s[c].y += T[c][z].y; s[c].z += T[c][z].z; s[c].w += T[c][z].w; }
+#pragma unroll
+    for (int c = 0; c < 2; ++c) {
+      if (c == 1 && !two) break;
+      const size_t i = qq[c] * 4;
+      hy.upd(P[c].x, s[c].x, M[c].x, V[c].x); hy.upd(P[c].y, s[c].y, M[c].y, V[c].y);
+      hy.upd(P[c].z, s[c].z, M[c].z, V[c].z); hy.upd(P[c].w, s[c].w, M[c].w, V[c].w);
+      *(float4*)(ps + i) = P[c]; nt_st4(ms + i, M[c]); nt_st4(vs + i, V[c]);
+      if (SHADOW) *(uint2*)(sh + i) = adam_pack_h16x4(P[c]);
+    }
+  }
+}
+template <bool SHADOW, bool S16>
+__device__ __forceinline__ void aq_slab1_any(const RgAdamHyper& hy, float* ps, float* ms, float* vs, uint16_t* sh, const float* slab,
+                                             int nsplit, size_t n, size_t q0, size_t q1, int t) {
+  if (nsplit == 1) aq_slab1<SHADOW, S16, 1>(hy, ps, ms, vs, sh, slab, n, q0, q1, t);
+  else if (nsplit == 2) aq_slab1<SHADOW, S16, 2>(hy, ps, ms, vs, sh, slab, n, q0, q1, t);
+  else if (nsplit == 3) aq_slab1<SHADOW, S16, 3>(hy, ps, ms, vs, sh, slab, n, q0, q1, t);
+  else aq_slab1<SHADOW, S16, 4>(hy, ps, ms, vs, sh, slab, n, q0, q1, t);
+}
+
+template <bool SHADOW, int SL, bool S16, int U, int ZU>
+__device__ __forceinline__ void aq_slabn(const RgAdamHyper& hy, float* __restrict__ ps, float* __restrict__ ms,
+                                         float* __restrict__ vs, uint16_t* __restrict__ sh, const float* __restrict__ slab,
+                                         int nsplit, size_t n, size_t q0, size_t q1, int t, float4* sm) {
+  constexpr int COLS = 256 / SL;
+  const int h = t >> 8, tt = t & 255, col = tt % COLS, l = tt / COLS;
+  float4* const smh = sm + (size_t)h * U * 256;
+  const size_t trips = (q1 - q0 + COLS - 1) / COLS;
+  for (size_t tb0 = 0; tb0 < trips; tb0 += 2 * U) {
+    size_t q[U], qc[U];
+    bool ok[U];
+    float4 s[U], P[U], M[U], V[U];
+#pragma unroll
+    for (int u = 0; u < U; ++u) {
+      q[u] = q0 + (tb0 + h * U + u) * COLS + col;
+      ok[u] = q[u] < q1;
+      qc[u] = ok[u] ? q[u] : q0;
+      s[u] = make_float4(0.f, 0.f, 0.f, 0.f);
+    }
+    if (l == 0) {
+#pragma unroll
+      for (int u = 0; u < U; ++u) { P[u] = *(const float4*)(ps + qc[u] * 4); M[u] = nt_ld4(ms + qc[u] * 4); V[u] = nt_ld4(vs + qc[u] * 4); }
+    }
+    for (int z = l; z < nsplit; z += ZU * SL) {
+      float4 a[ZU][U];
+#pragma unroll
+      for (int k = 0; k < ZU; ++k) {
+        const int zc = z + k * SL < nsplit ? z + k * SL : z;
+#pragma unroll
+        for (int u = 0; u < U; ++u) a[k][u] = adam_slab_ld<S16>(slab, (size_t)zc, n, qc[u]);
+      }
+#pragma unroll
+      for (int k = 0; k < ZU; ++k) {
+        const bool on = z + k * SL < nsplit;
+#pragma unroll
+        for (int u = 0; u < U; ++u)
+          if (on) { s[u].x += a[k][u].x; s[u].y += a[k][u].y; s[u].z += a[k][u].z; s[u].w += a[k][u].w; }
+      }
+    }
+    if (l == 0) {
+#pragma unroll
+      for (int u = 0; u < U; ++u) AQ_PIN(P[u]);
+    }
+    __syncthreads();
+#pragma unroll
+    for (int u = 0; u < U; ++u) smh[(u * SL + l) * COLS + col] = s[u];
+    __syncthreads();
+    if (l == 0) {
+#pragma unroll
+      for (int u = 0; u < U; ++u) {
+        if (!ok[u]) continue;
+        float4 sv = s[u];
+#pragma unroll
+        for (int k = 1; k < SL; ++k) { const float4 x = smh[(u * SL + k) * COLS + col]; sv.x += x.x; sv.y += x.y; sv.z += x.z; sv.w += x.w; }
+        const size_t i = q[u] * 4;
+        hy.upd(P[u].x, sv.x, M[u].x, V[u].x); hy.upd(P[u].y, sv.y, M[u].y, V[u].y);
+        hy.upd(P[u].z, sv.z, M[u].z, V[u].z); hy.upd(P[u].w, sv.w, M[u].w, V[u].w);
+        *(float4*)(ps + i) = P[u]; nt_st4(ms + i, M[u]); nt_st4(vs + i, V[u]);
+        if (SHADOW) *(uint2*)(sh + i) = adam_pack_h16x4(P[u]);
+      }
+    }
+  }
+}
+
+template <bool SHADOW, int SL, bool S16>
+__device__ __forceinline__ void aq_slabn_any(const RgAdamHyper& hy, float* ps, float* ms, float* vs, uint16_t* sh, const float* slab,
+                                             int nsplit, size_t n, size_t q0, size_t q1, int t, float4* sm) {
+  if (q1 - q0 <= 2 * (256 / SL)) aq_slabn<SHADOW, SL, S16, 1, 8>(hy, ps, ms, vs, sh, slab, nsplit, n, q0, q1, t, sm);
+  else if (nsplit >= 8 * SL) aq_slabn<SHADOW, SL, S16, 2, 8>(hy, ps, ms, vs, sh, slab, nsplit, n, q0, q1, t, sm);
+  else aq_slabn<SHADOW, SL, S16, 4, 2>(hy, ps, ms, vs, sh, slab, nsplit, n, q0, q1, t, sm);
+}
+
+template <bool SHADOW>
+__device__ __forceinline__ void aq_chunk(const AqArgs& a, int c, int t, float4* sm) {
+  asm volatile("" : "+v"(t));
+  RgAdamHyper hy;
+  hy.load(a.hyper);
+  int j = 0;
+  while (c >= a.cstart[j + 1]) ++j;
+  const AdamSeg sg = a.t.s[a.ord[j]];
+  float* ps = a.p + sg.off; float* ms = a.m + sg.off; float* vs = a.v + sg.off;
+  uint16_t* sh = SHADOW ? a.shadow + sg.off : nullptr;
+  const size_t cel = (size_t)a.cel[j];
+  const size_t e0 = (size_t)(c - a.cstart[j]) * cel;
+  const size_t e1 = e0 + cel < sg.n ? e0 + cel : (size_t)sg.n;
+  const size_t q0 = e0 / 4, q1 = e1 / 4;
+  if (sg.slab) {
+    const int SL = adam_slab_lanes(sg.nsplit);
+    if (sg.s16) {
+      if (SL == 1) aq_slab1_any<SHADOW, true>(hy, ps, ms, vs, sh, sg.slab, sg.nsplit, sg.n, q0, q1, t);
+      else if (SL == 4) aq_slabn_any<SHADOW, 4, true>(hy, ps, ms, vs, sh, sg.slab, sg.nsplit, sg.n, q0, q1, t, sm);
+      else aq_slabn_any<SHADOW, 16, true>(hy, ps, ms, vs, sh, sg.slab, sg.nsplit, sg.n, q0, q1, t, sm);
+    } else {
+      if (SL == 1) aq_slab1_any<SHADOW, false>(hy, ps, ms, vs, sh, sg.slab, sg.nsplit, sg.n, q0, q1, t);
+      else if (SL == 4) aq_slabn_any<SHADOW, 4, false>(hy, ps, ms, vs, sh, sg.slab, sg.nsplit, sg.n, q0, q1, t, sm);
+      else aq_slabn_any<SHADOW, 16, false>(hy, ps, ms, vs, sh, sg.slab, sg.nsplit, sg.n, q0, q1, t, sm);
+    }
+    return;
+  }
+  const float* gs = a.g + sg.off;
+  aq_plain<SHADOW>(hy, ps, gs, ms, vs, sh, q0, q1, t);
+  const size_t tl = q1 * 4 + t;
+  if (e1 == sg.n && tl < sg.n) {
+    hy.upd(ps[tl], gs[tl], ms[tl], vs[tl]);
+    if (SHADOW) sh[tl] = f32_to_h16(ps[tl]);
+  }
+}
+
+__global__ __launch_bounds__(512, 2) void adam_queue_kernel(AqArgs a) {
+  __shared__ __attribute__((aligned(16))) uint4 lds[W8_LDS_BYTES / 16];
+  __shared__ int s_item;
+  if (a.hyper[9] != 0.f) return;
+  const int t = threadIdx.x;
+  const int items = a.nt + a.nc;
+  for (;;) {
+    __syncthreads();
+    if (t == 0) s_item = (int)atomicAdd(a.sync, 1u);
+    __syncthreads();
+    const int i = __builtin_amdgcn_readfirstlane(s_item);
+    if (i >= items) {
+      if (t == 0 && i == items + (int)gridDim.x - 1) __hip_atomic_store(a.sync, 0u, __ATOMIC_RELAXED, __HIP_MEMORY_SCOPE_AGENT);
+      break;
+    }
+    bool tile;
+    int idx;
+    if (i < a.i1) {
+      const int ta = (int)((long long)i * a.qn / a.qd), tb = (int)((long long)(i + 1) * a.qn / a.qd);
+      tile = tb > ta;
+      idx = tile ? ta : i - ta;
+    } else if (a.a1 >= a.nt) {
+      tile = false; idx = i - a.nt;
+    } else {
+      tile = true; idx = i - a.nc;
+    }
+    if (tile) wgrad8_body<true, 0, 32>(a.w, idx, lds);
+    else if (a.shadow) aq_chunk<true>(a, idx, t, reinterpret_cast<float4*>(lds));
+    else aq_chunk<false>(a, idx, t, reinterpret_cast<float4*>(lds));
+  }
+}
+
+int aq_cu_count() {
+  static int n = 0;
+  if (n == 0) {
+    int dev = 0, v = 0;
+    if (hipGetDevice(&dev) == hipSuccess &&
+        hipDeviceGetAttribute(&v, hipDeviceAttributeMultiprocessorCount, dev) == hipSuccess && v > 0) n = v;
+    else n = 256;
+  }
+  return n;
+}
+
+}
+
+extern "C" int rg_adam_step_queue(const void* low0, const void* high0, const void* low1, const void* high1, int N, int Ho, int Wo,
+                                  int O, int I, int dtype, int algo, int fused_seg, float* p, const float* g, float* m, float* v,
+                                  size_t n, const float* hyper, void* shadow_bf16, int nseg, const unsigned long long* seg_off,
+                                  const unsigned long long* seg_n, const void* const* seg_slab, const int* seg_nsplit,
+                                  const int* seg_dtype, void* sync_word, void* stream) {
+  RG_REQUIRE(low0 && high0 && (low1 == nullptr) == (high1 == nullptr) && N > 0 && Ho > 0 && Wo > 0 && I > 0 && O > 0 && p && g &&
+                 m && v && hyper && seg_off && seg_n && seg_slab && seg_nsplit && seg_dtype && sync_word, RG_EINVAL,
+             "adam_step_queue: bad args");
+  RG_REQUIRE(nseg >= 1 && nseg <= ADAM_MAX_SEGS && fused_seg >= 0 && fused_seg < nseg, RG_EINVAL,
+             "adam_step_queue: 1 .. %d segments, one of them the fused tensor", ADAM_MAX_SEGS);
+  RG_REQUIRE((((uintptr_t)p | (uintptr_t)g | (uintptr_t)m | (uintptr_t)v) & 15) == 0 && ((uintptr_t)shadow_bf16 & 7) == 0 &&
+                 ((uintptr_t)sync_word & 3) == 0, RG_EINVAL, "adam_step_queue: alignment");
+  RG_REQUIRE(rg_conv_wgrad_adam_supported(N, Ho, Wo, O, I, low1 != nullptr, dtype, algo), RG_EUNSUPPORTED,
+             "adam_step_queue: shape / dtype without a single-split matrix-core plan");
+  RG_REQUIRE(seg_nsplit[fused_seg] == -1 && !seg_slab[fused_seg] && seg_n[fused_seg] == (unsigned long long)O * 16 * I, RG_EINVAL,
+             "adam_step_queue: segment %d is not the skipped segment of a [%d][16][%d] tensor", fused_seg, O, I);
+  const size_t foff = (size_t)seg_off[fused_seg];
+  void* const fshadow = shadow_bf16 ? (void*)((uint16_t*)shadow_bf16 + foff) : nullptr;
+  if (!rg_option("adamq", 1) || rg_option("wgrad8_mfma", RG_WGRAD8_MFMA_DEFAULT) == 16) {
+    const int rc = rg_conv_wgrad_adam(low0, high0, low1, high1, p + foff, m + foff, v + foff, hyper, fshadow, N, Ho, Wo, O, I,
+                                      dtype, algo, stream);
+    if (rc) return rc;
+    return rg_adam_step_slabs(p, g, m, v, n, hyper, shadow_bf16, nseg, seg_off, seg_n, seg_slab, seg_nsplit, seg_dtype, stream);
+  }
+  const int chunk = rg_option("adamq_chunk", 32) * 1024;
+  RG_REQUIRE(chunk >= 1024 && chunk <= (1 << 24), RG_EINVAL, "adam_step_queue: adamq_chunk must be 1 .. 16384 (x 1024 elements)");
+  AqArgs a{};
+  a.t.nseg = nseg;
+  unsigned long long pos = 0;
+  long long nc = 0;
+  for (int i = 0; i < nseg; ++i) {
+    RG_REQUIRE(seg_off[i] == pos && seg_off[i] % 4 == 0, RG_EINVAL, "adam_step_queue: segments must tile the range in order, "
+               "each starting on a multiple of 4 elements (segment %d)", i);
+    RG_REQUIRE(!seg_slab[i] || (seg_nsplit[i] >= 1 && seg_n[i] % 4 == 0 && ((uintptr_t)seg_slab[i] & 15) == 0 &&
+                                (seg_dtype[i] == RG_F32 || seg_dtype[i] == RG_H16)), RG_EINVAL,
+               "adam_step_queue: slab segment %d", i);
+    const int ns = seg_slab[i] ? seg_nsplit[i] : (seg_nsplit[i] < 0 ? -1 : 0);
+    a.t.s[i] = AdamSeg{seg_off[i], seg_n[i], (const float*)seg_slab[i], ns, seg_slab[i] && seg_dtype[i] == RG_H16 ? 1 : 0};
+    pos += seg_n[i];
+  }
+  RG_REQUIRE(pos == n, RG_EINVAL, "adam_step_queue: the segments cover %llu of %zu elements", pos, n);
+  for (int i = 0; i < nseg; ++i) a.ord[i] = (unsigned char)i;
+  std::stable_sort(a.ord, a.ord + nseg, [&](unsigned char x, unsigned char y) { return a.t.s[x].nsplit > a.t.s[y].nsplit; });
+  for (int j = 0; j < nseg; ++j) {
+    const AdamSeg& sg = a.t.s[a.ord[j]];
+    a.cstart[j] = (int)nc;
+    unsigned long long cel = (unsigned long long)chunk;
+    if (sg.nsplit > 0) {
+      cel = cel * 30 / (26 + (unsigned long long)sg.nsplit * (sg.s16 ? 2 : 4)) / 1024 * 1024;
+      if (cel < 1024) cel = 1024;
+    }
+    a.cel[j] = (int)cel;
+    if (sg.nsplit >= 0) nc += (long long)((sg.n + cel - 1) / cel);
+    RG_REQUIRE(nc < (1 << 24), RG_EINVAL, "adam_step_queue: %lld stream chunks (raise adamq_chunk)", nc);
+  }
+  for (int j = nseg; j <= ADAM_MAX_SEGS; ++j) a.cstart[j] = (int)nc;
+  const int Kseg = N * Ho * Wo, two = low1 != nullptr;
+  int per = 0;
+  rg_wgrad8_split((two ? 2 : 1) * Kseg, O, I, &per);
+  a.w = w8_adam_args(low0, high0, low1, high1, Kseg, two, O, I, Ho, Wo, per, p + foff, m + foff, v + foff, (uint16_t*)fshadow, hyper);
+  a.p = p; a.g = g; a.m = m; a.v = v; a.shadow = (uint16_t*)shadow_bf16; a.hyper = hyper;
+  a.nt = a.w.tiles_o * a.w.tiles_c;
+  a.nc = (int)nc;
+  const int ratio = rg_option("adamq_ratio", 0);
+  RG_REQUIRE(ratio >= 0 && ratio <= 100, RG_EINVAL, "adam_step_queue: adamq_ratio is a percentage");
+  a.qn = ratio; a.qd = 100;
+  int i1 = 0;
+  while ((long long)i1 * a.qn / a.qd < a.nt && i1 - (long long)i1 * a.qn / a.qd < a.nc) ++i1;
+  a.i1 = i1; a.a1 = (int)((long long)i1 * a.qn / a.qd);
+  a.sync = (unsigned*)sync_word;
+  int grid = rg_option("adamq_grid", 0);
+  if (grid <= 0) grid = aq_cu_count();
+  RG_REQUIRE(grid <= 4096, RG_EINVAL, "adam_step_queue: adamq_grid");
+  hipStream_t st = rg_stream(stream);
+  hipLaunchKernelGGL(adam_queue_kernel, dim3((unsigned)grid), dim3(512), 0, st, a);
+  RG_LAUNCH_CHECK("adam_step_queue");
+  return RG_OK;
+}
diff --git a/rna_gan_amd/csrc/rg_adamseg.h b/rna_gan_amd/csrc/rg_adamseg.h
--- /dev/null
+++ b/rna_gan_amd/csrc/rg_adamseg.h
@@ -0,0 +1,34 @@
+#pragma once
+#include "rg_common.h"
+
+typedef float nt_f4 __attribute__((ext_vector_type(4)));
+__device__ __forceinline__ float4 nt_ld4(const float* p) {
+  nt_f4 t = __builtin_nontemporal_load(reinterpret_cast<const nt_f4*>(p));
+  return make_float4(t.x, t.y, t.z, t.w);
+}
+__device__ __forceinline__ void nt_st4(float* p, float4 v) {
+  nt_f4 t = {v.x, v.y, v.z, v.w};
+  __builtin_nontemporal_store(t, reinterpret_cast<nt_f4*>(p));
+}
+
+constexpr int ADAM_MAX_SEGS = 24;
+struct AdamSeg { unsigned long long off, n; const float* slab; int nsplit; int s16; };
+struct AdamSegs { int nseg; int pad; AdamSeg s[ADAM_MAX_SEGS]; };
+
+template <bool S16>
+__device__ __forceinline__ float4 adam_slab_ld(const float* __restrict__ slab, size_t z, size_t n, size_t q) {
+  if (S16) {
+    typedef unsigned nt_u2 __attribute__((ext_vector_type(2)));
+    const nt_u2 w = __builtin_nontemporal_load(reinterpret_cast<const nt_u2*>(reinterpret_cast<const uint16_t*>(slab) + z * n + q * 4));
+    return make_float4(h16lo_to_f32(w.x), h16hi_to_f32(w.x), h16lo_to_f32(w.y),
+                       h16hi_to_f32(w.y));
+  }
+  return nt_ld4(slab + z * n + q * 4);
+}
+
+__host__ __device__ __forceinline__ int adam_slab_lanes(int nsplit) { return nsplit <= 4 ? 1 : (nsplit <= 32 ? 4 : 16); }
+
+__device__ __forceinline__ uint2 adam_pack_h16x4(float4 P) {
+  return make_uint2((uint32_t)f32_to_h16(P.x) | ((uint32_t)f32_to_h16(P.y) << 16),
+                    (uint32_t)f32_to_h16(P.z) | ((uint32_t)f32_to_h16(P.w) << 16));
+}
diff --git a/rna_gan_amd/csrc/rg_api.hip b/rna_gan_amd/csrc/rg_api.hip
--- a/rna_gan_amd/csrc/rg_api.hip
+++ b/rna_gan_amd/csrc/rg_api.hip
@@ -15,12 +15,13 @@
   va_end(ap);
 }
 
-extern "C" int rg_version(void) { return 615; }
+extern "C" int rg_version(void) { return 616; }
 extern "C" const char* rg_last_error(void) { return g_err; }
 
 static const char* const g_opt_names[] = {"conv8", "conv8_blocks", "conv_tile", "xcd", "class_fast", "wgrad_blocks",
                                           "wgrad8", "conv_v1", "stream_tile", "narrow8", "conv8_mfma", "conv8_epi", "wgrad8_blocks", "korder", "convp", "convp_blocks",
-                                          "fp8_mx", "wgrad8n", "f32mma", "convd", "convd_blocks", "skinny128", "slab16", "wslab16", "bn_rev", "wgrad8_mfma", "narrow32", "upimg", "upimg_blocks"};
+                                          "fp8_mx", "wgrad8n", "f32mma", "convd", "convd_blocks", "skinny128", "slab16", "wslab16", "bn_rev", "wgrad8_mfma", "narrow32", "upimg", "upimg_blocks",
+                                          "adamq", "adamq_chunk", "adamq_ratio", "adamq_grid"};
 constexpr int G_NOPT = sizeof(g_opt_names) / sizeof(g_opt_names[0]);
 static int g_opt_override[G_NOPT];
 static int g_opt_env[G_NOPT];
diff --git a/rna_gan_amd/csrc/rg_misc.hip b/rna_gan_amd/csrc/rg_misc.hip
--- a/rna_gan_amd/csrc/rg_misc.hip
+++ b/rna_gan_amd/csrc/rg_misc.hip
@@ -79,15 +79,7 @@
   __device__ void one(size_t i) const { upd(p[i], g[i], m[i], v[i]); }
 };
 
-typedef float nt_f4 __attribute__((ext_vector_type(4)));
-__device__ __forceinline__ float4 nt_ld4(const float* p) {
-  nt_f4 t = __builtin_nontemporal_load(reinterpret_cast<const nt_f4*>(p));
-  return make_float4(t.x, t.y, t.z, t.w);
-}
-__device__ __forceinline__ void nt_st4(float* p, float4 v) {
-  nt_f4 t = {v.x, v.y, v.z, v.w};
-  __builtin_nontemporal_store(t, reinterpret_cast<nt_f4*>(p));
-}
+#include "rg_adamseg.h"
 template <bool WIRE, bool SHADOW>
 __global__ __launch_bounds__(256) void adam_dev_kernel(float* __restrict__ p, const float* __restrict__ g,
                                                        float* __restrict__ m, float* __restrict__ v,
@@ -139,21 +131,6 @@
   }
   const size_t t = n4 * 4 + (size_t)blockIdx.x * blockDim.x + threadIdx.x;
   if (t < n) e[t] = e[t] + omd * (p[t] - e[t]);
-}
-
-constexpr int ADAM_MAX_SEGS = 24;
-struct AdamSeg { unsigned long long off, n; const float* slab; int nsplit; int s16; };
-struct AdamSegs { int nseg; int pad; AdamSeg s[ADAM_MAX_SEGS]; };
-
-template <bool S16>
-__device__ __forceinline__ float4 adam_slab_ld(const float* __restrict__ slab, size_t z, size_t n, size_t q) {
-  if (S16) {
-    typedef unsigned nt_u2 __attribute__((ext_vector_type(2)));
-    const nt_u2 w = __builtin_nontemporal_load(reinterpret_cast<const nt_u2*>(reinterpret_cast<const uint16_t*>(slab) + z * n + q * 4));
-    return make_float4(h16lo_to_f32(w.x), h16hi_to_f32(w.x), h16lo_to_f32(w.y),
-                       h16hi_to_f32(w.y));
-  }
-  return nt_ld4(slab + z * n + q * 4);
 }
 
 template <bool SHADOW, int SL, bool S16>
diff --git a/rna_gan_amd/csrc/rg_wgrad8.hip b/rna_gan_amd/csrc/rg_wgrad8.hip
--- a/rna_gan_amd/csrc/rg_wgrad8.hip
+++ b/rna_gan_amd/csrc/rg_wgrad8.hip
@@ -41,8 +41,10 @@
 
 __device__ __forceinline__ int w8_swz(int row) { return ((row & 3) << 2) | ((row >> 2) & 3); }
 
-template <bool ADAM, int NP = 0, int MF = 32>
-__global__ __launch_bounds__(512, 2) void wgrad8_kernel(W8Args g) {
+constexpr int W8_LDS_BYTES = 2 * 4 * 64 * 256;
+
+template <bool ADAM, int NP, int MF>
+__device__ __forceinline__ void wgrad8_body(const W8Args& g, const int wid, uint4* const lds) {
   constexpr int NAT = MF == 32 ? 2 : 4;
   constexpr int NBT = MF == 32 ? 1 : 2;
   constexpr int NKS = MF == 32 ? 4 : 2;
@@ -50,22 +52,12 @@
   constexpr int HT = 64 * 256;
   constexpr int STAGE = 4 * HT;
   constexpr int OFF_B = 0, OFF_A = 2 * HT;
-  constexpr int LDS_BYTES = 2 * STAGE;
-  __shared__ __attribute__((aligned(16))) uint4 lds[LDS_BYTES / 16];
-  if constexpr (ADAM) {
-    if (g.hyper[9] != 0.f) return;
-  }
+  static_assert(2 * STAGE == W8_LDS_BYTES, "stage LDS");
 
   const int t = threadIdx.x;
   const int wave = __builtin_amdgcn_readfirstlane(t >> 6);
   const int lane = t & 63;
   const int ntiles = g.tiles_o * g.tiles_c;
-  const int total = ntiles * g.nsplit;
-  int wid = blockIdx.x;
-  {
-    const int q = total >> 3, r = total & 7, xcd = wid & 7, j = wid >> 3;
-    wid = (xcd < r ? xcd * (q + 1) : r * (q + 1) + (xcd - r) * q) + j;
-  }
   const int zs = wid / ntiles;
   const int tid = wid - zs * ntiles;
   const int tile_o = tid / g.tiles_c, tile_c = tid - tile_o * g.tiles_c;
@@ -370,6 +362,21 @@
       }
     }
   }
+}
+
+template <bool ADAM, int NP = 0, int MF = 32>
+__global__ __launch_bounds__(512, 2) void wgrad8_kernel(W8Args g) {
+  __shared__ __attribute__((aligned(16))) uint4 lds[W8_LDS_BYTES / 16];
+  if constexpr (ADAM) {
+    if (g.hyper[9] != 0.f) return;
+  }
+  const int total = g.tiles_o * g.tiles_c * g.nsplit;
+  int wid = blockIdx.x;
+  {
+    const int q = total >> 3, r = total & 7, xcd = wid & 7, j = wid >> 3;
+    wid = (xcd < r ? xcd * (q + 1) : r * (q + 1) + (xcd - r) * q) + j;
+  }
+  wgrad8_body<ADAM, NP, MF>(g, wid, lds);
 }
 
 
@@ -651,6 +658,21 @@
   }
 }
 
+inline W8Args w8_adam_args(const void* low0, const void* high0, const void* low1, const void* high1, int Kseg, int two, int O,
+                           int I, int Ho, int Wo, int kt_per_split, float* p, float* m, float* v, uint16_t* shadow,
+                           const float* hyper) {
+  W8Args g{};
+  g.low[0] = (const uint16_t*)low0; g.high[0] = (const uint16_t*)high0;
+  g.low[1] = (const uint16_t*)(two ? low1 : low0); g.high[1] = (const uint16_t*)(two ? high1 : high0);
+  g.low_bytes = (unsigned)((size_t)Kseg * O * 2); g.high_bytes = (unsigned)((size_t)Kseg * 4 * I * 2);
+  g.Kseg[0] = Kseg; g.Kseg[1] = two ? Kseg : 0;
+  g.out = nullptr; g.O = O; g.I = I;
+  g.lgWo = rg_ilog2(Wo); g.lgHo = rg_ilog2(Ho); g.Hh = 2 * Ho; g.Wh = 2 * Wo;
+  g.tiles_o = O / 256; g.tiles_c = 16 * I / 256; g.nsplit = 1; g.kt_per_split = kt_per_split;
+  g.ap = p; g.am = m; g.av = v; g.ash = shadow; g.hyper = hyper;
+  return g;
+}
+
 }
 
 #ifndef RG_WGRAD8_KERNEL_ONLY
@@ -749,15 +771,7 @@
 int rg_wgrad8_adam_launch(const void* low0, const void* high0, const void* low1, const void* high1, int Kseg, int two, int O,
                           int I, int Ho, int Wo, int kt_per_split, float* p, float* m, float* v, uint16_t* shadow,
                           const float* hyper, hipStream_t st) {
-  W8Args g{};
-  g.low[0] = (const uint16_t*)low0; g.high[0] = (const uint16_t*)high0;
-  g.low[1] = (const uint16_t*)(two ? low1 : low0); g.high[1] = (const uint16_t*)(two ? high1 : high0);
-  g.low_bytes = (unsigned)((size_t)Kseg * O * 2); g.high_bytes = (unsigned)((size_t)Kseg * 4 * I * 2);
-  g.Kseg[0] = Kseg; g.Kseg[1] = two ? Kseg : 0;
-  g.out = nullptr; g.O = O; g.I = I;
-  g.lgWo = rg_ilog2(Wo); g.lgHo = rg_ilog2(Ho); g.Hh = 2 * Ho; g.Wh = 2 * Wo;
-  g.tiles_o = O / 256; g.tiles_c = 16 * I / 256; g.nsplit = 1; g.kt_per_split = kt_per_split;
-  g.ap = p; g.am = m; g.av = v; g.ash = shadow; g.hyper = hyper;
+  const W8Args g = w8_adam_args(low0, high0, low1, high1, Kseg, two, O, I, Ho, Wo, kt_per_split, p, m, v, shadow, hyper);
   if (rg_option("wgrad8_mfma", RG_WGRAD8_MFMA_DEFAULT) == 16)
     hipLaunchKernelGGL((wgrad8_kernel<true, 0, 16>), dim3((unsigned)(g.tiles_o * g.tiles_c)), dim3(512), 0, st, g);
   else
diff --git a/rna_gan_amd/optim.py b/rna_gan_amd/optim.py
--- a/rna_gan_amd/optim.py
+++ b/rna_gan_amd/optim.py
@@ -1,4 +1,6 @@
 from __future__ import annotations
+
+import os
 
 import torch
 
@@ -9,6 +11,8 @@
 
 
 class Adam(torch.optim.Adam):
+    QUEUE_LAUNCH = os.environ.get("RNAGAN_ADAM_QUEUE", "1") != "0"
+
     def __init__(self, params, lr=1e-3, betas=(0.9, 0.999), eps=1e-8, weight_decay=0, amsgrad=False, **kw):
         if amsgrad:
             raise NotImplementedError("rna_gan_amd.optim.Adam: amsgrad is not on the RNA-GAN path")
@@ -20,6 +24,7 @@
         self._flat_id = None
         self._step_dev = None
         self._hyper = None
+        self._queue_sync = None
         self._host_steps = 0
         self.buf_gen = 0
         self.grad_wire = None
@@ -81,6 +86,7 @@
             self._host_steps = step0
             self._step_dev = torch.tensor([step0], dtype=torch.int32, device=flat.data.device)
             self._hyper = torch.zeros(12, dtype=torch.float32, device=flat.data.device)
+            self._queue_sync = torch.zeros(1, dtype=torch.int32, device=flat.data.device)
             self._flat_id = flat
             self.buf_gen += 1
         if self._ema is not None and not torch.cuda.is_current_stream_capturing() and self._ema._rehomed():
@@ -197,6 +203,7 @@
                 segs.append((off, off + O_ * I_))
             segs.sort()
         slab_segs = []
+        fused = []
         net = getattr(self._module, "_rt_net", None)
         for cw in (net.convs() if net is not None and hasattr(net, "convs") else []):
             ps = getattr(cw, "pending_slabs", None)
@@ -222,10 +229,10 @@
                     0 if high1 is None else high1.data_ptr(), flat.data.data_ptr() + 4 * off, self._m.data_ptr() + 4 * off,
                     self._v.data_ptr() + 4 * off, self._hyper.data_ptr(), shadow.data_ptr() + 2 * off, N_, Ho_, Wo_, O_, I_, dt,
                     algo, stream), "rg_conv_wgrad_adam")
+                wrap = None
                 if ops is not None and hasattr(ops, "_timed"):
-                    launches.append(lambda call=call, flops=flops, cw=cw, ops=ops: ops._timed("conv_wgrad_adam", flops, call, cw=cw))
-                else:
-                    launches.append(call)
+                    wrap = lambda fn, flops=flops, cw=cw, ops=ops: ops._timed("conv_wgrad_adam", flops, fn, cw=cw)
+                fused.append((off, (low0, high0, low1, high1, N_, Ho_, Wo_, O_, I_, dt, algo), call, wrap))
                 probes += [seg(t) for t in (low0, high0, low1, high1) if t is not None]
                 slab_segs.append((off, cw.w.numel(), None, -1, 0))
         if slab_segs:
@@ -252,11 +259,27 @@
             slabs = (C.c_void_p * k)(*[t[2] or None for t in table])
             nsp = (C.c_int * k)(*[t[3] for t in table])
             sdts = (C.c_int * k)(*[t[4] for t in table])
-            launches.append(lambda k=k, offs=offs, lens=lens, slabs=slabs, nsp=nsp, sdts=sdts: check(lib.rg_adam_step_slabs(
+            tail = lambda k=k, offs=offs, lens=lens, slabs=slabs, nsp=nsp, sdts=sdts: check(lib.rg_adam_step_slabs(
                 flat.data.data_ptr() + 4 * lo, flat.grad.data_ptr() + 4 * lo, self._m.data_ptr() + 4 * lo,
                 self._v.data_ptr() + 4 * lo, total - lo, self._hyper.data_ptr(),
                 0 if shadow is None else shadow.data_ptr() + 2 * lo, k, C.addressof(offs), C.addressof(lens),
-                C.addressof(slabs), C.addressof(nsp), C.addressof(sdts), stream), "rg_adam_step_slabs"))
+                C.addressof(slabs), C.addressof(nsp), C.addressof(sdts), stream), "rg_adam_step_slabs")
+            if len(fused) == 1 and self.QUEUE_LAUNCH:
+                foff, (low0, high0, low1, high1, N_, Ho_, Wo_, O_, I_, dt, algo), _, wrap = fused[0]
+                fseg = [i for i, t in enumerate(table) if t[0] == foff - lo and t[3] == -1][0]
+                tail = lambda k=k, offs=offs, lens=lens, slabs=slabs, nsp=nsp, sdts=sdts, low0=low0, high0=high0, low1=low1, \
+                    high1=high1, N_=N_, Ho_=Ho_, Wo_=Wo_, O_=O_, I_=I_, dt=dt, algo=algo, fseg=fseg: check(lib.rg_adam_step_queue(
+                    low0.data_ptr(), high0.data_ptr(), 0 if low1 is None else low1.data_ptr(),
+                    0 if high1 is None else high1.data_ptr(), N_, Ho_, Wo_, O_, I_, dt, algo, fseg,
+                    flat.data.data_ptr() + 4 * lo, flat.grad.data_ptr() + 4 * lo, self._m.data_ptr() + 4 * lo,
+                    self._v.data_ptr() + 4 * lo, total - lo, self._hyper.data_ptr(), shadow.data_ptr() + 2 * lo, k,
+                    C.addressof(offs), C.addressof(lens), C.addressof(slabs), C.addressof(nsp), C.addressof(sdts),
+                    self._queue_sync.data_ptr(), stream), "rg_adam_step_queue")
+                launches.append(tail if wrap is None else (lambda tail=tail, wrap=wrap: wrap(tail)))
+            else:
+                launches += [call if wrap is None else (lambda call=call, wrap=wrap: wrap(call)) for _, _, call, wrap in fused]
+                launches.append(tail)
+            fused = []
             for off, n, sp, ns, sdt in table:
                 if sp:
                     probes.append(seg(sp, ns * n, _abi.RG_F32 if sdt == _abi.RG_F32 else H16))
```
